# moberweger/deep-prior-pp

Measured on AMD Instinct MI355X. Metric: depth-crops/sec (NYU ResNet50 bs128) 1/2/4/8 GPU; mean 3D joint err (mm), higher is better.
Workload: dtype f32; 1 GPU; NYU posereg_embedding ResNet (type 0, 30-D PCA prior) train step: fused augment + fwd + bwd + ADAM, bs128/GPU fp32, 128x128x1 crops; global_batch=128, parallelism=dp1, augment=True, augment_pipelined=True, bn=local per-GPU batch statistics, launch_mode=native

## Files before the change

deep-prior-pp_amd/csrc/elementwise.hip:

```cpp
#include "dpp_common.h"

namespace {

__global__ __launch_bounds__(DPP_THREADS) void colsum_partial_kernel(const float* __restrict__ X, int M, int C, int rpb,
                                                                     float* __restrict__ partial) {
    __shared__ float s[DPP_THREADS];
    const int tid = threadIdx.x;
    const int RP = DPP_THREADS / C > 0 ? DPP_THREADS / C : 1;
    const int r_begin = blockIdx.x * rpb;
    const int r_end = (r_begin + rpb < M) ? r_begin + rpb : M;
    for (int c0 = 0; c0 < C; c0 += DPP_THREADS) {
        int cw = (C - c0 < DPP_THREADS) ? C - c0 : DPP_THREADS;
        int rp = DPP_THREADS / cw;
        int c = tid % cw, rr = tid / cw;
        float acc = 0.0f;
        if (rr < rp)
            for (int r = r_begin + rr; r < r_end; r += rp) acc += X[(size_t)r * C + c0 + c];
        s[tid] = acc;
        __syncthreads();
        if (tid < cw) {
            double a = 0.0;
            for (int j = 0; j < rp; ++j) a += (double)s[j * cw + tid];
            partial[(size_t)blockIdx.x * C + c0 + tid] = (float)a;
        }
        __syncthreads();
    }
    (void)RP;
}

__global__ __launch_bounds__(DPP_THREADS) void loss_sse_kernel(const float* __restrict__ out, const float* __restrict__ y, int n,
                                                               float inv_denom, float* __restrict__ cost,
                                                               float* __restrict__ dout) {
    __shared__ double s[DPP_THREADS];
    double acc = 0.0;
    for (int i = threadIdx.x; i < n; i += DPP_THREADS) {
        float d = out[i] - y[i];
        acc += (double)d * (double)d;
        if (dout) dout[i] = 2.0f * inv_denom * d;
    }
    s[threadIdx.x] = acc;
    __syncthreads();
    for (int w = DPP_THREADS / 2; w > 0; w >>= 1) {
        if ((int)threadIdx.x < w) s[threadIdx.x] += s[threadIdx.x + w];
        __syncthreads();
    }
    if (threadIdx.x == 0) cost[0] = (float)(s[0] * (double)inv_denom);
}

constexpr int RPL_THREADS = 1024;
__global__ __launch_bounds__(RPL_THREADS) void reduce_partials_loss_kernel(const float* __restrict__ partial, int nz, int n,
                                                                           const float* __restrict__ bias, int nbias, float* __restrict__ out,
                                                                           const float* __restrict__ y, float inv_denom,
                                                                           float* __restrict__ cost, float* __restrict__ dout) {
    __shared__ double s[RPL_THREADS / DPP_WAVE];
    double acc = 0.0;
    const bool vec = (n & 3) == 0 && ((reinterpret_cast<uintptr_t>(partial) | reinterpret_cast<uintptr_t>(out) | reinterpret_cast<uintptr_t>(y) |
                                       reinterpret_cast<uintptr_t>(dout)) & 15) == 0;
    if (vec) {
        const int n4 = n >> 2;
        for (int q = threadIdx.x; q < n4; q += RPL_THREADS) {
            float4 v[16];
            const int nzc = nz < 16 ? nz : 16;
#pragma unroll
            for (int z = 0; z < 16; ++z) v[z] = reinterpret_cast<const float4*>(partial + (size_t)(z < nzc ? z : 0) * n)[q];
            const float4 yv = reinterpret_cast<const float4*>(y)[q];
            const int i0 = q << 2;
            const float4 bv = bias ? make_float4(bias[i0 % nbias], bias[(i0 + 1) % nbias], bias[(i0 + 2) % nbias], bias[(i0 + 3) % nbias])
                                   : make_float4(0.f, 0.f, 0.f, 0.f);
            float4 t = v[0];
#pragma unroll
            for (int z = 1; z < 16; ++z)
                if (z < nzc) { t.x += v[z].x; t.y += v[z].y; t.z += v[z].z; t.w += v[z].w; }
            for (int z = 16; z < nz; ++z) {
                const float4 u = reinterpret_cast<const float4*>(partial + (size_t)z * n)[q];
                t.x += u.x; t.y += u.y; t.z += u.z; t.w += u.w;
            }
            t.x += bv.x; t.y += bv.y; t.z += bv.z; t.w += bv.w;
            reinterpret_cast<float4*>(out)[q] = t;
            const float d0 = t.x - yv.x, d1 = t.y - yv.y, d2 = t.z - yv.z, d3 = t.w - yv.w;
            acc += (double)d0 * (double)d0 + (double)d1 * (double)d1 + (double)d2 * (double)d2 + (double)d3 * (double)d3;
            if (dout) reinterpret_cast<float4*>(dout)[q] = make_float4(2.0f * inv_denom * d0, 2.0f * inv_denom * d1, 2.0f * inv_denom * d2, 2.0f * inv_denom * d3);
        }
    } else {
        for (int i = threadIdx.x; i < n; i += RPL_THREADS) {
            float v = 0.0f;
            for (int z = 0; z < nz; ++z) v += partial[(size_t)z * n + i];
            if (bias) v += bias[i % nbias];
            out[i] = v;
            const float d = v - y[i];
            acc += (double)d * (double)d;
            if (dout) dout[i] = 2.0f * inv_denom * d;
        }
    }
    for (int o = 32; o > 0; o >>= 1) acc += __shfl_xor(acc, o);
    if ((threadIdx.x & 63) == 0) s[threadIdx.x >> 6] = acc;
    __syncthreads();
    if (threadIdx.x == 0) {
        double tsum = 0.0;
        for (int w = 0; w < RPL_THREADS / DPP_WAVE; ++w) tsum += s[w];
        cost[0] = (float)(tsum * (double)inv_denom);
    }
}

__global__ __launch_bounds__(DPP_THREADS) void loss_sse_bcast_kernel(const float* __restrict__ out, const float* __restrict__ y, int n,
                                                                     float* __restrict__ cost, float* __restrict__ dout,
                                                                     float* __restrict__ err) {
    __shared__ double s[4][DPP_THREADS];
    double so = 0.0, soo = 0.0, sy = 0.0, syy = 0.0;
    for (int i = threadIdx.x; i < n; i += DPP_THREADS) {
        const double o = out[i], t = y[i];
        so += o; soo += o * o; sy += t; syy += t * t;
    }
    s[0][threadIdx.x] = so; s[1][threadIdx.x] = soo; s[2][threadIdx.x] = sy; s[3][threadIdx.x] = syy;
    __syncthreads();
    for (int w = DPP_THREADS / 2; w > 0; w >>= 1) {
        if ((int)threadIdx.x < w)
            for (int k = 0; k < 4; ++k) s[k][threadIdx.x] += s[k][threadIdx.x + w];
        __syncthreads();
    }
    const double B = (double)n, ybar = s[2][0] / B;
    if (threadIdx.x == 0) cost[0] = (float)((B * s[1][0] - 2.0 * s[0][0] * s[2][0] + B * s[3][0]) / (B * B));
    if (dout)
        for (int i = threadIdx.x; i < n; i += DPP_THREADS) dout[i] = (float)(2.0 / B * ((double)out[i] - ybar));
    if (err == nullptr) return;
    __syncthreads();
    double acc = 0.0, mx = 0.0;
    for (int p = threadIdx.x; p < n * n; p += DPP_THREADS) {
        const double e = fabs((double)out[p / n] - (double)y[p % n]);
        acc += e;
        mx = e > mx ? e : mx;
    }
    s[0][threadIdx.x] = acc; s[1][threadIdx.x] = mx;
    __syncthreads();
    for (int w = DPP_THREADS / 2; w > 0; w >>= 1) {
        if ((int)threadIdx.x < w) {
            s[0][threadIdx.x] += s[0][threadIdx.x + w];
            s[1][threadIdx.x] = s[1][threadIdx.x + w] > s[1][threadIdx.x] ? s[1][threadIdx.x + w] : s[1][threadIdx.x];
        }
        __syncthreads();
    }
    if (threadIdx.x == 0) { err[0] = (float)(s[0][0] / (B * B)); err[1] = (float)s[1][0]; }
}

__global__ __launch_bounds__(DPP_THREADS) void error_l2_kernel(const float* __restrict__ out, const float* __restrict__ y, int rows,
                                                               int d, float* __restrict__ err) {
    __shared__ double s[DPP_THREADS];
    __shared__ double smax[DPP_THREADS];
    double acc = 0.0, mx = 0.0;
    for (int r = threadIdx.x; r < rows; r += DPP_THREADS) {
        double q = 0.0;
        for (int j = 0; j < d; ++j) {
            double e = (double)out[(size_t)r * d + j] - (double)y[(size_t)r * d + j];
            q += e * e;
        }
        q = sqrt(q);
        acc += q;
        mx = q > mx ? q : mx;
    }
    s[threadIdx.x] = acc;
    smax[threadIdx.x] = mx;
    __syncthreads();
    for (int w = DPP_THREADS / 2; w > 0; w >>= 1) {
        if ((int)threadIdx.x < w) {
            s[threadIdx.x] += s[threadIdx.x + w];
            smax[threadIdx.x] = smax[threadIdx.x + w] > smax[threadIdx.x] ? smax[threadIdx.x + w] : smax[threadIdx.x];
        }
        __syncthreads();
    }
    if (threadIdx.x == 0) { err[0] = (float)(s[0] / (double)rows); err[1] = (float)smax[0]; }
}

__device__ __forceinline__ void adam_take_ticket(float* state) {
    __syncthreads();
    if (threadIdx.x == 0) {
        unsigned* ctr = reinterpret_cast<unsigned*>(state + 7);
        if (atomicAdd(ctr, 1u) == gridDim.x - 1) { *ctr = 0u; state[1] += 1.0f; }
    }
}

__global__ __launch_bounds__(DPP_THREADS) void adam_kernel(float* __restrict__ w, const float* __restrict__ g, float* __restrict__ m,
                                                           float* __restrict__ v, size_t n, float* state, int tick) {
    const float lr = state[0], t = state[1], beta1 = state[2], b2 = state[3], eps = state[4], gamma = state[5];
    if (state[6] != 0.0f) {
        const float od = 1.0f - b2;
        for (size_t i = (size_t)blockIdx.x * DPP_THREADS + threadIdx.x; i < n; i += (size_t)gridDim.x * DPP_THREADS) {
            const float gg = g[i];
            const float ms = b2 * v[i] + od * (gg * gg);
            w[i] = w[i] + (-lr * gg) / fmaxf(sqrtf(ms), eps);
            v[i] = ms;
        }
        if (tick) adam_take_ticket(state);
        return;
    }
    const float b1 = beta1 * powf(gamma, t - 1.0f);
    const float ob1 = 1.0f - b1, ob2 = 1.0f - b2;
    const float c1 = 1.0f - powf(beta1, t), c2 = 1.0f - powf(b2, t);
    const size_t n4 = n >> 2;
    for (size_t i = (size_t)blockIdx.x * DPP_THREADS + threadIdx.x; i < n4; i += (size_t)gridDim.x * DPP_THREADS) {
        float4 W = reinterpret_cast<float4*>(w)[i], G = reinterpret_cast<const float4*>(g)[i];
        float4 Mv = reinterpret_cast<float4*>(m)[i], V = reinterpret_cast<float4*>(v)[i];
#define DPP_ADAM1(f)                                            \
        Mv.f = b1 * Mv.f + ob1 * G.f;                           \
        V.f = b2 * V.f + ob2 * (G.f * G.f);                     \
        W.f = W.f - (lr * (Mv.f / c1)) / (sqrtf(V.f / c2) + eps);
        DPP_ADAM1(x) DPP_ADAM1(y) DPP_ADAM1(z) DPP_ADAM1(w)
        reinterpret_cast<float4*>(w)[i] = W;
        reinterpret_cast<float4*>(m)[i] = Mv;
        reinterpret_cast<float4*>(v)[i] = V;
    }
    if (blockIdx.x == 0 && threadIdx.x < (n & 3)) {
        size_t i = (n4 << 2) + threadIdx.x;
        float mm = b1 * m[i] + ob1 * g[i];
        float vv = b2 * v[i] + ob2 * (g[i] * g[i]);
        w[i] = w[i] - (lr * (mm / c1)) / (sqrtf(vv / c2) + eps);
        m[i] = mm;
        v[i] = vv;
    }
#undef DPP_ADAM1
    if (tick) adam_take_ticket(state);
}

__global__ void adam_tick_kernel(float* state) {
    if (threadIdx.x == 0 && blockIdx.x == 0) state[1] += 1.0f;
}

__global__ __launch_bounds__(DPP_THREADS) void axpy_kernel(float* __restrict__ y, const float* __restrict__ x, float alpha, size_t n) {
    for (size_t i = (size_t)blockIdx.x * DPP_THREADS + threadIdx.x; i < n; i += (size_t)gridDim.x * DPP_THREADS) y[i] += alpha * x[i];
}
// ... 270 lines not shown
```

deep-prior-pp_amd/csrc/fcgemm.hip:

```cpp
#include <stdlib.h>
#include "dpp_common.h"

namespace {

typedef __bf16 bf16x8 __attribute__((ext_vector_type(8)));
typedef __bf16 bf16x4 __attribute__((ext_vector_type(4)));

template <int PREC> struct Prec;
template <> struct Prec<0> {
    typedef float elem;
    static constexpr int EPT = 4;
    static constexpr int PAD = 4;
};
template <> struct Prec<1> {
    typedef __bf16 elem;
    static constexpr int EPT = 8;
    static constexpr int PAD = 8;
};

struct FcArgs {
    dpp_gemm_desc d;
    int vecA, vecB;
    int Kper;
};
// ... 64 lines not shown
                    for (int j = 0; j < NLD; ++j)
                        if (k + 4 * j < k_end) r[s][j] = fc_act4(fc_load4(p + ((4 * j) >> sh), k + 4 * j, k_end, vec, sh != 0), act, k + 4 * j, k_end);
                }
            } else {
                const int q = slot % (ROWS / 4), kr = slot / (ROWS / 4);
                const int row = r0 + q * 4, k = kc + kr * EPT;
                if (row < rlim) {
#pragma unroll
                    for (int j = 0; j < NLD; ++j)
                        if (k + j < k_end)
                            r[s][j] = fc_act4(fc_load4(base + (((size_t)dpp_map_row(map, k + j) * ld + row) >> sh), row, rlim, vec, sh != 0), act, row, rlim);
                }
            }
        }
    }

    __device__ __forceinline__ void commit(elem* img) const {
        const int tid = threadIdx.x;
#pragma unroll
        for (int s = 0; s < SLOTS; ++s) {
            const int slot = tid + s * DPP_THREADS;
            if (slot >= NSLOT) continue;
            if (KCONT) {
                const int row = slot / (KC / EPT), k = (slot % (KC / EPT)) * EPT;
                float v[EPT];
#pragma unroll
                for (int j = 0; j < NLD; ++j) { v[4 * j] = r[s][j].x; v[4 * j + 1] = r[s][j].y; v[4 * j + 2] = r[s][j].z; v[4 * j + 3] = r[s][j].w; }
                fc_store_run(img + row * LD + k, v);
            } else {
                const int q = slot % (ROWS / 4), kr = slot / (ROWS / 4);
#pragma unroll
                for (int e = 0; e < 4; ++e) {
                    float v[EPT];
#pragma unroll
                    for (int j = 0; j < EPT; ++j) v[j] = dpp_f4_get(r[s][j], e);
                    fc_store_run(img + (q * 4 + e) * LD + kr * EPT, v);
                }
            }
        }
    }
};

template <int PREC, int RM, int CN, int KC, bool AKC, bool BKC>
__global__ __launch_bounds__(DPP_THREADS) void fc_gemm_kernel(FcArgs ga) {
    dpp_kernarg_warm<sizeof(FcArgs)>();
    const dpp_gemm_desc& d = ga.d;
    typedef typename Prec<PREC>::elem elem;
    constexpr int EPT = Prec<PREC>::EPT;
    constexpr int BM = 64 * RM, BN = 16 * CN;
    typedef Stage<PREC, BM, KC, AKC> SA;
    typedef Stage<PREC, BN, KC, BKC> SB;
    constexpr int LD = KC + Prec<PREC>::PAD;
    constexpr int SZA = BM * LD, SZB = BN * LD;
    constexpr int OPB = 2 * (SZA + SZB) * (int)sizeof(elem);
    constexpr int EPB = (BM * (BN + 4) + 16 * BN) * 4;
    HIP_DYNAMIC_SHARED(float4, smem4)
    static_assert(OPB % 16 == 0, "buffer alignment");
    elem* const img = reinterpret_cast<elem*>(smem4);
    (void)EPB;

    const int tid = threadIdx.x, wave = tid >> 6, lane = tid & 63, l15 = lane & 15, kq = lane >> 4;
    const int row0 = blockIdx.x * BM, col0 = blockIdx.y * BN;
    const int M = d.M, N = d.N;
    const int k_begin = blockIdx.z * ga.Kper;
    const int k_end = (k_begin + ga.Kper < d.K) ? (k_begin + ga.Kper) : d.K;
    const int nchunks = (k_end > k_begin) ? (k_end - k_begin + KC - 1) / KC : 0;

    f32x4 acc[RM][CN];
#pragma unroll
    for (int i = 0; i < RM; ++i)
#pragma unroll
        for (int j = 0; j < CN; ++j) acc[i][j] = (f32x4){0.f, 0.f, 0.f, 0.f};
    dpp_wide_coef wco;
    wco.load<BN>(col0, N, d.splitk == 1 ? d.bias : nullptr, d.epi, d.splitk > 1 ? d.partial : d.C);

    SA sa;
    SB sb;
    const dpp_rowmap ident = {1, 0, 0, 0, 0};
    auto fetch = [&](int c) __attribute__((always_inline)) {
        const int kc = k_begin + c * KC;
        sa.fetch(d.A, d.lda, d.mapA, row0, M, kc, k_end, d.actA, ga.vecA, (d.store & DPP_ST_A) ? 1 : 0);
        sb.fetch(d.B, d.ldb, BKC ? ident : d.mapB, col0, N, kc, k_end, d.actB, ga.vecB);
    };
    if (nchunks > 0) fetch(0);
    for (int c = 0; c < nchunks; ++c) {
        elem* As = img + (c & 1) * (SZA + SZB);
        elem* Bs = As + SZA;
        sa.commit(As);
        sb.commit(Bs);
        if (c + 1 < nchunks) fetch(c + 1);
        __syncthreads();
#pragma unroll
        for (int k0 = 0; k0 < KC; k0 += 4 * EPT) {
            if constexpr (PREC == 0) {
                float af[RM][4], bf[CN][4];
#pragma unroll
                for (int rt = 0; rt < RM; ++rt) {
                    const float4 v = *reinterpret_cast<const float4*>(reinterpret_cast<const float*>(As) + (wave * (BM / 4) + rt * 16 + l15) * LD + k0 + kq * 4);
                    af[rt][0] = v.x; af[rt][1] = v.y; af[rt][2] = v.z; af[rt][3] = v.w;
                }
#pragma unroll
                for (int ct = 0; ct < CN; ++ct) {
                    const float4 v = *reinterpret_cast<const float4*>(reinterpret_cast<const float*>(Bs) + (ct * 16 + l15) * LD + k0 + kq * 4);
                    bf[ct][0] = v.x; bf[ct][1] = v.y; bf[ct][2] = v.z; bf[ct][3] = v.w;
                }
#pragma unroll
                for (int t = 0; t < 4; ++t)
#pragma unroll
                    for (int rt = 0; rt < RM; ++rt)
#pragma unroll
                        for (int ct = 0; ct < CN; ++ct)
                            acc[rt][ct] = __builtin_amdgcn_mfma_f32_16x16x4f32(af[rt][t], bf[ct][t], acc[rt][ct], 0, 0, 0);
            } else {
                bf16x8 af[RM], bf[CN];
#pragma unroll
                for (int rt = 0; rt < RM; ++rt)
                    af[rt] = *reinterpret_cast<const bf16x8*>(reinterpret_cast<const __bf16*>(As) + (wave * (BM / 4) + rt * 16 + l15) * LD + k0 + kq * 8);
#pragma unroll
                for (int ct = 0; ct < CN; ++ct)
                    bf[ct] = *reinterpret_cast<const bf16x8*>(reinterpret_cast<const __bf16*>(Bs) + (ct * 16 + l15) * LD + k0 + kq * 8);
#pragma unroll
                for (int rt = 0; rt < RM; ++rt)
#pragma unroll
                    for (int ct = 0; ct < CN; ++ct)
                        acc[rt][ct] = __builtin_amdgcn_mfma_f32_16x16x32_bf16(af[rt], bf[ct], acc[rt][ct], 0, 0, 0);
            }
        }
    }
    __syncthreads();

    const int nvalid = (M - row0 < BM) ? (M - row0) : BM;
    float* smem = reinterpret_cast<float*>(smem4);
    if (d.splitk > 1) {
        dpp_epilogue ep0 = {};
        float* P = d.partial + (size_t)blockIdx.z * M * N;
        dpp_epilogue_wide<RM, CN, 4, 1, BM, BN>(acc, smem, col0, N, wco, nullptr, P, ep0, nvalid, wave, 0, l15, kq, [&](int rl) {
            const int row = row0 + rl;
            return row < M ? (long)row * N : -1L;
        });
    } else {
        dpp_epilogue_wide<RM, CN, 4, 1, BM, BN>(acc, smem, col0, N, wco, d.residual, d.C, d.epi, nvalid, wave, 0, l15, kq, [&](int rl) {
            const int row = row0 + rl;
            return row < M ? (long)dpp_map_row(d.mapC, row) * d.ldc : -1L;
        });
    }
}


struct FsArgs {
    dpp_gemm_desc d;
    int Kper;
};

template <int PREC, int BN, bool AKC, bool BKC>
__global__ __launch_bounds__(DPP_THREADS) DPP_WAVES_PER_EU(1, 2) void fc_stream_kernel(FsArgs ga) {
    dpp_kernarg_warm<sizeof(FsArgs)>();
    const dpp_gemm_desc& d = ga.d;
    typedef typename Prec<PREC>::elem elem;
    constexpr int BM = 128, KC = 32, LD = KC + Prec<PREC>::PAD, NST = 3, WM = 2, WN = 2;
    constexpr int RM = BM / (16 * WM), CN = BN / (16 * WN);
    constexpr int SZA = BM * LD, SZB = BN * LD, SZ = SZA + SZB;
    HIP_DYNAMIC_SHARED(float4, smem4)
    elem* const img = reinterpret_cast<elem*>(smem4);
    auto put4 = [](elem* dst, float x, float y, float z, float w) __attribute__((always_inline)) {
        if constexpr (PREC == 0) *reinterpret_cast<float4*>(dst) = make_float4(x, y, z, w);
        else {
            bf16x4 o;
            o[0] = (__bf16)x; o[1] = (__bf16)y; o[2] = (__bf16)z; o[3] = (__bf16)w;
            *reinterpret_cast<bf16x4*>(dst) = o;
        }
    };
    const int tid = threadIdx.x, wave = tid >> 6, lane = tid & 63, l15 = lane & 15, kq = lane >> 4;
    const int wm = wave / WN, wn = wave % WN;
    const int row0 = blockIdx.x * BM, col0 = blockIdx.y * BN;
    const int M = d.M, N = d.N;
    const int k_begin = blockIdx.z * ga.Kper;
    const int nchunks = ga.Kper / KC;

    constexpr int SA = AKC ? BM / 32 : 4, SB = BKC ? BN / 32 : 4;
    const int shA = (d.store & DPP_ST_A) ? 1 : 0;
    const float* pa[SA];
    const float* pb[SB];
    int la, lb;
    bool bvalid = true;
    if (AKC) {
        const int r = tid >> 3, quad = (tid & 7) * 4;
#pragma unroll
        for (int s = 0; s < SA; ++s) pa[s] = d.A + (((size_t)(row0 + r + 32 * s) * d.lda + k_begin + quad) >> shA);
        la = r * LD + quad;
    } else {
        const int cq = tid % (BM / 4), kg = tid / (BM / 4);
#pragma unroll
        for (int s = 0; s < SA; ++s) pa[s] = d.A + (((size_t)(k_begin + 4 * kg + s) * d.lda + row0 + 4 * cq) >> shA);
        la = (4 * cq) * LD + 4 * kg;
    }
    if (BKC) {
        const int r = tid >> 3, quad = (tid & 7) * 4;
#pragma unroll
        for (int s = 0; s < SB; ++s) pb[s] = d.B + (size_t)(col0 + r + 32 * s) * d.ldb + k_begin + quad;
        lb = r * LD + quad;
    } else {
        const int cq = tid % (BN / 4), kg = tid / (BN / 4);
        bvalid = kg < KC / 4;
#pragma unroll
        for (int s = 0; s < SB; ++s) pb[s] = d.B + (size_t)(k_begin + 4 * (bvalid ? kg : 0) + s) * d.ldb + col0 + 4 * cq;
        lb = (4 * cq) * LD + 4 * kg;
    }
    const int modeA = d.actA.mode;
    float4 mu = make_float4(0.f, 0.f, 0.f, 0.f), sc = mu, be = mu;
    int cidx = 0;
    if (modeA & 2) {
        cidx = AKC ? (k_begin + (tid & 7) * 4) % d.actA.cmod : (row0 + 4 * (tid % (BM / 4))) % d.actA.cmod;
        if (!AKC) {
            mu = *reinterpret_cast<const float4*>(d.actA.mean + cidx);
            sc = *reinterpret_cast<const float4*>(d.actA.scale + cidx);
            be = *reinterpret_cast<const float4*>(d.actA.beta + cidx);
        }
    }
    float4 ra[SA];
    f32x4 rb[SB];
    const size_t stepA = AKC ? (size_t)KC : (size_t)KC * d.lda, stepB = BKC ? (size_t)KC : (size_t)KC * d.ldb;
    auto fetch = [&](int c) __attribute__((always_inline)) {
        if (AKC && (modeA & 2)) {
            mu = *reinterpret_cast<const float4*>(d.actA.mean + cidx);
            sc = *reinterpret_cast<const float4*>(d.actA.scale + cidx);
            be = *reinterpret_cast<const float4*>(d.actA.beta + cidx);
            cidx += KC;
            if (cidx >= d.actA.cmod) cidx -= d.actA.cmod;
        }
        if (shA) {
#pragma unroll
            for (int s = 0; s < SA; ++s) ra[s] = dpp_raw8(pa[s] + ((c * stepA) >> 1));
        } else {
#pragma unroll
            for (int s = 0; s < SA; ++s) ra[s] = *reinterpret_cast<const float4*>(pa[s] + c * stepA);
        }
        if (BKC || bvalid) {
#pragma unroll
            for (int s = 0; s < SB; ++s) rb[s] = *reinterpret_cast<const f32x4*>(pb[s] + c * stepB);
        }
    };
    auto act = [&](float4 v) __attribute__((always_inline)) {
        if (modeA & 2) {
            v.x = dpp_fma(v.x - mu.x, sc.x, be.x); v.y = dpp_fma(v.y - mu.y, sc.y, be.y);
            v.z = dpp_fma(v.z - mu.z, sc.z, be.z); v.w = dpp_fma(v.w - mu.w, sc.w, be.w);
        }
        if (modeA & 1) { v.x = fmaxf(v.x, 0.0f); v.y = fmaxf(v.y, 0.0f); v.z = fmaxf(v.z, 0.0f); v.w = fmaxf(v.w, 0.0f); }
        return v;
    };
    auto commit = [&](int buf) __attribute__((always_inline)) {
        elem* As = img + buf * SZ;
        elem* Bs = As + SZA;
        if constexpr (AKC) {
#pragma unroll
            for (int s = 0; s < SA; ++s) {
                const float4 w = shA ? dpp_widen4(ra[s]) : ra[s];
                const float4 v = modeA ? act(w) : w;
                put4(&As[la + 32 * s * LD], v.x, v.y, v.z, v.w);
            }
        } else {
            float4 v[4];
#pragma unroll
            for (int s = 0; s < 4; ++s) { const float4 w = shA ? dpp_widen4(ra[s]) : ra[s]; v[s] = modeA ? act(w) : w; }
            put4(&As[la + 0 * LD], v[0].x, v[1].x, v[2].x, v[3].x);
            put4(&As[la + 1 * LD], v[0].y, v[1].y, v[2].y, v[3].y);
            put4(&As[la + 2 * LD], v[0].z, v[1].z, v[2].z, v[3].z);
            put4(&As[la + 3 * LD], v[0].w, v[1].w, v[2].w, v[3].w);
        }
        if constexpr (BKC) {
#pragma unroll
            for (int s = 0; s < SB; ++s) {
                if constexpr (PREC == 0) *reinterpret_cast<f32x4*>(&Bs[lb + 32 * s * LD]) = rb[s];
                else put4(&Bs[lb + 32 * s * LD], rb[s][0], rb[s][1], rb[s][2], rb[s][3]);
            }
        } else if (bvalid) {
            put4(&Bs[lb + 0 * LD], rb[0][0], rb[1][0], rb[2][0], rb[3][0]);
            put4(&Bs[lb + 1 * LD], rb[0][1], rb[1][1], rb[2][1], rb[3][1]);
            put4(&Bs[lb + 2 * LD], rb[0][2], rb[1][2], rb[2][2], rb[3][2]);
            put4(&Bs[lb + 3 * LD], rb[0][3], rb[1][3], rb[2][3], rb[3][3]);
        }
    };

    f32x4 acc[RM][CN];
#pragma unroll
    for (int i = 0; i < RM; ++i)
#pragma unroll
        for (int j = 0; j < CN; ++j) acc[i][j] = (f32x4){0.f, 0.f, 0.f, 0.f};
    dpp_wide_coef wco;
    wco.load<BN>(col0, N, d.splitk == 1 ? d.bias : nullptr, d.epi, d.splitk > 1 ? d.partial : d.C);

    fetch(0);
    commit(0);
    if (nchunks > 1) fetch(1);
    __syncthreads();
    int cur = 0;
    constexpr int EPT = Prec<PREC>::EPT;
    const int aoff = (wm * (BM / WM) + l15) * LD + kq * EPT, boff = (wn * (BN / WN) + l15) * LD + kq * EPT;
    for (int c = 0; c < nchunks; ++c) {
        const int nxt = cur == NST - 1 ? 0 : cur + 1;
        if (c + 1 < nchunks) commit(nxt);
        if (c + 2 < nchunks) fetch(c + 2);
        const elem* As = img + cur * SZ;
        const elem* Bs = As + SZA;
        if constexpr (PREC == 0) {
#pragma unroll
            for (int k0 = 0; k0 < KC; k0 += 16) {
                float4 af[RM], bf[CN];
#pragma unroll
                for (int rt = 0; rt < RM; ++rt) af[rt] = *reinterpret_cast<const float4*>(&As[aoff + rt * 16 * LD + k0]);
#pragma unroll
                for (int ct = 0; ct < CN; ++ct) bf[ct] = *reinterpret_cast<const float4*>(&Bs[boff + ct * 16 * LD + k0]);
#pragma unroll
                for (int t = 0; t < 4; ++t)
#pragma unroll
                    for (int rt = 0; rt < RM; ++rt)
#pragma unroll
                        for (int ct = 0; ct < CN; ++ct)
                            acc[rt][ct] = __builtin_amdgcn_mfma_f32_16x16x4f32(dpp_f4_get(af[rt], t), dpp_f4_get(bf[ct], t), acc[rt][ct], 0, 0, 0);
            }
        } else {
            bf16x8 af[RM], bf[CN];
#pragma unroll
            for (int rt = 0; rt < RM; ++rt) af[rt] = *reinterpret_cast<const bf16x8*>(&As[aoff + rt * 16 * LD]);
#pragma unroll
            for (int ct = 0; ct < CN; ++ct) bf[ct] = *reinterpret_cast<const bf16x8*>(&Bs[boff + ct * 16 * LD]);
#pragma unroll
            for (int rt = 0; rt < RM; ++rt)
#pragma unroll
                for (int ct = 0; ct < CN; ++ct)
                    acc[rt][ct] = __builtin_amdgcn_mfma_f32_16x16x32_bf16(af[rt], bf[ct], acc[rt][ct], 0, 0, 0);
        }
        __syncthreads();
        cur = nxt;
    }

    float* smem = reinterpret_cast<float*>(smem4);
    if (d.splitk > 1) {
        dpp_epilogue ep0 = {};
        float* P = d.partial + (size_t)blockIdx.z * M * N;
        dpp_epilogue_wide<RM, CN, WM, WN, BM, BN>(acc, smem, col0, N, wco, nullptr, P, ep0, BM, wm, wn, l15, kq,
                                                  [&](int rl) { return (long)(row0 + rl) * N; });
    } else {
        dpp_epilogue_wide<RM, CN, WM, WN, BM, BN>(acc, smem, col0, N, wco, d.residual, d.C, d.epi, BM, wm, wn, l15, kq,
                                                  [&](int rl) { return (long)dpp_map_row(d.mapC, row0 + rl) * d.ldc; });
    }
}

template <int PREC, int BN, bool AKC, bool BKC>
int fs_launch(const FsArgs& ga, dim3 grid, hipStream_t st) {
    constexpr size_t opb = 3 * (size_t)(128 + BN) * (32 + Prec<PREC>::PAD) * sizeof(typename Prec<PREC>::elem);
    constexpr size_t epb = ((size_t)128 * (BN + 4) + 16 * BN) * 4;
    const size_t lds = opb > epb ? opb : epb;
    (void)hipFuncSetAttribute(reinterpret_cast<const void*>(&fc_stream_kernel<PREC, BN, AKC, BKC>), hipFuncAttributeMaxDynamicSharedMemorySize, (int)lds);
    DPP_LAUNCH((fc_stream_kernel<PREC, BN, AKC, BKC>), grid, dim3(DPP_THREADS), lds, st, ga);
    return dpp_launch_status();
}

template <int PREC, int BN>
int fs_dispatch(const FsArgs& ga, dim3 grid, hipStream_t st) {
    const dpp_gemm_desc& d = ga.d;
    if (d.a_kc && d.b_kc) return fs_launch<PREC, BN, true, true>(ga, grid, st);
    if (d.a_kc && !d.b_kc) return fs_launch<PREC, BN, true, false>(ga, grid, st);
    if (!d.a_kc && !d.b_kc) return fs_launch<PREC, BN, false, false>(ga, grid, st);
    return fs_launch<PREC, BN, false, true>(ga, grid, st);
}

bool fs_accepts(const dpp_gemm_desc& d, int& bn) {
    static const bool on = []() { const char* e = getenv("DPP_FC_STREAM3"); return !(e && e[0] == '0'); }();
    if (!on) return false;
    auto al = [](const void* p) { return (reinterpret_cast<uintptr_t>(p) & 15) == 0; };
    if (d.M % 128 || d.K % d.splitk || (d.K / d.splitk) % 32) return false;
    if (!al(d.A) || !al(d.B) || (d.lda & 3) || (d.ldb & 3)) return false;
    if (d.mapA.s != 1 || d.mapB.s != 1 || d.actB.mode != 0) return false;
    if (d.actA.mode & 2) {
        if ((d.actA.cmod & 3) || d.actA.cmod < 32) return false;
        if (!al(d.actA.mean) || !al(d.actA.scale) || !al(d.actA.beta)) return false;
    }
    bn = (d.N % 128 == 0 && (long)(d.M / 128) * (d.N / 128) * d.splitk >= 256) ? 128 : 64;
    return d.N % bn == 0;
}

template <int PREC, int RM, int CN, int KC, bool AKC, bool BKC>
int fc_launch(const FcArgs& ga, dim3 grid, hipStream_t st) {
    typedef typename Prec<PREC>::elem elem;
    constexpr int BM = 64 * RM, BN = 16 * CN, LD = KC + Prec<PREC>::PAD;
    constexpr size_t opb = 2 * (size_t)(BM + BN) * LD * sizeof(elem);
    constexpr size_t epb = ((size_t)BM * (BN + 4) + 16 * BN) * 4;
    const size_t lds = opb > epb ? opb : epb;
    if (lds > 64 * 1024)
        (void)hipFuncSetAttribute(reinterpret_cast<const void*>(&fc_gemm_kernel<PREC, RM, CN, KC, AKC, BKC>), hipFuncAttributeMaxDynamicSharedMemorySize, (int)lds);
    DPP_LAUNCH((fc_gemm_kernel<PREC, RM, CN, KC, AKC, BKC>), grid, dim3(DPP_THREADS), lds, st, ga);
    return dpp_launch_status();
}

template <int PREC, int KC>
int fc_dispatch(const FcArgs& ga, dim3 grid, hipStream_t st) {
    const dpp_gemm_desc& d = ga.d;
    if (d.a_kc && d.b_kc) return fc_launch<PREC, 2, 4, KC, true, true>(ga, grid, st);
    if (d.a_kc && !d.b_kc) return fc_launch<PREC, 2, 4, KC, true, false>(ga, grid, st);
    if (!d.a_kc && !d.b_kc) return fc_launch<PREC, 2, 4, KC, false, false>(ga, grid, st);
    return fc_launch<PREC, 2, 4, KC, false, true>(ga, grid, st);
}

}

extern "C" int dpp_fc_gemm(const dpp_gemm_desc* dp, int precision, int kchunk, dpp_stream_t stream) {
    if (!dp) return DPP_E_BADARG;
    const dpp_gemm_desc& d = *dp;
    if (!d.A || !d.B || d.M < 1 || d.N < 1 || d.K < 1 || d.splitk < 1) return DPP_E_BADARG;
    if (d.splitk > 1 ? !d.partial : !d.C) return DPP_E_BADARG;
    if (precision != 0 && precision != 1) return DPP_E_BADARG;
    if (d.actA.mode > 3 || d.actB.mode > 3 || d.epi.stats || d.epi.bn_x) return DPP_E_UNSUPPORTED;
    if (d.N % 4) return DPP_E_UNSUPPORTED;
    if (d.store & ~DPP_ST_A) return DPP_E_UNSUPPORTED;
    if ((d.store & DPP_ST_A) && ((reinterpret_cast<uintptr_t>(d.A) & 15) || (d.lda & 3))) return DPP_E_UNSUPPORTED;
    const int ldc = d.splitk > 1 ? d.N : d.ldc;
    if (ldc % 4 || (reinterpret_cast<uintptr_t>(d.splitk > 1 ? d.partial : d.C) & 15)) return DPP_E_UNSUPPORTED;
    if (d.residual && (reinterpret_cast<uintptr_t>(d.residual) & 15)) return DPP_E_UNSUPPORTED;
    if (d.splitk == 1 && d.bias && (reinterpret_cast<uintptr_t>(d.bias) & 15)) return DPP_E_UNSUPPORTED;
    const int KC = kchunk == 0 ? 64 : kchunk;
    if (KC != 32 && KC != 64) return DPP_E_BADARG;
    hipStream_t st = static_cast<hipStream_t>(stream);
    int bn3 = 0;
    static const bool fs_bf16 = []() { const char* e = getenv("DPP_FC_STREAM3_BF16"); return !(e && e[0] == '0'); }();
    if ((precision == 0 || fs_bf16) && fs_accepts(d, bn3)) {
        FsArgs fa;
        fa.d = d;
        fa.Kper = d.K / d.splitk;
        dim3 g3(d.M / 128, d.N / bn3, d.splitk);
        if (precision == 0) return bn3 == 128 ? fs_dispatch<0, 128>(fa, g3, st) : fs_dispatch<0, 64>(fa, g3, st);
        return bn3 == 128 ? fs_dispatch<1, 128>(fa, g3, st) : fs_dispatch<1, 64>(fa, g3, st);
    }
    FcArgs ga;
    ga.d = d;
    auto aligned = [](const float* p, int ld) { return (reinterpret_cast<uintptr_t>(p) & 15) == 0 && (ld & 3) == 0; };
    ga.vecA = aligned(d.A, d.lda);
    ga.vecB = aligned(d.B, d.ldb);
    int per = (d.K + d.splitk - 1) / d.splitk;
    per = (per + KC - 1) / KC * KC;
    ga.Kper = per;
    dim3 grid(dpp_cdiv(d.M, 128), dpp_cdiv(d.N, 64), d.splitk);
    if (precision == 0) return KC == 64 ? fc_dispatch<0, 64>(ga, grid, st) : fc_dispatch<0, 32>(ga, grid, st);
    return KC == 64 ? fc_dispatch<1, 64>(ga, grid, st) : fc_dispatch<1, 32>(ga, grid, st);
}
```

deep-prior-pp_amd/hipdp/backward.py:

```python
import numpy as np

from . import ops
from . import heuristics as hz
from .lib import Act, RowMap
from .store import TensorV, View, _layer_kind, _pad4


class BackwardMixin(object):
    def _grad_dtype(self, t, flattened=False):
        if not self.grad16 or not t.is16 or flattened or t.rows <= 256:
            return np.float32
        for io in self.layer_io.values():
            if io.get('out') is t and io.get('stem'):
                return np.float32
        return np.uint16

    def _view_grad(self, view):
        if view.plain:
            t = view.base
            if t.grad is None:
                t.grad = self.rt.alloc(t.shape, self._grad_dtype(t), zero=False)
            return t, t.grad
        key = view.key()
        vg = self.view_grads.get(key)
# ... 246 lines not shown
        rpb = max(32, -(-rows // 256))
        nb = -(-rows // rpb)
        part = self.rt.alloc(nb * C, zero=False)
        self.bwd.add(ops.colsum_partial(self.rt, dY, rows, C, rpb, part), side=True)
        self.bwd.add(ops.reduce_partials(self.rt, part, nb, C, gslot), side=True)

    def _bwd_conv(self, layer, io, src, dY, dY_act=None, dY_keep=None):
        rt, st = self.rt, self.store
        c = layer.cfgParams
        N, Hi, Wi, Ci = src.base.shape
        _, Co, Ho, Wo = c.outputDim
        k, s = tuple(c.filterDim), c.stride[0]
        M = N * Ho * Wo
        act = self._act(src)
        gW, gb = self._grad_view(layer.W), self._grad_view(layer.b)
        if io.get('residual') is not None:
            io['residual'].pending.append(dY)
        need_dx = src.base not in self.x_ins

        def emit_param_grads(dy, dy_act):
            self.bwd.fork()
            if dY_act is None:
                self._bias_grad(dy, M, Co, gb)
            else:
                assert k == (1, 1) and io.get('residual') is None
                self.reduce_jobs.add(dy, 0, Co, gb)
            if k != (1, 1):
                return
            mp = RowMap.strided(s, Ho, Wo, Hi, Wi) if s != 1 else None
            rpw = hz.wgrad_stream_rows(M)
            if dy_act is None and hz.WGRAD_STREAM and rpw > 0 and rt.lib.dpp_wgrad_stream_slices(Co, Ci, M, rpw) > 0:
                nsl = rt.lib.dpp_wgrad_stream_slices(Co, Ci, M, rpw)
                part = rt.alloc(nsl * Co * Ci, zero=False)
                p16 = int(bool(self._gemm_prec(0, M, role='wgrad') and rt.lib.dpp_wgrad_stream_bf16_ok(Co, Ci)))
                self.bwd.add(ops.wgrad_stream(rt, dy, Co, src.base.buf, Ci, M, rpw, part, mapX=mp, actX=act,
                                              name='wgrad1x1_%d' % layer.layerNum, precision=p16), side=True)
                self.reduce_jobs.add(part, nsl, Co * Ci, gW)
                return
            tile, splitk = hz.wgrad_plan(Co, Ci, M)
            part = rt.alloc(splitk * Co * Ci, zero=False) if splitk > 1 else None
            self.bwd.add(ops.gemm(rt, dy, src.base.buf, None if splitk > 1 else gW, Co, Ci, M, 0, 0, Co, Ci, Ci, mapB=mp, actA=dy_act,
                                  actB=act, splitk=splitk, partial=part, tile=tile, name='wgrad1x1_%d' % layer.layerNum,
                                  precision=self._gemm_prec(0, M, lazy=dy_act is not None, role='wgrad')), side=True)
            if splitk > 1:
                self.reduce_jobs.add(part, splitk, Co * Ci, gW)

        if dY_keep is None:
            emit_param_grads(dY, dY_act)
        if k == (1, 1):
            mp = RowMap.strided(s, Ho, Wo, Hi, Wi) if s != 1 else None
            if need_dx:
                tgt, dst = self._view_grad(src)
                acc = tgt.grad_written
                if s != 1 and not acc:
                    self.early_side.append(ops.fill_zero(rt, dst))
                tile, _ = hz.gemm_plan(M, Ci, Co, allow_split=False)
                rs = hz.rowstream_plan(M, Ci, Co, False)
                if rs is not None:
                    tile = rs
                ks = hz.ksplit_plan(M, Ci, Co) if (s == 1 and rs is None and dY_act is None) else None
                if ks is not None:
                    tile = ks
                ex = hz.expand_plan(M, Ci, Co, False) if (s == 1 and rs is None and ks is None) else None
                s16 = hz.stream16_plan(M, Ci, Co, False) if (s == 1 and rs is None and ks is None and dY_act is None and ex is None) else None
                if s16 is not None:
                    tile = s16
                if ex is not None:
                    tile = ex
                variant = 1 if (rs is not None and dY_act is None) else (2 if ks is not None else (4 if ex is not None else (3 if s16 is not None else 0)))

                def build(tile, variant, epi):
                    return ops.gemm(rt, dY, st.view(layer.W), dst, M, Ci, Co, 1, 0, Co, Ci, Ci, mapC=mp, actA=dY_act,
                                    residual=dst if acc else None, tile=tile, epi=epi, variant=variant,
                                    name='dgrad1x1_%d' % layer.layerNum,
                                    precision=self._gemm_prec(variant, Co, lazy=dY_act is not None, role='dgrad'))
                if variant in (2, 3, 4) and ops.gemm_variant_rows(rt, build(tile, variant, None)) != tile[0]:
                    variant, (tile, _) = 0, hz.gemm_plan(M, Ci, Co, allow_split=False)
                epi = None
                if (s == 1 and not acc and self._sole_consumer_bn_view(src)) or (acc and self._two_conv1x1_consumers(src)):
                    nb2 = -(-M // tile[0])
                    tgt.fused_reduce = (rt.alloc((nb2, 2, Ci), zero=False), nb2)
                    epi = ops.epilogue(bn=src.bn, bn_x=src.base.buf, bn_relu=src.relu, bn_partial=tgt.fused_reduce[0])
                self.bwd.add(build(tile, variant, epi))
                tgt.grad_written = True
            if dY_keep is not None:
                assert need_dx
                emit_param_grads(dY_keep, None)
        else:
            bm = 64
            p16 = int(bool(self.prec and hz.BF16_WGRAD3 and Ci == Co and rt.lib.dpp_conv3x3_wgrad_bf16_ok(N, Hi, Wi, Ci, Co)))
            rpw = hz.wgrad3_stream_rows(N * Hi * Wi, Ci) if (Ci == Co and not p16) else 0
            nblk = rt.lib.dpp_wgrad3_stream_slices(Co, Ci, N, Hi, Wi, rpw) if rpw > 0 else 0
            if nblk > 0:
                part = rt.alloc(nblk * Co * 9 * Ci, zero=False)
                self.bwd.add(ops.wgrad3_stream(rt, dY, Co, src.base.buf, Ci, N, Hi, Wi, rpw, part, actX=act), side=True)
            else:
                nblk = rt.lib.dpp_conv3x3_wgrad_blocks(N, Hi, Wi, Ci, Co, bm)
                part = rt.alloc(nblk * Co * 9 * Ci, zero=False)
                self.bwd.add(ops.conv3x3_wgrad(rt, src.base.buf, N, Hi, Wi, Ci, dY, Co, part, actX=act, bm=bm, precision=p16,
                                               name='wgrad3x3_%d' % layer.layerNum), side=True)
            self.reduce_jobs.add(part, nblk, Co * 9 * Ci, gW)
            if need_dx:
                tgt, dst = self._view_grad(src)
                acc = tgt.grad_written
                Wd = rt.alloc(Co * 9 * Ci, zero=False)
                self._wtrans_jobs.append((st.view(layer.W), Co, Ci, Wd))
                bmd = hz.conv3x3_bm(N * Hi * Wi, Ci, hw=(Hi, Wi), prec=self.prec)
                epi = None
                fuse = not acc and self._sole_consumer_bn_view(src)
                if not acc and self._conv3_stream(N, Hi, Wi, Ci, Co, dY, dst, src.base.buf if fuse else None):
                    if fuse:
                        nb2 = N * Hi * Wi // rt.lib.dpp_conv3x3_stream_rows(N, Hi, Wi, Ci)
                        tgt.fused_reduce = (rt.alloc((nb2, 2, Ci), zero=False), nb2)
                        epi = ops.epilogue(bn=src.bn, bn_x=src.base.buf, bn_relu=src.relu, bn_partial=tgt.fused_reduce[0])
                    self.bwd.add(ops.conv3x3_stream(rt, dY, N, Hi, Wi, Ci, Wd, dst, epi=epi, name='dgrad3x3_%d' % layer.layerNum))
                    tgt.grad_written = True
                    return
                if fuse:
                    nb2 = rt.lib.dpp_conv3x3_tiling(N, Hi, Wi, bmd, None, None, None)
                    tgt.fused_reduce = (rt.alloc((nb2, 2, Ci), zero=False), nb2)
                    epi = ops.epilogue(bn=src.bn, bn_x=src.base.buf, bn_relu=src.relu, bn_partial=tgt.fused_reduce[0])
                self.bwd.add(ops.conv3x3(rt, dY, N, Hi, Wi, Co, Wd, Ci, dst, residual=dst if acc else None, bm=bmd, epi=epi,
                                         name='dgrad3x3_%d' % layer.layerNum, precision=self.prec))
                tgt.grad_written = True

    def _bwd_fc(self, layer, io, src, dY):
        rt, st = self.rt, self.store
        Nb, K = src.shape
        Nout = layer.cfgParams.outputDim[1]
        gW, gb = self._grad_view(layer.W), self._grad_view(layer.b)
        act = self._act(src)
        self.bwd.fork()
        self._bias_grad(dY, Nb, Nout, gb)
        stream_kernel = self._fc1_stream(Nb, K, Nout)
        if stream_kernel and self.prec == 0 and hz.FC1_WGRAD_STREAM and (act is None or act.mode < 4) and rt.lib.dpp_fc_wgrad_stream_ok(Nb, K, Nout):
            op = self.bwd.add(ops.fc_wgrad_stream(rt, src.base.buf, dY, gW, Nb, K, Nout, actX=act, name='fc_wgrad_%d' % layer.layerNum), side=True)
            if K * Nout >= hz.EARLY_BUCKET_MIN:
                self._fc1_wgrad_op = op
        elif stream_kernel:
            op = self.bwd.add(ops.fc_gemm(rt, src.base.buf, dY, gW, K, Nout, Nb, 0, 0, K, Nout, Nout, actA=act, precision=self.prec,
                                          kchunk=hz.FC1_KCHUNK, name='fc_wgrad_%d' % layer.layerNum), side=True)
            if K * Nout >= hz.EARLY_BUCKET_MIN:
                self._fc1_wgrad_op = op
        else:
            tile, _ = hz.gemm_plan(K, Nout, Nb, allow_split=False)
            if K >= 4096 and Nout >= 64 and hz.knob('DPP_FC1_TILE128', '1') != '0':
                tile = (128, 64, 4)
            self.bwd.add(ops.gemm(rt, src.base.buf, dY, gW, K, Nout, Nb, 0, 0, K, Nout, Nout, actA=act, tile=tile,
                                  name='fc_wgrad_%d' % layer.layerNum), side=True)
        if self.dp is not None and self._early_slice is None and K * Nout >= hz.EARLY_BUCKET_MIN and hz.OVERLAP_ALLREDUCE:
            off = (gW.ptr - st.g.ptr) // 4
            self._early_slice = (off, off + K * Nout)
            self.bwd.add(self.dp.allreduce_sum_async_op(gW, self._early_work, 'grad_allreduce_early'), side=True)
        if src.base not in self.x_ins:
            tgt, dst = self._view_grad(src)
            acc = tgt.grad_written
            tile, splitk = hz.gemm_plan(Nb, K, Nout, allow_split=not acc)
            if stream_kernel:
                self.bwd.add(ops.fc_gemm(rt, dY, st.view(layer.W), dst, Nb, K, Nout, 1, 1, Nout, Nout, K, residual=dst if acc else None,
                                         precision=self.prec, kchunk=hz.FC1_KCHUNK, name='fc_dgrad_%d' % layer.layerNum))
            elif splitk > 1:
                part = self.scratch(splitk * Nb * K)
                self.bwd.add(ops.gemm(rt, dY, st.view(layer.W), None, Nb, K, Nout, 1, 1, Nout, Nout, K, splitk=splitk, partial=part,
                                      tile=tile, name='fc_dgrad_%d' % layer.layerNum))
                self.bwd.add(ops.reduce_partials(rt, part, splitk, Nb * K, dst))
            else:
                self.bwd.add(ops.gemm(rt, dY, st.view(layer.W), dst, Nb, K, Nout, 1, 1, Nout, Nout, K, residual=dst if acc else None,
                                      tile=tile, name='fc_dgrad_%d' % layer.layerNum))
            tgt.grad_written = True
            if getattr(src.base, 'concat_parts', None) is not None:
                self._split_concat_grad(src.base)
        if self._early_adam is None and K * Nout >= hz.EARLY_BUCKET_MIN and gW.ptr >= st.g.ptr and \
                gW.ptr + 4 * K * Nout <= st.g.ptr + 4 * st.n_w:
            off = (gW.ptr - st.g.ptr) // 4
            self._early_adam = dict(after=self.bwd.ops[-1][0], lo=off, hi=off + K * Nout, W=layer.W)

    def _bwd_convpool(self, layer, io, dY):
        rt, st = self.rt, self.store
        g, src = io['geom'], io['in_view']
        nW = g['Co'] * g['kh'] * g['kw'] * g['Ci']
        self.bwd.fork()
        self._bias_grad(dY, io['out'].rows, g['Co'], self._grad_view(layer.b))
        nblk = rt.lib.dpp_convpool_wgrad_blocks(g['N'], g['Hp'], g['Wp'])
        part = rt.alloc(nblk * nW, zero=False)
        self.bwd.add(ops.convpool_wgrad(rt, src.base.buf, g['N'], g['H'], g['W'], g['Ci'], dY, io['ties'], g['kh'], g['kw'], g['pad'],
                                        g['Co'], g['pool'], part, actX=self._act(src), name='convpool_wgrad_%d' % layer.layerNum), side=True)
        self.reduce_jobs.add(part, nblk, nW, self._grad_view(layer.W))
        if src.base not in self.x_ins:
            tgt, dst = self._view_grad(src)
            if tgt.grad_written:
                raise NotImplementedError("ConvPoolLayer input with several consumers")
            self.bwd.add(ops.convpool_dgrad(rt, dY, io['ties'], g['N'], g['H'], g['W'], g['Ci'], st.view(layer.W), g['kh'], g['kw'],
                                            g['pad'], g['Co'], g['pool'], dst, name='convpool_dgrad_%d' % layer.layerNum))
            tgt.grad_written = True

    def _bwd_stem(self, layer, io, dY):
        if not io.get('stem', True):
            return self._bwd_convpool(layer, io, dY)
        rt, st = self.rt, self.store
        N, H, W, _ = self.in_shape
        Co = layer.cfgParams.nFilters
        out = io['out']
        self.bwd.fork()
        self._bias_grad(dY, out.rows, Co, self._grad_view(layer.b))
        tpb = 8
        nblk = rt.lib.dpp_stem_wgrad_blocks(N, H, W, tpb)
        part = rt.alloc(nblk * Co * 25, zero=False)
        self.bwd.add(ops.stem_wgrad(rt, self.x_in.buf, N, H, W, dY, io['argmax'], Co, part, tpb),
                     side=hz.knob('DPP_STEM_WGRAD_SIDE', '0') == '1')
        self.reduce_jobs.add(part, nblk, Co * 25, self._grad_view(layer.W))
```

deep-prior-pp_amd/hipdp/engine.py:

```python
import os
from ctypes import c_int as C_int

import numpy as np

from . import evalfuse, layout, ops
from . import heuristics as hz
from .lib import Act, RowMap
from .ops import Plan
from .runtime import default_runtime
from .backward import BackwardMixin
from .store import BNState, ParamStore, TensorV, View, _collect, _dedupe_specs, _layer_kind, _pad4, _param_specs, bf16_bits_to_f32, get_store


class CompiledNet(BackwardMixin):
    def __init__(self, net, train=False, runtime=None, loss=None, weight_decay=0.0, dp=None, fuse_bn=True, bf16=None, optimizer=None,
                 fuse_blocks=None):
        self.rt = rt = runtime or default_runtime()
        self.optimizer = dict(optimizer) if optimizer else dict(name='ADAM')
        self.prec = int(bool(hz.BF16_DEFAULT if bf16 is None else bf16))
        self.store16 = self.grad16 = False
        self.dp = dp
        self.fuse_bn = bool(fuse_bn) and not (dp is not None and dp.sync_bn)
        self.net, self.train = net, train
        self.N = net.cfgParams.batch_size
        self.key = None
        self.weight_decay = float(weight_decay)
        self.order, self.consumers, self.layers = _collect(net)
        resnet_like = all(_layer_kind(l) != 'ConvPoolLayer' or (tuple(l.cfgParams.filterDim) == (5, 5) and tuple(l.cfgParams.poolsize) == (2, 2)
                                                                 and l.cfgParams.nFilters <= 32 and l.cfgParams.activation is None)
                          for l in self.layers) and not any(v.kind == 'concat' for v in self.order)
        self.store16 = bool(self.prec and hz.BF16_STORE and resnet_like)
        self.grad16 = bool(self.store16 and hz.BF16_GRADS)
        self.store = get_store(net, rt, self.layers)
        self.fwd, self.bwd, self.upd = Plan('forward'), Plan('backward'), Plan('update')
        self.views = {}
        self.tensors = []
        self.bn_states = {}
        self.layer_io = {}
        self.view_grads = {}
        self._scratch = None
        self._bn_scratch = None
        self.colsum_of = {}
        self.reduce_jobs = ops.ReduceJobs(rt)
        self.dropout_masks = {}
        self.step_ctr = rt.alloc(1, np.int64) if train else None
        in_dims = net.cfgParams.inputDim
        in_vars = net.inputVar
        if not isinstance(in_vars, (list, tuple)):
            in_dims, in_vars = [in_dims], [in_vars]
        self.x_ins, self.input_of = [], {}
        for k, (d, v) in enumerate(zip(in_dims, in_vars)):
            shp = (d[0], d[2], d[3], d[1])
            t = TensorV(rt.alloc(shp), shp, 'x%d' % k)
            self.x_ins.append(t)
            self.input_of[id(v)] = t
        self.x_in, self.in_shape = self.x_ins[0], self.x_ins[0].shape
        self._memo = {}
        self.fuse_blocks = (hz.EVAL_FUSE if fuse_blocks is None else bool(fuse_blocks)) and not train
        self.fused_blocks = []
        self._bn_eval_jobs = []
        self._beside = []
        self._bwd_after = {}
        out_view = self._emit(net.output)
        if self._bn_eval_jobs:
            self.fwd.ops[0:0] = [(ops.bn_eval_coeffs_multi(rt, self._bn_eval_jobs), False)]
        self.out = self._materialize_plain(out_view)
        self.out_dim = int(np.prod(self.out.shape[1:]))
        self.loss_cfg = loss
        if loss is not None:
            self.y_in = rt.alloc((self.N, self.out_dim))
            self.cost = rt.alloc(1)
            self.err = rt.alloc(2)
            self.lossplan = Plan('loss')
            gN = self.N * (dp.world if (dp is not None and train) else 1)
            denom = gN if loss.get('kind', 'embedding') in ('embedding', 'scalar') else gN * loss['numJoints']
            if train:
                self.out.grad = rt.alloc(self.out.shape)
                self.out.grad_written = True
            if loss.get('kind') == 'scalar':
                if self.out_dim != 1:
                    raise ValueError("the scalar cost needs a one-dimensional output")
                if dp is not None and train:
                    raise NotImplementedError("the broadcast cost of the scalar target couples all samples of the global batch")
                self.lossplan.add(ops.loss_sse_bcast(rt, self.out.buf, self.y_in, self.N, self.cost, self.out.grad if train else None,
                                                     err=None if train else self.err))
            else:
                last = self.fwd.ops[-1][0] if self.fwd.ops else None
                fus = getattr(self, '_loss_fusable', None)
                if (train and hz.FUSE_LOSS and fus is not None and fus[0] is last and fus[1]['out'] is self.out.buf
                        and self.N * self.out_dim <= 65536):
                    f = fus[1]
                    self.fwd.ops[-1] = (ops.reduce_partials_loss(rt, f['partial'], f['nz'], self.N, self.out_dim, self.out.buf, f['bias'], self.y_in,
                                                                 denom, self.cost, self.out.grad), False)
                else:
                    self.lossplan.add(ops.loss_sse(rt, self.out.buf, self.y_in, self.N, self.out_dim, denom, self.cost,
                                                   self.out.grad if train else None))
            if self.weight_decay and not net.hasDropout():
                share = self.weight_decay / (dp.world if (dp is not None and train) else 1)
                seg = self._weight_segments()
                if seg is not None:
                    self.lossplan.add(ops.sumsq_multi(rt, self.store.w, seg[0], seg[1], share, self.cost, 1))
                else:
                    for W in self._unique_weights():
                        self.lossplan.add(ops.sumsq(rt, self.store.view(W), int(np.prod(W.shape)), share, self.cost, 1))
            if not train and loss.get('kind') != 'scalar':
                d = loss['nDims'] if loss.get('kind', 'embedding') == 'joints' else self.out_dim
                rows = self.N * (loss['numJoints'] if loss.get('kind', 'embedding') == 'joints' else 1)
                self.lossplan.add(ops.error_l2(rt, self.out.buf, self.y_in, rows, d, self.err))
        if train:
            if loss is None:
                raise ValueError("a training engine needs a loss")
            self.store.ensure_train_buffers()
            self.hyper = rt.alloc(8)
            self.early_side = []
            self._early_slice, self._early_work = None, [None]
            self._early_adam = None
            self._wtrans_jobs = []
            self._emit_backward()
            if self._wtrans_jobs:
                self.early_side.append(ops.conv3x3_wtrans_multi(rt, self._wtrans_jobs))
            if self.early_side:
                self.fwd.ops[0:0] = [(ops.Fork(), False)] + [(o, True) for o in self.early_side]
                self.fwd.uses_side = True
                self.bwd.ops[0:0] = [(ops.Join(), False)]
            self._grad_allreduce = []
            if dp is not None:
                dp.broadcast_store(self.store)
                lo, hi = self._early_slice if self._early_slice is not None else (0, 0)
                n = self.store.g.size
                if self._early_slice is not None:
                    self._grad_allreduce.append(dp.wait_op(self._early_work, 'grad_allreduce_wait_early'))
                for a, b in ((0, lo), (hi, n)) if self._early_slice is not None else ((0, n),):
                    if b > a:
                        self._grad_allreduce.append(dp.allreduce_sum_op(self.store.g.view(a, (b - a,)), 'grad_allreduce'))
                self._grad_allreduce += self._wd_ops
                for op in self._grad_allreduce:
                    self.upd.add(op)
            self.upd.add(ops.adam(rt, self.store.w, self.store.g, self.store.m, self.store.v, self.store.n_w, self.hyper, tick=hz.ADAM_TICKED))
            if not hz.ADAM_TICKED:
                self.upd.add(ops.adam_tick(rt, self.hyper))
            if self.dropout_masks:
                self.upd.add(ops.counter_add(rt, self.step_ctr, 1))
            self._lr = None
            self.reset_optimizer()

    def scratch(self, nfloats):
        if self._scratch is None or self._scratch.size < nfloats:
            self._scratch = self.rt.alloc(max(nfloats, 1 << 20), zero=False)
        return self._scratch

    def scratch_side(self, nfloats):
        if getattr(self, '_scratch2', None) is None or self._scratch2.size < nfloats:
            self._scratch2 = self.rt.alloc(max(nfloats, 1 << 20), zero=False)
        return self._scratch2

    def _new_tensor(self, shape, name, act=False):
        t = TensorV(self.rt.alloc(shape, np.uint16 if (act and self.store16) else np.float32, zero=False), shape, name)
        self.tensors.append(t)
        return t

    def _drop_tensor(self, t):
        self.tensors = [u for u in self.tensors if u is not t]

    def _gemm_prec(self, variant, K, lazy=False, role='fwd'):
        if not (self.prec and hz.BF16_GEMM) or lazy or variant == 1:
            return 0
        if variant == 4:
            return int(K >= 32 or (K == 16 and hz.BF16_GEMM_ALL))
        if not hz.BF16_GEMM_ALL or role not in hz.BF16_GEMM_ROLES or str(variant) not in hz.BF16_GEMM_VARIANTS:
            return 0
        return int(variant in (2, 3) or K > 16)

    def _act(self, view):
        mode = (Act.BN if view.bn is not None else 0) | (Act.RELU if view.relu else 0)
        if mode == 0:
            return None
        if view.bn is not None:
            b = view.bn
            return ops.act(mode, b.mean, b.scale, b.beta_buf, view.chan)
        return ops.act(mode, None, None, None, view.chan)

    def _grad_view(self, param):
        uses = self.__dict__.setdefault('_grad_uses', {})
        n = uses.get(param.auto_name, 0)
        uses[param.auto_name] = n + 1
        slot = self.store.view(param, 'g')
        if n == 0:
            return slot
        priv = self.rt.alloc(slot.size, zero=False)
        self.__dict__.setdefault('_shared_grad_adds', []).append((slot, priv))
        return priv

    def _unique_weights(self):
        seen, out = set(), []
        for l in self.layers:
            if hasattr(l, 'W') and l.W.auto_name not in seen:
                seen.add(l.W.auto_name)
                out.append(l.W)
        return out

    def _weight_segments(self):
        if '_wseg' not in self.__dict__:
            st = self.store
            Ws = self._unique_weights()
            ok = bool(Ws) and all(st.slots[st.by_param[W.auto_name]]['trained'] for W in Ws)
            self._wseg = ops.segment_table(self.rt, st.w, [st.view(W) for W in Ws]) if ok else None
        return self._wseg

    def _fc1_stream(self, Nb, K, Nout):
        if not hz.is_fc1_shape(Nb, K, Nout) or hz.FC1_STREAM == '0':
            return False
        if hz.FC1_STREAM == '1' or self.prec == 1:
            return True
        if hz.FC1_STREAM != 'auto':
            return False
# ... 18 lines not shown
            src = self._emit(var.inputs[0])
            n = src.shape[0]
            v = View(src.base, src.bn, src.relu, shape=(n, int(np.prod(src.shape[1:]))), chan=src.base.C)
        elif k == 'relu':
            src = self._emit(var.inputs[0], residual)
            if src.relu:
                v = src
            else:
                v = View(src.base, src.bn, True, shape=src.shape, chan=src.chan)
        elif k == 'add':
            v = self._emit_add(var)
        elif k == 'concat':
            v = self._emit_concat(var)
        elif k == 'layer':
            v = self._emit_layer(var, residual, out_var)
        else:
            raise NotImplementedError("graph node '%s'" % k)
        if residual is None:
            self._memo[id(var)] = v
        return v

    def _emit_concat(self, var):
        parts = [self._emit(p) for p in var.inputs]
        if any(p.base.is16 for p in parts):
            raise NotImplementedError("concatenation of bf16-stored maps")
        N = parts[0].shape[0]
        widths = [int(p.shape[1]) for p in parts]
        total = sum(widths)
        cat = self._new_tensor((N, total), 'concat')
        cat.concat_parts = []
        off = 0
        for p, w in zip(parts, widths):
            if p.bn is not None or len(p.shape) != 2 or int(np.prod(p.base.shape[1:])) != w:
                raise NotImplementedError("concatenation of anything but flattened (ReLU) maps")
            self.fwd.add(ops.copy2d(self.rt, p.base.buf, w, cat.buf.view(off, (N * total - off,)), total, N, w, relu=p.relu,
                                    name='concat_pack'))
            cat.concat_parts.append((p, off, w))
            off += w
        return View(cat)

    def _split_concat_grad(self, cat):
        N, total = cat.shape
        for p, off, w in cat.concat_parts:
            if p.base in self.x_ins:
                continue
            tgt, dst = self._view_grad(p)
            if tgt.grad_written:
                raise NotImplementedError("concatenated value with another consumer")
            self.bwd.add(ops.copy2d(self.rt, cat.grad.view(off, (N * total - off,)), total, dst, w, N, w, name='concat_split'))
            tgt.grad_written = True

    def _emit_add(self, var):
        a, b = var.inputs
        if self.fuse_blocks:
            fused = evalfuse.emit_block(self, var)
            if fused is not None:
                return fused

        def fusable(x):
            return x.kind == 'layer' and _layer_kind(x.layer) in ('ConvLayer',) and self._single_consumer(x) \
                and x.layer.cfgParams.activation is None

        cand = [x for x in (a, b) if fusable(x)]
        if not cand:
            raise NotImplementedError("residual add whose operands are not conv outputs")
        q = max(cand, key=lambda x: (self._depth(x) if hz.SIDE_SHORTCUT else 0, x.layer.layerNum))
        p = b if q is a else a
        beside = hz.SIDE_SHORTCUT and self.train and p in cand and id(p) not in self._memo
        if beside:
            self._emit(p.inputs[0])
            n0 = len(self.fwd.ops)
        pv = self._emit(p)
        if not pv.plain:
            raise NotImplementedError("residual add on a non-materialised operand")
        if beside:
            moved = list(self.fwd.ops[n0:])
            if all(isinstance(op, ops.Launch) for op, _ in moved):
                fork = ops.Fork()
                self.fwd.ops[n0:] = [(fork, False)] + [(op, True) for op, _ in moved]
                self.fwd.uses_side = True
                self._emit(q.inputs[0])
                self.fwd.join()
                self._beside.append(([id(fork), id(self.fwd.ops[-1][0])], [id(op) for op, _ in moved]))
        if p.kind == 'layer' and p.layer.layerNum > q.layer.layerNum:
            self._bwd_after[id(p.layer)] = q.layer
        out = self._emit(q, residual=pv.base, out_var=var)
        self._memo[id(q)] = out
        return out

    def _depth(self, var):
        memo = self.__dict__.setdefault('_depth_memo', {})
        if id(var) not in memo:
            d = max([self._depth(i) for i in getattr(var, 'inputs', None) or []] or [0])
            memo[id(var)] = d + (1 if var.kind == 'layer' else 0)
        return memo[id(var)]

    def _feeds_batchnorm(self, var):
        for c in self.consumers.get(id(var), []):
            if c.kind == 'layer' and _layer_kind(c.layer) == 'BatchNormLayer':
                return True
        return False

    def _emit_layer(self, var, residual, out_var=None):
        layer = var.layer
        kind = _layer_kind(layer)
        rt, st = self.rt, self.store
        src = self._emit(var.inputs[0])
        if kind == 'BatchNormLayer':
            if not src.plain:
                raise NotImplementedError("BatchNorm on a non-materialised input")
            C = src.base.C
            M = src.base.rows
            sync = self.train and self.dp is not None and self.dp.sync_bn
            b = BNState(layer, C, M, self.dp.world if sync else 1)
            b.mean, b.inv_std, b.scale = (rt.alloc(_pad4(C)) for _ in range(3))
            b.beta_buf, b.gamma_buf = st.view(layer.beta), st.view(layer.gamma)
            b.run_mean, b.run_inv_std = st.view(layer.mean), st.view(layer.inv_std)
            self.bn_states[id(layer)] = b
            fused = getattr(src.base, 'stats', None) if self.train else None
            if fused is not None:
                part, nblk, rows = fused
                self.fwd.add(ops.bn_finalize(rt, part, nblk, M, rows, C, b.gamma_buf, layer.cfgParams.epsilon, b.mean, b.inv_std,
                                             b.scale, b.run_mean, b.run_inv_std, layer.cfgParams.alpha))
            elif self.train:
                W = b.world
                part = self.scratch(b.nb * 2 * C * (W + 1)).view(0, (b.nb * 2 * C,))
                self.fwd.add(ops.bn_stats_partial(rt, src.base.buf, M, C, b.rpb, part))
                if W > 1:
                    allp = self.scratch(b.nb * 2 * C * (W + 1)).view(b.nb * 2 * C, (W * b.nb * 2 * C,))
                    self.fwd.add(self.dp.all_gather_op(part, allp, 'bn_stats_allgather'))
                    part = allp
                self.fwd.add(ops.bn_finalize(rt, part, b.nb, M * W, b.rpb, C, b.gamma_buf, layer.cfgParams.epsilon, b.mean, b.inv_std,
                                             b.scale, b.run_mean, b.run_inv_std, layer.cfgParams.alpha, nseg=W))
            elif hz.EVAL_FUSE:
                self._bn_eval_jobs.append((b.gamma_buf, b.run_mean, b.run_inv_std, C, b.mean, b.inv_std, b.scale))
            else:
                self.fwd.add(ops.bn_eval_coeffs(rt, b.gamma_buf, b.run_mean, b.run_inv_std, C, b.mean, b.inv_std, b.scale))
            v = View(src.base, b, False, shape=src.shape, chan=src.chan)
            v.var = var
            return v
        if kind == 'NonlinearityLayer':
            if layer.cfgParams.activation is None:
                return src
            if layer.cfgParams.activation_str != 'ReLU':
                raise NotImplementedError("only ReLU is on the hot path")
            v = View(src.base, src.bn, True, shape=src.shape, chan=src.chan)
            v.var = var
            return v
        if kind == 'ConvPoolLayer':
            return self._emit_stem(layer, src, out_var if out_var is not None else var)
        if kind == 'ConvLayer':
            return self._emit_conv(layer, src, residual, out_var if out_var is not None else var)
        if kind == 'HiddenLayer':
            return self._emit_fc(layer, src)
        if kind == 'DropoutLayer':
            return self._emit_dropout(layer, src)
        raise NotImplementedError(kind)

    def _emit_stem(self, layer, src, out_var=None):
        c = layer.cfgParams
        N, H, W, Ci = src.base.shape
        ok = (src.base is self.x_in and Ci == 1 and tuple(c.filterDim) == (5, 5) and c.border_mode == 'half' and
              tuple(c.poolsize) == (2, 2) and tuple(c.stride) == (1, 1) and c.activation is None and c.nFilters <= 32)
        if not ok:
            return self._emit_convpool(layer, src)
        Co = c.nFilters
        out = self._new_tensor((N, H // 2, W // 2, Co), 'stem', act=True)
        arg = self.rt.alloc((N, H // 2, W // 2, Co), np.uint8, zero=False) if self.train else None
        stats = None
        if self.train and self.fuse_bn and H % 16 == 0 and W % 16 == 0 and out_var is not None and self._feeds_batchnorm(out_var):
            nblk = N * (H // 16) * (W // 16)
            out.stats = (self.rt.alloc((nblk, 2, Co), zero=False), nblk, 64)
            stats = out.stats[0]
        self.fwd.add(ops.stem_fwd(self.rt, src.base.buf.reshape(N, H, W), N, H, W, self.store.view(layer.W), self.store.view(layer.b), Co,
                                  out.buf, arg, stats))
        self.layer_io[id(layer)] = dict(in_view=src, out=out, argmax=arg, stem=True)
        return View(out)

    def _emit_convpool(self, layer, src):
        c = layer.cfgParams
        N, H, W, Ci = src.base.shape
        kh, kw = c.filterDim[0], c.filterDim[1]
        if len(src.shape) != 4:
            raise NotImplementedError("ConvPoolLayer on a flattened input")
        if self.store16:
            raise NotImplementedError("bf16 storage is built for the ResNet path (stem + ConvLayer); the generic ConvPoolLayer kernels are f32")
        if c.border_mode not in ('valid', 'half') or tuple(c.stride) != (1, 1) or c.poolsize[0] != c.poolsize[1]:
            raise NotImplementedError("ConvPoolLayer border %s stride %s pool %s" % (c.border_mode, c.stride, c.poolsize))
        if c.border_mode == 'half' and (kh % 2 == 0 or kw % 2 == 0):
            raise NotImplementedError("'half' padding with an even filter size")
        pad = kh // 2 if c.border_mode == 'half' else 0
        if c.border_mode == 'half' and kh != kw:
            raise NotImplementedError("'half' padding with a non-square filter")
        pool, Co = int(c.poolsize[0]), c.nFilters
        _, Co_, Hp, Wp = c.outputDim
        assert Co_ == Co
        out = self._new_tensor((N, Hp, Wp, Co), 'convpool%d' % layer.layerNum)
        ties = self.rt.alloc((N, Hp, Wp, Co), np.uint16, zero=False) if (self.train and pool > 1) else None
        geom = dict(N=N, H=H, W=W, Ci=Ci, kh=kh, kw=kw, pad=pad, Co=Co, pool=pool, Hp=Hp, Wp=Wp)
        self.fwd.add(ops.convpool_fwd(self.rt, src.base.buf, N, H, W, Ci, self.store.view(layer.W), kh, kw, pad, Co, pool,
                                      self.store.view(layer.b), out.buf, ties, actX=self._act(src), name='convpool_%d' % layer.layerNum))
        self.layer_io[id(layer)] = dict(in_view=src, out=out, ties=ties, geom=geom, stem=False)
        return View(out)

    def _emit_conv(self, layer, src, residual, out_var=None):
        c = layer.cfgParams
        N, Hi, Wi, Ci = src.base.shape
        _, Co, Ho, Wo = c.outputDim
        k, s = tuple(c.filterDim), tuple(c.stride)
        if c.border_mode != 'half' or k not in ((1, 1), (3, 3)) or s[0] != s[1] or (k == (3, 3) and s != (1, 1)):
            raise NotImplementedError("ConvLayer %s stride %s border %s" % (k, s, c.border_mode))
        out = self._new_tensor((N, Ho, Wo, Co), 'conv%d' % layer.layerNum, act=True)
        act = self._act(src)
        rt, st = self.rt, self.store
        res = residual.buf if residual is not None else None
        want_stats = self.train and self.fuse_bn and out_var is not None and self._feeds_batchnorm(out_var)
        M = N * Ho * Wo
        epi = None
        if k == (1, 1):
            tile, _ = hz.gemm_plan(M, Co, Ci, allow_split=False)
            rs = hz.rowstream_plan(M, Co, Ci, True)
            if rs is not None:
                tile = rs
            ks = hz.ksplit_plan(M, Co, Ci) if (s[0] == 1 and rs is None) else None
            if ks is not None:
                tile = ks
            ex = hz.expand_plan(M, Co, Ci, True) if (s[0] == 1 and rs is None and ks is None) else None
            s16 = hz.stream16_plan(M, Co, Ci, True) if (s[0] == 1 and rs is None and ks is None and ex is None) else None
            if s16 is not None:
                tile = s16
            if ex is not None:
                tile = ex
            mp = RowMap.strided(s[0], Ho, Wo, Hi, Wi) if s[0] != 1 else None
            variant = 1 if rs is not None else (2 if ks is not None else (4 if ex is not None else (3 if s16 is not None else 0)))

            def build(tile, variant, epi):
                return ops.gemm(rt, src.base.buf, st.view(layer.W), out.buf, M, Co, Ci, 1, 1, Ci, Ci, Co, mapA=mp, actA=act,
                                bias=st.view(layer.b), residual=res, tile=tile, epi=epi, variant=variant,
                                name='conv1x1_%d' % layer.layerNum, precision=self._gemm_prec(variant, Ci))
            if variant in (2, 3, 4) and ops.gemm_variant_rows(rt, build(tile, variant, None)) != tile[0]:
                variant, (tile, _) = 0, hz.gemm_plan(M, Co, Ci, allow_split=False)
            if want_stats:
                nblk = -(-M // tile[0])
                out.stats = (rt.alloc((nblk, 2, Co), zero=False), nblk, tile[0])
                epi = ops.epilogue(stats=out.stats[0])
            self.fwd.add(build(tile, variant, epi))
        elif self._conv3_stream(N, Hi, Wi, Ci, Co, src.base.buf, out.buf) and residual is None:
            rows = rt.lib.dpp_conv3x3_stream_rows(N, Hi, Wi, Ci)
            if want_stats:
                out.stats = (rt.alloc((M // rows, 2, Co), zero=False), M // rows, rows)
                epi = ops.epilogue(stats=out.stats[0])
            self.fwd.add(ops.conv3x3_stream(rt, src.base.buf, N, Hi, Wi, Ci, st.view(layer.W), out.buf, actX=act, bias=st.view(layer.b), epi=epi,
                                            name='conv3x3_%d' % layer.layerNum))
        else:
            bm = hz.conv3x3_bm(M, Co, hw=(Hi, Wi), prec=self.prec)
            if want_stats:
                th, tw, img = (C_int() for _ in range(3))
                nblk = rt.lib.dpp_conv3x3_tiling(N, Hi, Wi, bm, th, tw, img)
                if Hi % th.value == 0 and Wi % tw.value == 0 and (N % img.value == 0 or nblk == 1):
                    out.stats = (rt.alloc((nblk, 2, Co), zero=False), nblk, bm)
                    epi = ops.epilogue(stats=out.stats[0])
            self.fwd.add(ops.conv3x3(rt, src.base.buf, N, Hi, Wi, Ci, st.view(layer.W), Co, out.buf, actX=act, bias=st.view(layer.b),
                                     residual=res, bm=bm, epi=epi, name='conv3x3_%d' % layer.layerNum, precision=self.prec))
        self.layer_io[id(layer)] = dict(in_view=src, out=out, residual=residual)
        return View(out)

    def _conv3_stream(self, N, H, W, Ci, Co, *bufs):
        if Ci != Co or Ci not in hz.CONV3_STREAM_C or self.prec:
            return False
        if any(b is not None and b.dtype == ops.BF16 for b in bufs):
            return False
        return self.rt.lib.dpp_conv3x3_stream_rows(N, H, W, Ci) > 0

    def _emit_fc(self, layer, src):
        c = layer.cfgParams
        if len(src.shape) != 2:
            raise NotImplementedError("HiddenLayer on a non-flattened input")
        Nb, K = src.shape
        Nout = c.outputDim[1]
        assert K == c.inputDim[1], (K, c.inputDim)
        out = self._new_tensor((Nb, Nout), 'fc%d' % layer.layerNum)
        rt, st = self.rt, self.store
        act = self._act(src)
        if self._fc1_stream(Nb, K, Nout):
            splitk = max(1, min(hz.FC1_SLICES, K // 512))
            part = self.scratch(splitk * Nb * Nout)
            self.fwd.add(ops.fc_gemm(rt, src.base.buf, st.view(layer.W), None, Nb, Nout, K, 1, 0, K, Nout, Nout, actA=act, splitk=splitk,
                                     partial=part, precision=self.prec, kchunk=hz.FC1_KCHUNK, name='fc_%d' % layer.layerNum))
            self.fwd.add(ops.reduce_partials(rt, part, splitk, Nb * Nout, out.buf, bias=st.view(layer.b), nbias=Nout))
            self.layer_io[id(layer)] = dict(in_view=src, out=out)
            return View(out)
        tile, splitk = hz.gemm_plan(Nb, Nout, K)
        if K >= 4096 and Nb <= 128 and Nout >= 64:
            tile, splitk = ((128, 64, 4) if Nb > 64 and hz.knob('DPP_FC1_TILE128', '1') != '0' else (64, 64, 4)), max(1, K // 512)
        act = self._act(src)
        if splitk > 1:
            part = self.scratch(splitk * Nb * Nout)
            self.fwd.add(ops.gemm(rt, src.base.buf, st.view(layer.W), None, Nb, Nout, K, 1, 0, K, Nout, Nout, actA=act, splitk=splitk,
                                  partial=part, tile=tile, name='fc_%d' % layer.layerNum))
            red = self.fwd.add(ops.reduce_partials(rt, part, splitk, Nb * Nout, out.buf, bias=st.view(layer.b), nbias=Nout))
            self._loss_fusable = (red, dict(partial=part, nz=splitk, bias=st.view(layer.b), out=out.buf))
        else:
            self.fwd.add(ops.gemm(rt, src.base.buf, st.view(layer.W), out.buf, Nb, Nout, K, 1, 0, K, Nout, Nout, actA=act,
                                  bias=st.view(layer.b), tile=tile, name='fc_%d' % layer.layerNum))
        self.layer_io[id(layer)] = dict(in_view=src, out=out)
        return View(out)

    def _emit_dropout(self, layer, src):
        if src.bn is not None or len(src.shape) != 2:
            raise NotImplementedError("DropoutLayer after BatchNorm / on a 4-D map")
        n = int(np.prod(src.shape))
        out = self._new_tensor(src.shape, 'drop%d' % layer.layerNum)
        keep = np.float32(1.0 - layer.cfgParams.p)
        mask = None
        if self.train:
            mask = self.rt.alloc(src.shape)
            self.dropout_masks[id(layer)] = (mask, float(keep), layer.mask_seed)
            rank = self.dp.rank if self.dp is not None else 0
            self.fwd.add(ops.bernoulli_mask(self.rt, mask, n, float(keep), layer.mask_seed, (layer.layerNum << 40) + (rank << 32), self.step_ctr))
        self.fwd.add(ops.scale(self.rt, src.base.buf, out.buf, n, a=keep, relu=src.relu, mask=mask))
        self.layer_io[id(layer)] = dict(in_view=src, out=out, mask=mask)
        return View(out)

    def set_input(self, x):
        xs = x if isinstance(x, (list, tuple)) else [x]
        if len(xs) != len(self.x_ins):
            raise ValueError("the net takes %d inputs, got %d" % (len(self.x_ins), len(xs)))
        for t, a in zip(self.x_ins, xs):
            a = np.asarray(a, np.float32)
            want = (t.shape[0], t.shape[3], t.shape[1], t.shape[2])
            if tuple(a.shape) != want:
                raise ValueError("input shape %s, expected %s" % (a.shape, want))
            t.buf.set(a if a.shape[1] == 1 else layout.nchw_to_nhwc(a))

    def forward(self, x=None):
        self.store.check_live()
        if x is not None:
            self.set_input(x)
        self.fwd.run(self.rt)
        return self.out.buf.get()

    def reset_optimizer(self, lr=0.0):
        f = np.float32
        o = self.optimizer
        if o.get('name', 'ADAM') == 'RMSProp':
            self.hyper.set(np.array([f(lr), f(1.0), 0, f(o.get('decay', 0.9)), f(o.get('epsilon', 1.0 / 100.)), 0, 1, 0], np.float32))
        else:
            self.hyper.set(np.array([f(lr), f(1.0), f(o.get('beta1', 0.9)), f(o.get('beta2', 0.999)), f(o.get('epsilon', 1e-8)),
                                     f(o.get('gamma', 1 - 1e-8)), 0, 0], np.float32))
        self.store.m.zero()
        self.store.v.zero()
        self._lr = float(lr)

    def set_lr(self, lr):
        if self._lr != float(np.float32(lr)):
            self.hyper.view(0, (1,)).set(np.array([lr], np.float32))
            self._lr = float(np.float32(lr))

    def run_step_plans(self, allreduce=None):
        st = self.rt
        self.store.check_live()
        if allreduce is None:
            self.step_plan().run(st)
            return
        self.fwd.run(st)
        self.lossplan.run(st)
        self.bwd.run(st)
        allreduce(self.store.g)
        self.upd.run(st)

    def step_plan(self, before=None, prefetch=None, early=None):
        key = (id(before) if before is not None else 0, id(prefetch) if prefetch is not None else 0, id(early) if early is not None else 0)
        cache = self.__dict__.setdefault('_step_plans', {})
        if key not in cache:
            bwd, upd = self._early_adam_plans()
            fwd = self.fwd
            if early is not None and self._beside:
                marks = set(m for ms, _ in self._beside for m in ms)
                chain = set(o for _, os_ in self._beside for o in os_)
                fwd = Plan('forward')
                fwd.ops = [(op, side and id(op) not in chain) for (op, side) in self.fwd.ops if id(op) not in marks]
                fwd.uses_side = getattr(self.fwd, 'uses_side', False)
            parts = ([before] if before is not None else []) + [fwd, self.lossplan, bwd]
            if prefetch is not None:
                pre, post = Plan('prefetch_join'), Plan('prefetch')
                pre.join()
                post.fork()
                for op in prefetch.steps():
                    post.add(op, side=True)
                parts = [pre] + parts + [post]
            if early is not None:
                head = Plan('early')
                head.fork()
                for op in early.steps():
                    head.add(op, side=True)
                at = 1 if prefetch is not None else 0
                parts = parts[:at] + [head] + parts[at:]
            plan = Plan.concat('step', parts + [upd])
            skip = tuple(x for x in hz.knob('DPP_WHATIF_SKIP', '').split(',') if x)
            if skip:
                plan.ops = [(op, side) for (op, side) in plan.ops if not str(getattr(op, 'name', '')).startswith(skip)]
            cache[key] = (before, prefetch, early, plan)
        return cache[key][-1]

    def _early_adam_plans(self):
        ea = self._early_adam
        if not hz.EARLY_ADAM or ea is None or self.dp is not None:
            return self.bwd, self.upd
        if '_early_adam_cache' in self.__dict__:
            return self._early_adam_cache
        rt, st = self.rt, self.store
        lo, hi, n = ea['lo'], ea['hi'], st.n_w
        sl = lambda b, a, z: b.view(a, (z - a,))
        bwd = Plan('backward')
        early = [o for o in self._wd_ops if self._wd_of.get(id(o)) == ea['W'].auto_name]
        early.append(ops.adam(rt, sl(st.w, lo, hi), sl(st.g, lo, hi), sl(st.m, lo, hi), sl(st.v, lo, hi), hi - lo, self.hyper, name='adam_fc1'))
        pos = 1 + [i for i, (op, _) in enumerate(self.bwd.ops) if op is ea['after']][0]
        head = list(self.bwd.ops[:pos])
        tail = [(op, side) for (op, side) in self.bwd.ops[pos:] if not any(op is e for e in early)]
        bwd.ops = head + [(ops.Fork(), False)] + [(o, True) for o in early] + tail
        bwd.uses_side = True
        upd = Plan('update')
        for a, z in ((0, lo), (hi, n)):
            if z > a:
                upd.add(ops.adam(rt, sl(st.w, a, z), sl(st.g, a, z), sl(st.m, a, z), sl(st.v, a, z), z - a, self.hyper))
        if hz.ADAM_TICKED:
            upd.add(ops.adam_tick(rt, self.hyper))
        for (op, side) in self.upd.ops:
            if getattr(op, 'name', '') != 'adam':
                upd.add(op, side)
        self._early_adam_cache = (bwd, upd)
        return self._early_adam_cache

    def train_step_device(self, lr, allreduce=None):
        self.set_lr(lr)
        self.run_step_plans(allreduce)

    def train_step(self, x, y, lr):
        self.set_input(x)
        self.y_in.set(np.asarray(y, np.float32).reshape(self.N, self.out_dim))
        self.train_step_device(lr)
        return float(self.cost.get()[0])

    def cost_and_grads(self, x, y):
        self.set_input(x)
        self.y_in.set(np.asarray(y, np.float32).reshape(self.N, self.out_dim))
        st = self.rt
        self.fwd.run(st)
        self.lossplan.run(st)
        self.bwd.run(st)
        return float(self.cost.get()[0]), self.out.buf.get()

    def global_cost(self):
        c = float(self.cost.get()[0])
        if self.dp is None:
            return c
        import torch
        t = torch.tensor([c], dtype=torch.float64)
        if self.dp.dist.get_backend() == 'nccl':
# ... 22 lines not shown
```

deep-prior-pp_amd/hipdp/heuristics.py:

```python
import os

def knob(name, default):
    if os.environ.get('DPP_EXPERIMENT', '0') != '1':
        return default
    return os.environ.get(name, default)


BN_RPB_TARGET_BLOCKS = int(knob('DPP_BN_BLOCKS', '1024'))
BN_BWD_FUSE_MAX_BLOCKS = int(knob('DPP_BN_BWD_FUSE_NB', '0'))
BN_BWD_FUSE_TARGET_WGS = int(knob('DPP_BN_BWD_FUSE_WGS', '512'))



GEMM_TARGET_BLOCKS = int(knob('DPP_GEMM_TARGET_BLOCKS', '1024'))


def gemm_plan(M, N, K, allow_split=True):
    if M <= 16:
        bm, bn, wm = 16, 64, 1
    elif M <= 32:
        bm, bn, wm = 32, 64, 1
    else:
        wm = 4
        cands = [(128, 64), (64, 64), (128, 32), (64, 32), (128, 16), (64, 16)]
        if knob('DPP_NO_128x64', '1') != '0':
            cands = cands[1:]
        cands = [(a, b) for (a, b) in cands if b <= max(16, 16 * (-(-N // 16))) or b == 16]
        bm, bn = cands[-1]
        for (a, b) in cands:
            if (-(-M // a)) * (-(-N // b)) >= GEMM_TARGET_BLOCKS:
                bm, bn = a, b
                break
    tiles = (-(-M // bm)) * (-(-N // bn))
    splitk = 1
    if allow_split and tiles < 512 and K >= 256:
        splitk = int(min(max(1, 2048 // tiles), max(1, K // 128), 256))
    return (bm, bn, wm), splitk


EVAL_FUSE = knob('DPP_EVAL_FUSE', '1') != '0'
FUSE_LOSS = knob('DPP_FUSE_LOSS', '1') != '0'
ADAM_TICKED = knob('DPP_ADAM_TICKED', '1') != '0'
EVAL_FUSE_BF16 = knob('DPP_EVAL_FUSE_BF16', '1') != '0'
OVERLAP_ALLREDUCE = knob('DPP_OVERLAP_ALLREDUCE', '1') != '0'
EARLY_BUCKET_MIN = int(knob('DPP_EARLY_BUCKET_MIN', str(1 << 22)))
LAZY_BN_BWD = int(knob('DPP_LAZY_BN_BWD', '0'))
BF16_DEFAULT = os.environ.get('DPP_BF16', '0') == '1'
BF16_STORE = knob('DPP_BF16_STORE', '1') != '0'
BF16_GRADS = knob('DPP_BF16_GRADS', '1') != '0'
BF16_GEMM = knob('DPP_BF16_GEMM', '1') != '0'
BF16_GEMM_ALL = knob('DPP_BF16_GEMM_ALL', '1') != '0'
BF16_GEMM_ROLES = tuple(knob('DPP_BF16_GEMM_ROLES', 'fwd,dgrad,wgrad').split(','))
BF16_GEMM_VARIANTS = tuple(knob('DPP_BF16_GEMM_VARIANTS', '0,2,3').split(','))
BF16_WGRAD3 = knob('DPP_BF16_WGRAD3', '1') != '0'
EARLY_ADAM = knob('DPP_EARLY_ADAM', '0') != '0'
EARLY_REDUCE_BYTES = int(knob('DPP_EARLY_REDUCE_MB', '0')) << 20
TAIL_REDUCE = knob('DPP_TAIL_REDUCE', '0') != '0'
FC1_STREAM = knob('DPP_FC1_STREAM', 'auto')
FC1_WGRAD_STREAM = knob('DPP_FC1_WGRAD_STREAM', '1') != '0'
FC1_WGRAD_DEFER = int(knob('DPP_FC1_WGRAD_DEFER', '0'))
FC1_KCHUNK = int(knob('DPP_FC1_KCHUNK', '0'))
FC1_SLICES = int(knob('DPP_FC1_SLICES', '32'))
FC1_MIN_K = int(knob('DPP_FC1_MIN_K', '4096'))


def is_fc1_shape(Nb, K, Nout):
    return K >= FC1_MIN_K and Nout >= 64 and Nout % 4 == 0 and K % 4 == 0
ROWSTREAM = knob('DPP_ROWSTREAM', '0') != '0'

def rowstream_plan(M, N, K, b_kc):
    if not ROWSTREAM or M < 2048:
        return None
    K16 = (K + 15) // 16 * 16
    for bn in (64, 32, 16):
        if bn > 16 and bn >= 2 * N:
            continue
        lds = (bn * (K16 + 4) if b_kc else K16 * (bn + 4)) * 4
        if lds > 48 * 1024:
            continue
        bm = 128 if (M // 128) * (-(-N // bn)) >= 1024 else 64
        return (bm, bn, 4)
    return None


KSPLIT = int(knob('DPP_KSPLIT', '2'))
KSPLIT_MAX_M = int(knob('DPP_KSPLIT_MAX_M', '65536'))


def ksplit_plan(M, N, K):
    if KSPLIT <= 0 or M % 32 or M > KSPLIT_MAX_M * (2 if K == 128 else 1):
        return None
    if K == 256 and N % 64 == 0:
        return (32, 64, 4)
    if K == 128 and N % 32 == 0 and KSPLIT >= 2:
        return (32, 32, 4)
    return None


STREAM16 = int(knob('DPP_STREAM16', '2'))
STREAM16_MIN_M = int(knob('DPP_STREAM16_MIN_M', '128'))


def stream16_plan(M, N, K, forward):
    if STREAM16 <= 0 or M < STREAM16_MIN_M:
        return None
    if N == 16 and K == 64 and M % 128 == 0:
        return (128, 16, 4)
    if N == 64 and K == 16 and M % 64 == 0 and (STREAM16 >= 3 or (STREAM16 >= 2 and not forward)):
        return (64, 64, 4)
    return None


EXPAND = int(knob('DPP_EXPAND', '3'))
EXPAND_RPW = tuple(int(v) for v in knob('DPP_EXPAND_RPW', '128,64,32').split(','))
EXPAND_MAX_WGS = int(knob('DPP_EXPAND_MAX_WGS', '256'))


def expand_plan(M, N, K, forward):
    if not (EXPAND & (1 if forward else 2)) or K not in (16, 32, 64) or N % 64 or N < 2 * K:
        return None
    rpw = EXPAND_RPW[0 if M >= 65536 else (1 if M >= 16384 else 2)]
    while rpw > 32 and M % rpw:
        rpw //= 2
    while EXPAND_MAX_WGS and (M // rpw) * (N // 64) // 4 > EXPAND_MAX_WGS and M % (2 * rpw) == 0:
        rpw *= 2
    if M % rpw:
        return None
    return (rpw, 64, 4)


C3_BM128_32 = knob('DPP_C3_BM128_32', '1') != '0'


C3_P64 = knob('DPP_C3_P64', '1') != '0'


def conv3x3_bm(pixels, Co, hw=None, prec=0):
    if Co == 64 and C3_P64 and prec and hw in ((8, 8), (16, 16)) and pixels % 128 == 0:
        return 128
    if Co == 32 and C3_BM128_32 and pixels % 128 == 0 and pixels // 128 >= 256:
        return 128
    return 128 if (pixels // 128) * (-(-Co // 64)) >= 512 else 64


SIDE_SHORTCUT = knob('DPP_SIDE_SHORTCUT', '1') != '0'


CONV3_STREAM_C = tuple(int(v) for v in knob('DPP_CONV3_STREAM_C', '').split(',') if v)


WGRAD_TARGET_BLOCKS = int(knob('DPP_WGRAD_TARGET_BLOCKS', '256'))


def wgrad_plan(Co, Ci, K):
    if Co <= 16:
        tile = (16, 64, 1)
    elif Co <= 32:
        tile = (32, 64, 1)
    else:
        tile = (64, 64 if Ci > 32 else (32 if Ci > 16 else 16), 4)
    tiles = (-(-Co // tile[0])) * (-(-Ci // tile[1]))
    splitk = int(max(1, min(WGRAD_TARGET_BLOCKS // tiles, max(K // 128, min(128, K // 64)))))
    return tile, splitk


WGRAD_STREAM = knob('DPP_WGRAD_STREAM', '1') != '0'
WGRAD_STREAM_RPW = tuple(int(v) for v in knob('DPP_WGRAD_STREAM_RPW', '256,128,128').split(','))
WGRAD_STREAM_STAGES = knob('DPP_WGRAD_STREAM_STAGES', '1')


WGRAD3_STREAM_C = tuple(int(v) for v in knob('DPP_WGRAD3_STREAM_C', '64').split(',') if v)


WGRAD3_STREAM_SLICE_BUDGET = int(knob('DPP_WGRAD3_STREAM_SLICES', '1024'))


def wgrad3_stream_rows(M, C):
    if C not in WGRAD3_STREAM_C:
        return 0
    slices = max(1, WGRAD3_STREAM_SLICE_BUDGET // max(1, (C // 16) ** 2))
    return max(64, (M // slices) & ~3)


def wgrad_stream_rows(M):
    stage = 0 if M >= 65536 else (1 if M >= 16384 else 2)
    if str(stage + 1) not in WGRAD_STREAM_STAGES:
        return 0
    r = WGRAD_STREAM_RPW[min(stage, len(WGRAD_STREAM_RPW) - 1)]
    return r if M >= 1024 else 32
```

deep-prior-pp_amd/hipdp/lib.py:

```python
import ctypes as C
import os

_HERE = os.path.dirname(os.path.abspath(__file__))
DEFAULT_LIB = os.path.join(os.path.dirname(_HERE), 'lib', 'libdpp_hip.so')

ABI_VERSION = 13
ST_A, ST_B, ST_C, ST_BNX = 1, 2, 4, 8
c_float_p = C.c_void_p
stream_t = C.c_void_p


class RowMap(C.Structure):
    _fields_ = [('s', C.c_int), ('Wo', C.c_int), ('HoWo', C.c_int), ('Wi', C.c_int), ('HiWi', C.c_int)]

    @staticmethod
    def identity():
        return RowMap(1, 0, 0, 0, 0)

    @staticmethod
    def strided(s, Ho, Wo, Hi, Wi):
        return RowMap(s, Wo, Ho * Wo, Wi, Hi * Wi)


class Act(C.Structure):
    _fields_ = [('mean', C.c_void_p), ('scale', C.c_void_p), ('beta', C.c_void_p), ('mode', C.c_int), ('cmod', C.c_int),
                ('x2', C.c_void_p), ('aux', C.c_void_p), ('out', C.c_void_p)]

    NONE, RELU, BN, BN_RELU, BN_BWD = 0, 1, 2, 3, 4

    @staticmethod
    def none():
        return Act(None, None, None, 0, 1, None, None, None)


class Epilogue(C.Structure):
    _fields_ = [('stats', C.c_void_p), ('bn_x', C.c_void_p), ('bn_mean', C.c_void_p), ('bn_inv_std', C.c_void_p),
                ('bn_scale', C.c_void_p), ('bn_beta', C.c_void_p), ('bn_relu', C.c_int), ('pad_', C.c_int),
                ('bn_partial', C.c_void_p)]


class GemmDesc(C.Structure):
    _fields_ = [('A', C.c_void_p), ('lda', C.c_int), ('a_kc', C.c_int), ('mapA', RowMap), ('actA', Act),
                ('B', C.c_void_p), ('ldb', C.c_int), ('b_kc', C.c_int), ('mapB', RowMap), ('actB', Act),
                ('C', C.c_void_p), ('ldc', C.c_int), ('mapC', RowMap),
                ('bias', C.c_void_p), ('residual', C.c_void_p),
                ('M', C.c_int), ('N', C.c_int), ('K', C.c_int),
                ('splitk', C.c_int), ('partial', C.c_void_p),
                ('bm', C.c_int), ('bn', C.c_int), ('wm', C.c_int), ('variant', C.c_int), ('epi', Epilogue), ('store', C.c_int), ('precision', C.c_int)]


class BnEval(C.Structure):
    _fields_ = [('mean', C.c_void_p), ('inv_std', C.c_void_p), ('gamma', C.c_void_p), ('beta', C.c_void_p)]


class ResblockDesc(C.Structure):
    _fields_ = [('X', C.c_void_p), ('N', C.c_int), ('H', C.c_int), ('W', C.c_int), ('Cin', C.c_int),
                ('stride', C.c_int), ('Ho', C.c_int), ('Wo', C.c_int), ('Cout', C.c_int), ('Nb', C.c_int),
                ('bn0', BnEval), ('bn1', BnEval), ('bn2', BnEval),
                ('W1', C.c_void_p), ('b1', C.c_void_p), ('W2', C.c_void_p), ('b2', C.c_void_p), ('W3', C.c_void_p), ('b3', C.c_void_p),
                ('Wsc', C.c_void_p), ('bsc', C.c_void_p), ('Y', C.c_void_p), ('store', C.c_int)]


SIGNATURES = {
    'dpp_abi_version': (C.c_int, []),
    'dpp_gemm': (C.c_int, [C.POINTER(GemmDesc), stream_t]),
    'dpp_gemm_variant_rows': (C.c_int, [C.POINTER(GemmDesc)]),
    'dpp_fc_gemm': (C.c_int, [C.POINTER(GemmDesc), C.c_int, C.c_int, stream_t]),
    'dpp_reduce_partials': (C.c_int, [C.c_void_p, C.c_int, C.c_int, C.c_void_p, C.c_int, C.c_void_p, stream_t]),
    'dpp_conv3x3': (C.c_int, [C.c_void_p, C.c_int, C.c_int, C.c_int, C.c_int, C.POINTER(Act), C.c_void_p, C.c_int,
                              C.c_void_p, C.c_void_p, C.c_void_p, C.c_int, C.POINTER(Epilogue), C.c_int, stream_t]),
    'dpp_conv3x3_bf16': (C.c_int, [C.c_void_p, C.c_int, C.c_int, C.c_int, C.c_int, C.POINTER(Act), C.c_void_p, C.c_int,
                                   C.c_void_p, C.c_void_p, C.c_void_p, C.c_int, C.POINTER(Epilogue), C.c_int, stream_t]),
    'dpp_conv3x3_tiling': (C.c_int, [C.c_int, C.c_int, C.c_int, C.c_int, C.POINTER(C.c_int), C.POINTER(C.c_int), C.POINTER(C.c_int)]),
    'dpp_conv3x3_stream_rows': (C.c_int, [C.c_int, C.c_int, C.c_int, C.c_int]),
    'dpp_conv3x3_stream': (C.c_int, [C.c_void_p, C.c_int, C.c_int, C.c_int, C.c_int, C.POINTER(Act), C.c_void_p, C.c_void_p, C.c_void_p,
                                     C.POINTER(Epilogue), stream_t]),
    'dpp_conv3x3_wtrans': (C.c_int, [C.c_void_p, C.c_int, C.c_int, C.c_void_p, stream_t]),
    'dpp_conv3x3_wgrad_blocks': (C.c_int, [C.c_int, C.c_int, C.c_int, C.c_int, C.c_int, C.c_int]),
    'dpp_conv3x3_wgrad': (C.c_int, [C.c_void_p, C.c_int, C.c_int, C.c_int, C.c_int, C.POINTER(Act), C.c_void_p, C.c_int,
                                    C.c_void_p, C.c_int, C.c_int, stream_t]),
    'dpp_conv3x3_wgrad_bf16': (C.c_int, [C.c_void_p, C.c_int, C.c_int, C.c_int, C.c_int, C.POINTER(Act), C.c_void_p, C.c_int,
                                    C.c_void_p, C.c_int, C.c_int, stream_t]),
    'dpp_conv3x3_wgrad_bf16_ok': (C.c_int, [C.c_int, C.c_int, C.c_int, C.c_int, C.c_int]),
    'dpp_stem_fwd': (C.c_int, [C.c_void_p, C.c_int, C.c_int, C.c_int, C.c_void_p, C.c_void_p, C.c_int, C.c_void_p,
                               C.c_void_p, C.c_void_p, C.c_int, stream_t]),
    'dpp_stem_wgrad_blocks': (C.c_int, [C.c_int, C.c_int, C.c_int, C.c_int]),
    'dpp_stem_wgrad': (C.c_int, [C.c_void_p, C.c_int, C.c_int, C.c_int, C.c_void_p, C.c_void_p, C.c_int, C.c_void_p,
                                 C.c_int, stream_t]),
    'dpp_convpool_fwd': (C.c_int, [C.c_void_p, C.c_int, C.c_int, C.c_int, C.c_int, C.c_void_p, C.c_void_p, C.c_int, C.c_int,
                                   C.c_int, C.c_int, C.c_int, C.c_void_p, C.c_void_p, C.c_void_p, stream_t]),
    'dpp_convpool_wgrad_blocks': (C.c_int, [C.c_int, C.c_int, C.c_int]),
    'dpp_convpool_wgrad': (C.c_int, [C.c_void_p, C.c_int, C.c_int, C.c_int, C.c_int, C.c_void_p, C.c_void_p, C.c_void_p, C.c_int,
                                     C.c_int, C.c_int, C.c_int, C.c_int, C.c_void_p, stream_t]),
    'dpp_convpool_dgrad': (C.c_int, [C.c_void_p, C.c_void_p, C.c_int, C.c_int, C.c_int, C.c_int, C.c_void_p, C.c_int, C.c_int,
                                     C.c_int, C.c_int, C.c_int, C.c_void_p, stream_t]),
    'dpp_bn_stats_partial': (C.c_int, [C.c_void_p, C.c_int, C.c_int, C.c_int, C.c_void_p, C.c_int, stream_t]),
    'dpp_bn_finalize': (C.c_int, [C.c_void_p, C.c_int, C.c_int, C.c_int, C.c_int, C.c_int, C.c_void_p, C.c_float, C.c_void_p,
                                  C.c_void_p, C.c_void_p, C.c_void_p, C.c_void_p, C.c_float, stream_t]),
    'dpp_bn_eval_coeffs': (C.c_int, [C.c_void_p, C.c_void_p, C.c_void_p, C.c_int, C.c_void_p, C.c_void_p, C.c_void_p,
                                     stream_t]),
    'dpp_bn_eval_job_bytes': (C.c_size_t, []),
    'dpp_bn_eval_coeffs_multi': (C.c_int, [C.c_void_p, C.c_int, C.c_int, stream_t]),
    'dpp_resblock_eval_ok': (C.c_int, [C.c_int] * 5),
    'dpp_resblock_eval': (C.c_int, [C.POINTER(ResblockDesc), stream_t]),
    'dpp_resblock_eval_check': (C.c_int, [C.POINTER(ResblockDesc)]),
    'dpp_bn_bwd_reduce': (C.c_int, [C.c_void_p, C.c_void_p, C.c_int, C.c_int, C.c_void_p, C.c_void_p, C.c_void_p,
                                    C.c_void_p, C.c_int, C.c_void_p, C.c_int, C.c_void_p, C.c_int, stream_t]),
    'dpp_bn_bwd_finalize': (C.c_int, [C.c_void_p, C.c_int, C.c_int, C.c_int, C.c_int, C.c_void_p, C.c_void_p, C.c_void_p,
                                      C.c_void_p, C.c_void_p, C.c_void_p, C.c_void_p, C.c_void_p, stream_t]),
    'dpp_bn_bwd_finalize_apply_ok': (C.c_int, [C.c_int, C.c_int, C.c_int]),
    'dpp_bn_bwd_finalize_apply': (C.c_int, [C.c_void_p, C.c_void_p, C.c_int, C.c_int, C.c_void_p, C.c_void_p, C.c_void_p, C.c_void_p, C.c_int,
                                            C.c_void_p, C.c_void_p, C.c_int, C.c_void_p, C.c_void_p, C.c_void_p, C.c_int, stream_t]),
    'dpp_bn_bwd_apply': (C.c_int, [C.c_void_p, C.c_void_p, C.c_int, C.c_int, C.c_void_p, C.c_void_p, C.c_void_p,
                                   C.c_void_p, C.c_void_p, C.c_void_p, C.c_void_p, C.c_int, C.c_void_p, C.c_int, stream_t]),
    'dpp_reduce_job_bytes': (C.c_size_t, []),
    'dpp_reduce_multi_block_cols': (C.c_int, []),
    'dpp_reduce_multi': (C.c_int, [C.c_void_p, C.c_int, C.c_int, stream_t]),
    'dpp_colsum_partial': (C.c_int, [C.c_void_p, C.c_int, C.c_int, C.c_int, C.c_void_p, stream_t]),
    'dpp_wgrad_stream_slices': (C.c_int, [C.c_int, C.c_int, C.c_int, C.c_int]),
    'dpp_wgrad_stream': (C.c_int, [C.c_void_p, C.c_int, C.c_void_p, C.c_int, C.c_void_p, C.c_void_p, C.c_int, C.c_int, C.c_void_p, C.c_int, stream_t]),
    'dpp_fc_wgrad_stream_ok': (C.c_int, [C.c_int, C.c_int, C.c_int]),
    'dpp_fc_wgrad_stream': (C.c_int, [C.c_void_p, C.c_void_p, C.c_void_p, C.c_int, C.c_int, C.c_int, C.c_void_p, C.c_int, stream_t]),
    'dpp_wgrad_stream_bf16': (C.c_int, [C.c_void_p, C.c_int, C.c_void_p, C.c_int, C.c_void_p, C.c_void_p, C.c_int, C.c_int, C.c_void_p, C.c_int, stream_t]),
    'dpp_wgrad_stream_bf16_ok': (C.c_int, [C.c_int, C.c_int]),
    'dpp_wgrad3_stream_slices': (C.c_int, [C.c_int] * 6),
    'dpp_wgrad3_stream': (C.c_int, [C.c_void_p, C.c_int, C.c_void_p, C.c_int, C.c_int, C.c_int, C.c_int, C.c_void_p, C.c_int, C.c_void_p, C.c_int, stream_t]),
    'dpp_wtrans_job_bytes': (C.c_size_t, []),
    'dpp_conv3x3_wtrans_multi': (C.c_int, [C.c_void_p, C.c_int, C.c_int, stream_t]),
    'dpp_loss_sse': (C.c_int, [C.c_void_p, C.c_void_p, C.c_int, C.c_int, C.c_int, C.c_void_p, C.c_void_p, stream_t]),
    'dpp_reduce_partials_loss': (C.c_int, [C.c_void_p, C.c_int, C.c_int, C.c_int, C.c_void_p, C.c_void_p, C.c_void_p, C.c_int, C.c_void_p, C.c_void_p, stream_t]),
    'dpp_loss_sse_bcast': (C.c_int, [C.c_void_p, C.c_void_p, C.c_int, C.c_void_p, C.c_void_p, C.c_void_p, stream_t]),
    'dpp_error_l2': (C.c_int, [C.c_void_p, C.c_void_p, C.c_int, C.c_int, C.c_void_p, stream_t]),
    'dpp_adam': (C.c_int, [C.c_void_p, C.c_void_p, C.c_void_p, C.c_void_p, C.c_size_t, C.c_void_p, stream_t]),
    'dpp_adam_ticked': (C.c_int, [C.c_void_p, C.c_void_p, C.c_void_p, C.c_void_p, C.c_size_t, C.c_void_p, stream_t]),
    'dpp_adam_tick': (C.c_int, [C.c_void_p, stream_t]),
    'dpp_counter_add': (C.c_int, [C.c_void_p, C.c_ulonglong, stream_t]),
    'dpp_axpy': (C.c_int, [C.c_void_p, C.c_void_p, C.c_float, C.c_size_t, stream_t]),
    'dpp_sumsq': (C.c_int, [C.c_void_p, C.c_size_t, C.c_float, C.c_void_p, C.c_int, stream_t]),
    'dpp_sumsq_multi_workspace_bytes': (C.c_size_t, []),
    'dpp_sumsq_multi': (C.c_int, [C.c_void_p, C.c_void_p, C.c_int, C.c_float, C.c_void_p, C.c_void_p, C.c_int, stream_t]),
    'dpp_axpy_multi': (C.c_int, [C.c_void_p, C.c_void_p, C.c_void_p, C.c_int, C.c_float, stream_t]),
    'dpp_scale': (C.c_int, [C.c_void_p, C.c_void_p, C.c_float, C.c_int, C.c_void_p, C.c_size_t, stream_t]),
    'dpp_relu_bwd': (C.c_int, [C.c_void_p, C.c_void_p, C.c_void_p, C.c_float, C.c_void_p, C.c_size_t, stream_t]),
    'dpp_fill_zero': (C.c_int, [C.c_void_p, C.c_size_t, stream_t]),
    'dpp_copy2d': (C.c_int, [C.c_void_p, C.c_int, C.c_void_p, C.c_int, C.c_int, C.c_int, C.c_int, stream_t]),
    'dpp_rowscale': (C.c_int, [C.c_void_p, C.c_void_p, C.c_int, C.c_int, C.c_float, C.c_void_p, C.c_int, C.c_int, stream_t]),
    'dpp_crop_center': (C.c_int, [C.c_void_p, C.c_int, C.c_int, C.c_int, C.c_void_p, C.c_int, C.c_int, stream_t]),
    'dpp_bernoulli_mask': (C.c_int, [C.c_void_p, C.c_size_t, C.c_float, C.c_ulonglong, C.c_ulonglong, C.c_void_p, stream_t]),
    'dpp_augment_record_bytes': (C.c_size_t, []),
    'dpp_augment_prepare': (C.c_int, [C.c_void_p] * 5 + [C.c_int] * 3 + [C.c_void_p] * 5 + [C.c_int, C.c_ulonglong,
                                      C.c_ulonglong, C.c_double, C.c_double, C.c_double, C.c_double, C.c_double,
                                      C.c_double, C.c_double, C.c_int, C.c_int, C.c_void_p, C.c_void_p, C.c_int, C.c_void_p,
                                      C.c_void_p, C.c_void_p, C.c_void_p, stream_t]),
    'dpp_augment_warp': (C.c_int, [C.c_void_p, C.c_void_p, C.c_int, C.c_int, C.c_void_p, stream_t]),
    'dpp_augment': (C.c_int, [C.c_void_p] * 5 + [C.c_int] * 3 + [C.c_void_p] * 5 + [C.c_int, C.c_ulonglong,
                              C.c_ulonglong, C.c_double, C.c_double, C.c_double, C.c_double, C.c_double,
                              C.c_double, C.c_double, C.c_int, C.c_int, C.c_void_p, C.c_void_p, C.c_int, C.c_void_p,
                              C.c_void_p, C.c_void_p, C.c_void_p, C.c_void_p, C.c_void_p, C.c_ulonglong, C.c_ulonglong, C.c_int,
                              stream_t]),
    'dpp_crop_record_bytes': (C.c_size_t, []),
    'dpp_crop_prepare': (C.c_int, [C.c_void_p, C.c_int, C.c_int, C.c_int, C.c_void_p, C.c_void_p, C.c_double, C.c_double, C.c_int, C.c_int,
                                   C.c_void_p, C.c_void_p, stream_t]),
    'dpp_crop_com_workspace_bytes': (C.c_size_t, [C.c_int]),
    'dpp_crop_com': (C.c_int, [C.c_void_p, C.c_void_p, C.c_int, C.c_int, C.c_int, C.c_void_p, C.c_void_p, stream_t]),
    'dpp_crop_warp': (C.c_int, [C.c_void_p, C.c_void_p, C.c_int, C.c_int, C.c_int, C.c_int, C.c_int, C.c_float, C.c_void_p, stream_t]),
    'dpp_crop_warp_ex': (C.c_int, [C.c_void_p, C.c_void_p, C.c_int, C.c_int, C.c_int, C.c_int, C.c_int, C.c_float, C.c_float, C.c_float,
                                   C.c_void_p, stream_t]),
    'dpp_resize_crops': (C.c_int, [C.c_void_p, C.c_int, C.c_int, C.c_int, C.c_int, C.c_int, C.c_int, C.c_float, C.c_void_p, stream_t]),
    'dpp_recrop': (C.c_int, [C.c_void_p, C.c_int, C.c_int, C.c_int, C.c_void_p, C.c_void_p, C.c_int, C.c_int, C.c_float, C.c_double, C.c_int,
                             C.c_void_p, C.c_void_p, stream_t]),
    'dpp_inverse_crop': (C.c_int, [C.c_void_p, C.c_int, C.c_int, C.c_int, C.c_void_p, C.c_void_p, C.c_int, C.c_int, C.c_int, C.c_float, C.c_float,
                                   C.c_int, C.c_void_p, stream_t]),
    'dpp_crop_refine': (C.c_int, [C.c_void_p, C.c_void_p, C.c_int, C.c_int, C.c_int, C.c_void_p, C.c_void_p, C.c_void_p, C.c_double, C.c_double,
                                  C.c_double, C.c_double, C.c_int, C.c_void_p, C.c_int, C.c_void_p, C.c_void_p, C.c_int, C.c_void_p, C.c_void_p,
                                  C.c_void_p, C.c_void_p, stream_t]),
    'dpp_frame_range_bytes': (C.c_size_t, [C.c_int]),
    'dpp_frame_range': (C.c_int, [C.c_void_p, C.c_int, C.c_int, C.c_int, C.c_void_p, stream_t]),
    'dpp_crop_prepare_ranged': (C.c_int, [C.c_void_p, C.c_int, C.c_void_p, C.c_void_p, C.c_double, C.c_double, C.c_int, C.c_int, C.c_void_p,
                                          C.c_void_p, stream_t]),
    'dpp_track_refine': (C.c_int, [C.c_void_p, C.c_void_p, C.c_int, C.c_int, C.c_int, C.c_void_p, C.c_void_p, C.c_void_p] + [C.c_double] * 4 +
                         [C.c_int, C.c_double, C.c_double, C.c_int] + [C.c_void_p] * 5 + [stream_t]),
    'dpp_pose_finish': (C.c_int, [C.c_void_p, C.c_int, C.c_int, C.c_void_p, C.c_void_p] + [C.c_double] * 4 + [C.c_int, C.c_int, C.c_void_p,
                                                                                                              C.c_void_p, stream_t]),
    'dpp_refine_com_iterative': (C.c_int, [C.c_void_p, C.c_void_p, C.c_int, C.c_int, C.c_int, C.c_void_p, C.c_void_p, C.c_double, C.c_double,
                                           C.c_int, C.c_void_p, C.c_void_p, stream_t]),
    'dpp_pose_sample': (C.c_int, [C.c_void_p, C.c_void_p, C.c_void_p, C.c_int, C.c_int, C.c_void_p, C.c_void_p, C.c_void_p, C.c_void_p,
                                  C.c_void_p, C.c_long, C.c_double, C.c_double, C.c_double, C.c_double, C.c_int, C.c_void_p, C.c_void_p,
                                  C.c_void_p, stream_t]),
    'dpp_pose_sample_rot3d': (C.c_int, [C.c_void_p, C.c_void_p, C.c_void_p, C.c_int, C.c_int, C.c_void_p, C.c_void_p, C.c_void_p, C.c_void_p,
                                        C.c_void_p, C.c_long, C.c_double, C.c_double, C.c_double, C.c_double, C.c_int, C.c_void_p, C.c_void_p,
                                        C.c_void_p, stream_t]),
    'dpp_pca_workspace_bytes': (C.c_size_t, [C.c_long, C.c_int]),
    'dpp_pca_fit': (C.c_int, [C.c_void_p, C.c_long, C.c_int, C.c_void_p, C.c_void_p, C.c_void_p, C.c_void_p, stream_t]),
    'dpp_pose_eval': (C.c_int, [C.c_void_p, C.c_void_p, C.c_int, C.c_int, C.c_void_p, C.c_int, C.c_void_p, C.c_void_p, C.c_void_p, stream_t]),
    'dpp_prof_set': (C.c_int, [C.c_void_p]),
    'dpp_plan_create': (C.c_int, [C.POINTER(C.c_void_p)]),
    'dpp_plan_destroy': (C.c_int, [C.c_void_p]),
    'dpp_plan_record_begin': (C.c_int, [C.c_void_p]),
    'dpp_plan_record_lane': (C.c_int, [C.c_void_p, C.c_int]),
    'dpp_plan_record_end': (C.c_int, [C.c_void_p]),
    'dpp_plan_fork': (C.c_int, [C.c_void_p]),
    'dpp_plan_join': (C.c_int, [C.c_void_p]),
    'dpp_plan_count': (C.c_int, [C.c_void_p, C.POINTER(C.c_int), C.POINTER(C.c_int), C.POINTER(C.c_int)]),
    'dpp_plan_run': (C.c_int, [C.c_void_p, stream_t, stream_t]),
    'dpp_plan_graph_build': (C.c_int, [C.c_void_p, C.c_int]),
    'dpp_plan_graph_launch': (C.c_int, [C.c_void_p, stream_t]),
}


class DppError(RuntimeError):
    pass


def check(status, what):
    if status != 0:
        raise DppError("%s failed with status %d" % (what, status))


_cache = {}

# ... 19 lines not shown
```

deep-prior-pp_amd/hipdp/ops.py:

```python
import ctypes as C
import os

import numpy as np

from .lib import ST_A, ST_B, ST_BNX, ST_C, Act, BnEval, DppError, Epilogue, GemmDesc, ResblockDesc, RowMap, check


class Launch(object):
    __slots__ = ('fn', 'args', 'keep', 'name', 'meta', 'kernels')

    def __init__(self, fn, args, keep, name, meta=None, kernels=1):
        self.fn, self.args, self.keep, self.name, self.meta = fn, args, keep, name, meta
        self.kernels = kernels

    def __call__(self, stream):
        st = self.fn(*self.args, stream)
        if st != 0:
            check(st, self.name)


class Fork(object):
    name = 'fork'
    meta = None

# ... 137 lines not shown
        return segs

    def segment_counts(self):
        native, host, open_ = 0, 0, False
        for op, _ in self.ops:
            if isinstance(op, (Launch, Fork, Join)):
                if not open_:
                    native, open_ = native + 1, True
            else:
                host, open_ = host + 1, False
        return native, host

    def run(self, rt_or_stream):
        rt = rt_or_stream if hasattr(rt_or_stream, 'stream') else None
        if rt is not None and LAUNCH_MODE != 'python':
            for seg in self._compile(rt):
                if isinstance(seg, NativePlan):
                    seg.run(rt)
                else:
                    seg(rt.stream)
            return
        if rt is None or not self.uses_side or not getattr(rt, 'has_side_stream', False):
            st = rt.stream if rt is not None else rt_or_stream
            for op, _ in self.ops:
                if not isinstance(op, (Fork, Join)):
                    op(st)
            return
        main, side = rt.stream, rt.side_stream
        for op, on_side in self.ops:
            if isinstance(op, Fork):
                rt.side_wait_main()
            elif isinstance(op, Join):
                rt.main_wait_side()
            else:
                op(side if on_side else main)

    def __len__(self):
        return len(self.launches())


def _p(buf):
    return None if buf is None else buf.ptr


BF16 = np.dtype(np.uint16)


def _is16(buf):
    return buf is not None and getattr(buf, 'dtype', None) == BF16


def _store(a=None, b=None, c=None, bnx=None):
    return (ST_A if _is16(a) else 0) | (ST_B if _is16(b) else 0) | (ST_C if _is16(c) else 0) | (ST_BNX if _is16(bnx) else 0)


def _esz(buf):
    return 2.0 if _is16(buf) else 4.0


def act(mode=0, mean=None, scale=None, beta=None, cmod=1, x2=None, aux=None, out=None):
    a = Act(_p(mean), _p(scale), _p(beta), int(mode), int(cmod), _p(x2), _p(aux), _p(out))
    a._keep = (mean, scale, beta, x2, aux, out)
    return a


def act_bn_bwd(bn, q, p, x, C, out=None):
    return act(Act.BN_BWD, mean=bn.mean, scale=bn.scale, beta=q, cmod=C, x2=x, aux=p, out=out)


def epilogue(stats=None, bn=None, bn_x=None, bn_relu=True, bn_partial=None):
    e = Epilogue()
    e.stats = _p(stats)
    if bn is not None:
        e.bn_x, e.bn_mean, e.bn_inv_std, e.bn_scale, e.bn_beta = bn_x.ptr, bn.mean.ptr, bn.inv_std.ptr, bn.scale.ptr, bn.beta_buf.ptr
        e.bn_relu, e.bn_partial = int(bn_relu), bn_partial.ptr
    e._bn_x = bn_x
    e._keep = (stats, bn, bn_x, bn_partial)
    return e


def gemm(rt, A, B, Cbuf, M, N, K, a_kc, b_kc, lda, ldb, ldc=0, mapA=None, mapB=None, mapC=None, actA=None, actB=None,
         bias=None, residual=None, splitk=1, partial=None, tile=(0, 0, 0), epi=None, variant=0, name='gemm', precision=0):
    d = GemmDesc()
    d.A, d.lda, d.a_kc = A.ptr, lda, int(a_kc)
    d.mapA = mapA or RowMap.identity()
    d.actA = actA or Act.none()
    d.B, d.ldb, d.b_kc = B.ptr, ldb, int(b_kc)
    d.mapB = mapB or RowMap.identity()
    d.actB = actB or Act.none()
    d.C, d.ldc = _p(Cbuf), ldc
    d.mapC = mapC or RowMap.identity()
    d.bias, d.residual = _p(bias), _p(residual)
    d.M, d.N, d.K = int(M), int(N), int(K)
    d.splitk, d.partial = int(splitk), _p(partial)
    d.bm, d.bn, d.wm = tile
    d.variant = int(variant)
    if epi is not None:
        d.epi = epi
    if _is16(residual) != _is16(Cbuf) and residual is not None and Cbuf is not None:
        raise ValueError("dpp_gemm: C and residual must be stored alike")
    d.store = _store(A, B, Cbuf, getattr(epi, '_bn_x', None) if epi is not None else None)
    d.precision = int(precision)
    meta = dict(kernel='gemm_mfma_bf16' if precision else 'gemm_mfma_f32', flops=2.0 * M * N * K,
                bytes=_esz(A) * M * K + _esz(B) * K * N + (4.0 * M * N * max(1, splitk) if splitk > 1 else _esz(Cbuf) * M * N) +
                (_esz(residual) * M * N if residual is not None else 0))
    return Launch(rt.lib.dpp_gemm, (C.byref(d),), (d, A, B, Cbuf, bias, residual, partial, actA, actB, epi), name, meta)


def gemm_variant_rows(rt, launch):
    return int(rt.lib.dpp_gemm_variant_rows(C.byref(launch.keep[0])))


def wgrad_stream(rt, dY, Co, X, Ci, M, rows_per_wave, partial, mapX=None, actX=None, name='wgrad_stream', precision=0):
    nsl = rt.lib.dpp_wgrad_stream_slices(Co, Ci, M, rows_per_wave)
    meta = dict(kernel='gemm_mfma_bf16' if precision else 'gemm_mfma_f32', flops=2.0 * M * Co * Ci,
                bytes=_esz(dY) * M * Co + 4.0 * nsl * Co * Ci + _esz(X) * M * Ci)
    return Launch(rt.lib.dpp_wgrad_stream_bf16 if precision else rt.lib.dpp_wgrad_stream, (dY.ptr, int(Co), X.ptr, int(Ci), C.byref(mapX) if mapX is not None else None, _actp(actX), int(M),
                                            int(rows_per_wave), partial.ptr, _store(a=dY, b=X)), (dY, X, partial, mapX, actX), name, meta)


def wgrad3_stream(rt, dY, Co, X, Ci, N, H, W, rows_per_wave, partial, actX=None, name='conv3x3_wgrad_stream'):
    nsl = rt.lib.dpp_wgrad3_stream_slices(Co, Ci, N, H, W, rows_per_wave)
    px = float(N) * H * W
    meta = dict(kernel='conv3x3_wgrad_mfma_f32', flops=2.0 * px * 9 * Ci * Co, bytes=4.0 * (px * Co + nsl * 9.0 * Ci * Co) + _esz(X) * px * Ci)
    return Launch(rt.lib.dpp_wgrad3_stream, (dY.ptr, int(Co), X.ptr, int(Ci), int(N), int(H), int(W), _actp(actX), int(rows_per_wave),
                                             partial.ptr, _store(a=dY, b=X)), (dY, X, partial, actX), name, meta)


def fc_gemm(rt, A, B, Cbuf, M, N, K, a_kc, b_kc, lda, ldb, ldc=0, actA=None, actB=None, bias=None, residual=None, splitk=1, partial=None,
            precision=0, kchunk=0, name='fc_gemm'):
    d = GemmDesc()
    d.A, d.lda, d.a_kc = A.ptr, lda, int(a_kc)
    d.mapA, d.mapB, d.mapC = RowMap.identity(), RowMap.identity(), RowMap.identity()
    d.actA = actA or Act.none()
    d.B, d.ldb, d.b_kc = B.ptr, ldb, int(b_kc)
    d.actB = actB or Act.none()
    d.C, d.ldc = _p(Cbuf), ldc
    d.bias, d.residual = _p(bias), _p(residual)
    d.M, d.N, d.K = int(M), int(N), int(K)
    d.splitk, d.partial = int(splitk), _p(partial)
    d.store = _store(A, B, Cbuf)
    if _is16(residual) != _is16(Cbuf) and residual is not None and Cbuf is not None:
        raise ValueError("dpp_fc_gemm: C and residual must be stored alike")
    meta = dict(kernel='fc_gemm_mfma_bf16' if precision else 'gemm_mfma_f32', flops=2.0 * M * N * K,
                bytes=4.0 * (M * K + K * N + M * N * (max(1, splitk) if splitk > 1 else 1) + (M * N if residual is not None else 0)))
    return Launch(rt.lib.dpp_fc_gemm, (C.byref(d), int(precision), int(kchunk)), (d, A, B, Cbuf, bias, residual, partial, actA, actB), name, meta)


def fc_wgrad_stream(rt, X, dY, dW, Nb, K, N, actX=None, name='fc_wgrad_stream'):
    meta = dict(kernel='gemm_mfma_f32', flops=2.0 * Nb * K * N, bytes=4.0 * (Nb * K + Nb * N + K * N))
    return Launch(rt.lib.dpp_fc_wgrad_stream, (X.ptr, dY.ptr, dW.ptr, int(Nb), int(K), int(N), _actp(actX), _store(b=X)), (X, dY, dW, actX), name, meta)


def reduce_partials(rt, partial, nz, n, out, bias=None, nbias=1, name='reduce_partials'):
    return Launch(rt.lib.dpp_reduce_partials, (partial.ptr, int(nz), int(n), _p(bias), int(nbias), out.ptr),
                  (partial, out, bias), name, dict(kernel='reduce_partials', flops=float(nz) * n, bytes=4.0 * (nz + 1) * n))


def _actp(a):
    return C.byref(a) if a is not None else None


def conv3x3(rt, X, N, H, W, Ci, Wk, Co, Y, actX=None, bias=None, residual=None, bm=0, epi=None, name='conv3x3', precision=0):
    px = float(N) * H * W
    meta = dict(kernel='conv3x3_mfma_bf16' if precision else 'conv3x3_mfma_f32', flops=2.0 * px * 9 * Ci * Co,
                bytes=px * (_esz(X) * Ci + _esz(Y) * Co + (_esz(residual) * Co if residual is not None else 0)) + 4.0 * 9 * Ci * Co)
    if residual is not None and _is16(residual) != _is16(Y):
        raise ValueError("dpp_conv3x3: Y and residual must be stored alike")
    st = _store(X, None, Y, getattr(epi, '_bn_x', None) if epi is not None else None)
    return Launch(rt.lib.dpp_conv3x3_bf16 if precision else rt.lib.dpp_conv3x3, (X.ptr, N, H, W, Ci, _actp(actX), Wk.ptr, Co, _p(bias), _p(residual), Y.ptr, bm,
                                       C.byref(epi) if epi is not None else None, st),
                  (X, Wk, Y, actX, bias, residual, epi), name, meta)


def conv3x3_stream(rt, X, N, H, W, Cc, Wk, Y, actX=None, bias=None, epi=None, name='conv3x3'):
    _f32_only('dpp_conv3x3_stream', X, Y, getattr(epi, '_bn_x', None) if epi is not None else None)
    px = float(N) * H * W
    meta = dict(kernel='conv3x3_mfma_f32', flops=2.0 * px * 9 * Cc * Cc, bytes=px * 8.0 * Cc + 4.0 * 9 * Cc * Cc)
    return Launch(rt.lib.dpp_conv3x3_stream, (X.ptr, N, H, W, Cc, _actp(actX), Wk.ptr, _p(bias), Y.ptr, C.byref(epi) if epi is not None else None),
                  (X, Wk, Y, actX, bias, epi), name, meta)


def conv3x3_wtrans(rt, Wk, Co, Ci, Wd, name='conv3x3_wtrans'):
    return Launch(rt.lib.dpp_conv3x3_wtrans, (Wk.ptr, Co, Ci, Wd.ptr), (Wk, Wd), name)


def conv3x3_wtrans_multi(rt, jobs, name='conv3x3_wtrans'):
    import struct
    assert rt.lib.dpp_wtrans_job_bytes() == 32
    raw, block0 = b'', 0
    for (Wk, Co, Ci, Wd) in jobs:
        raw += struct.pack('<QQiiii', Wk.ptr, Wd.ptr, int(Co), int(Ci), block0, 0)
        block0 += -(-(Co * 9 * Ci) // 256)
    table = rt.upload(np.frombuffer(raw, np.uint8).copy())
    return Launch(rt.lib.dpp_conv3x3_wtrans_multi, (table.ptr, len(jobs), block0), (table, list(jobs)), name)


def conv3x3_wgrad(rt, X, N, H, W, Ci, dY, Co, partial, actX=None, bm=64, name='conv3x3_wgrad', precision=0):
    px = float(N) * H * W
    nblk = rt.lib.dpp_conv3x3_wgrad_blocks(N, H, W, Ci, Co, bm)
    meta = dict(kernel='conv3x3_wgrad_mfma_bf16' if precision else 'conv3x3_wgrad_mfma_f32', flops=2.0 * px * 9 * Ci * Co,
                bytes=_esz(dY) * px * Co + 4.0 * nblk * 9.0 * Ci * Co + _esz(X) * px * Ci)
    fn = rt.lib.dpp_conv3x3_wgrad_bf16 if precision else rt.lib.dpp_conv3x3_wgrad
    return Launch(fn, (X.ptr, N, H, W, Ci, _actp(actX), dY.ptr, Co, partial.ptr, bm, _store(a=X, b=dY)),
                  (X, dY, partial, actX), name, meta)


def stem_fwd(rt, X, N, H, W, Wk, bias, Co, Y, argmax, stats=None, name='stem_fwd'):
    px = float(N) * H * W
    return Launch(rt.lib.dpp_stem_fwd, (X.ptr, N, H, W, Wk.ptr, bias.ptr, Co, Y.ptr, _p(argmax), _p(stats), _store(c=Y)), (X, Wk, bias, Y, argmax, stats), name,
                  dict(kernel='stem_fwd_mfma_f32', flops=2.0 * px * 25 * Co, bytes=4.0 * px + px / 4 * Co * (1.0 + _esz(Y))))


def stem_wgrad(rt, X, N, H, W, dY, argmax, Co, partial, tiles_per_block, name='stem_wgrad'):
    px = float(N) * H * W
    return Launch(rt.lib.dpp_stem_wgrad, (X.ptr, N, H, W, dY.ptr, argmax.ptr, Co, partial.ptr, tiles_per_block),
                  (X, dY, argmax, partial), name, dict(kernel='stem_wgrad', flops=2.0 * px / 4 * Co * 25, bytes=4.0 * px + px / 4 * Co * 5.0))


def convpool_fwd(rt, X, N, H, W, Ci, Wk, kh, kw, pad, Co, pool, bias, Y, ties=None, actX=None, name='convpool_fwd'):
    px = float(N) * (H + 2 * pad - kh + 1) * (W + 2 * pad - kw + 1)
    return Launch(rt.lib.dpp_convpool_fwd, (X.ptr, N, H, W, Ci, _actp(actX), Wk.ptr, kh, kw, pad, Co, pool, bias.ptr, Y.ptr, _p(ties)),
                  (X, Wk, bias, Y, ties, actX), name,
                  dict(kernel='convpool_fwd', flops=2.0 * px * kh * kw * Ci * Co, bytes=4.0 * N * H * W * Ci + 6.0 * px / (pool * pool) * Co))


def convpool_wgrad(rt, X, N, H, W, Ci, dY, ties, kh, kw, pad, Co, pool, partial, actX=None, name='convpool_wgrad'):
    px = float(N) * (H + 2 * pad - kh + 1) * (W + 2 * pad - kw + 1) / (pool * pool)
    return Launch(rt.lib.dpp_convpool_wgrad, (X.ptr, N, H, W, Ci, _actp(actX), dY.ptr, _p(ties), kh, kw, pad, Co, pool, partial.ptr),
                  (X, dY, ties, partial, actX), name,
                  dict(kernel='convpool_wgrad', flops=2.0 * px * kh * kw * Ci * Co, bytes=4.0 * N * H * W * Ci + 6.0 * px * Co))


def convpool_dgrad(rt, dY, ties, N, H, W, Ci, Wk, kh, kw, pad, Co, pool, dX, name='convpool_dgrad'):
    px = float(N) * (H + 2 * pad - kh + 1) * (W + 2 * pad - kw + 1) / (pool * pool)
    return Launch(rt.lib.dpp_convpool_dgrad, (dY.ptr, _p(ties), N, H, W, Ci, Wk.ptr, kh, kw, pad, Co, pool, dX.ptr), (dY, ties, Wk, dX), name,
                  dict(kernel='convpool_dgrad', flops=2.0 * px * kh * kw * Ci * Co, bytes=4.0 * N * H * W * Ci + 6.0 * px * Co))


def bn_stats_partial(rt, X, M, Cc, rpb, partial, name='bn_stats_partial'):
    return Launch(rt.lib.dpp_bn_stats_partial, (X.ptr, M, Cc, rpb, partial.ptr, _store(a=X)), (X, partial), name,
                  dict(kernel='bn_stats_partial', flops=3.0 * M * Cc, bytes=_esz(X) * M * Cc))


def bn_finalize(rt, partial, nb, M, rpb, Cc, gamma, eps, mean, inv_std, scale, run_mean=None, run_inv_std=None, alpha=0.0,
                nseg=1, name='bn_finalize'):
    return Launch(rt.lib.dpp_bn_finalize, (partial.ptr, nb, int(nseg), M, rpb, Cc, gamma.ptr, float(eps), mean.ptr, inv_std.ptr, scale.ptr,
                                           _p(run_mean), _p(run_inv_std), float(alpha)),
                  (partial, gamma, mean, inv_std, scale, run_mean, run_inv_std), name,
                  dict(kernel='bn_finalize', flops=0.0, bytes=8.0 * nb * Cc))


def bn_eval_coeffs(rt, gamma, run_mean, run_inv_std, Cc, mean, inv_std, scale, name='bn_eval_coeffs'):
    return Launch(rt.lib.dpp_bn_eval_coeffs, (gamma.ptr, run_mean.ptr, run_inv_std.ptr, Cc, mean.ptr, inv_std.ptr, scale.ptr),
                  (gamma, run_mean, run_inv_std, mean, inv_std, scale), name)


def bn_eval_coeffs_multi(rt, jobs, name='bn_eval_coeffs'):
    import struct
    assert rt.lib.dpp_bn_eval_job_bytes() == 56
    raw, block0 = b'', 0
    for (gamma, rm, ris, Cc, mean, inv_std, scale) in jobs:
        raw += struct.pack('<QQQQQQii', gamma.ptr, rm.ptr, ris.ptr, mean.ptr, inv_std.ptr, scale.ptr, int(Cc), block0)
        block0 += -(-int(Cc) // 256)
    table = rt.upload(np.frombuffer(raw, np.uint8).copy())
    return Launch(rt.lib.dpp_bn_eval_coeffs_multi, (table.ptr, len(jobs), block0), (table, list(jobs)), name,
                  dict(kernel='bn_eval_coeffs', flops=0.0, bytes=24.0 * sum(int(j[3]) for j in jobs)))


def bn_eval(mean, inv_std, gamma, beta):
    b = BnEval(mean.ptr, inv_std.ptr, gamma.ptr, beta.ptr)
    b._keep = (mean, inv_std, gamma, beta)
    return b


def resblock_eval(rt, X, N, H, W, Cin, stride, Cout, Nb, bn0, bn1, bn2, W1, b1, W2, b2, W3, b3, Y, Wsc=None, bsc=None, name='resblock_eval'):
    d = ResblockDesc()
    d.store = _store(a=X, c=Y)
    Ho, Wo = -(-H // stride), -(-W // stride)
    d.X, d.N, d.H, d.W, d.Cin = X.ptr, int(N), int(H), int(W), int(Cin)
    d.stride, d.Ho, d.Wo, d.Cout, d.Nb = int(stride), Ho, Wo, int(Cout), int(Nb)
    d.bn0, d.bn1, d.bn2 = bn0, bn1, bn2
    d.W1, d.b1, d.W2, d.b2, d.W3, d.b3 = W1.ptr, b1.ptr, W2.ptr, b2.ptr, W3.ptr, b3.ptr
    d.Wsc, d.bsc, d.Y = _p(Wsc), _p(bsc), Y.ptr
    px = float(N) * Ho * Wo
    flops = 2.0 * px * (Cin * Nb + 9.0 * Nb * Nb + Nb * Cout + (Cin * Cout if Wsc is not None else 0))
    byts = _esz(X) * (float(N) * H * W * Cin + (px * Cout if Wsc is None else 0)) + _esz(Y) * px * Cout + 4.0 * (Cin * Nb + 9.0 * Nb * Nb + Nb * Cout)
    return Launch(rt.lib.dpp_resblock_eval, (C.byref(d),), (d, X, Y, bn0, bn1, bn2, W1, b1, W2, b2, W3, b3, Wsc, bsc), name,
                  dict(kernel='resblock_eval_mfma_f32', flops=flops, bytes=byts))


def bn_bwd_reduce(rt, dA, X, M, Cc, mean, inv_std, scale, beta, relu, G, rpb, partial, name='bn_bwd_reduce'):
    return Launch(rt.lib.dpp_bn_bwd_reduce, (dA.ptr, X.ptr, M, Cc, mean.ptr, inv_std.ptr, scale.ptr, beta.ptr, int(relu), G.ptr, rpb,
                                             partial.ptr, _store(a=dA, c=G, bnx=X)), (dA, X, mean, inv_std, scale, beta, G, partial), name,
                  dict(kernel='bn_bwd_reduce', flops=8.0 * M * Cc, bytes=(8.0 + _esz(X)) * M * Cc))


def bn_bwd_finalize(rt, partial, nb, M, Cc, dbeta, dgamma, c1, c2, nseg=1, bn=None, q=None, p=None, name='bn_bwd_finalize'):
    return Launch(rt.lib.dpp_bn_bwd_finalize, (partial.ptr, nb, int(nseg), M, Cc, dbeta.ptr, dgamma.ptr, c1.ptr, c2.ptr,
                                               _p(bn.inv_std) if q is not None else None, _p(bn.scale) if q is not None else None,
                                               _p(q), _p(p)),
                  (partial, dbeta, dgamma, c1, c2, bn, q, p), name, dict(kernel='bn_bwd_finalize', flops=0.0, bytes=8.0 * nb * Cc))


def bn_bwd_apply(rt, G, X, M, Cc, mean, inv_std, scale, c1, c2, dX, add=None, rpb=None, colsum=None, name='bn_bwd_apply'):
    rpb = rpb or max(32, -(-M // 1024))
# ... 290 lines not shown
```

include/dpp_hip.h:

```cpp
#ifndef DPP_HIP_H
#define DPP_HIP_H

#include <stddef.h>
#include <stdint.h>

#ifdef __cplusplus
extern "C" {
#endif

typedef void* dpp_stream_t;

#define DPP_OK 0
#define DPP_E_BADARG 10001
#define DPP_E_UNSUPPORTED 10002

#define DPP_ABI_VERSION 13
int dpp_abi_version(void);

#define DPP_ST_A 1
#define DPP_ST_B 2
#define DPP_ST_C 4
#define DPP_ST_BNX 8

typedef struct {
    int s, Wo, HoWo, Wi, HiWi;
} dpp_rowmap;

typedef struct {
    const float* mean;
    const float* scale;
    const float* beta;
    int mode;
    int cmod;
    const float* x2;
    const float* aux;
    float* out;
} dpp_act;

typedef struct {
    float* stats;
    const float* bn_x;
    const float* bn_mean;
    const float* bn_inv_std;
    const float* bn_scale;
    const float* bn_beta;
    int bn_relu;
    int pad_;
    float* bn_partial;
} dpp_epilogue;

typedef struct {
    const float* A; int lda; int a_kc; dpp_rowmap mapA; dpp_act actA;
    const float* B; int ldb; int b_kc; dpp_rowmap mapB; dpp_act actB;
    float* C; int ldc; dpp_rowmap mapC;
    const float* bias;
    const float* residual;
    int M, N, K;
    int splitk;
    float* partial;
    int bm, bn, wm;
    int variant;
    dpp_epilogue epi;
    int store;
    int precision;
} dpp_gemm_desc;
int dpp_gemm(const dpp_gemm_desc* d, dpp_stream_t stream);
int dpp_gemm_variant_rows(const dpp_gemm_desc* d);

int dpp_wgrad_stream_slices(int Co, int Ci, int M, int rows_per_wave);
int dpp_wgrad_stream(const float* dY, int Co, const float* X, int Ci, const dpp_rowmap* mapX, const dpp_act* actX, int M,
                     int rows_per_wave, float* partial, int store , dpp_stream_t stream);
int dpp_wgrad_stream_bf16_ok(int Co, int Ci);
int dpp_wgrad_stream_bf16(const float* dY, int Co, const float* X, int Ci, const dpp_rowmap* mapX, const dpp_act* actX, int M,
                     int rows_per_wave, float* partial, int store , dpp_stream_t stream);

int dpp_fc_wgrad_stream_ok(int Nb, int K, int N);
int dpp_fc_wgrad_stream(const float* X, const float* dY, float* dW, int Nb, int K, int N, const dpp_act* actX,
                        int store , dpp_stream_t stream);
int dpp_wgrad3_stream_slices(int Co, int Ci, int N, int H, int W, int rows_per_wave);
int dpp_wgrad3_stream(const float* dY, int Co, const float* X, int Ci, int N, int H, int W, const dpp_act* actX, int rows_per_wave,
                      float* partial, int store , dpp_stream_t stream);

int dpp_fc_gemm(const dpp_gemm_desc* d, int precision, int kchunk, dpp_stream_t stream);

int dpp_reduce_partials(const float* partial, int nz, int n, const float* bias, int nbias, float* out,
                        dpp_stream_t stream);


size_t dpp_reduce_job_bytes(void);
int dpp_reduce_multi_block_cols(void);
int dpp_reduce_multi(const void* jobs_dev, int njobs, int total_blocks, dpp_stream_t stream);

int dpp_conv3x3(const float* X, int N, int H, int W, int Ci, const dpp_act* act, const float* Wk, int Co,
                const float* bias, const float* residual, float* Y, int bm, const dpp_epilogue* epi,
                int store , dpp_stream_t stream);
int dpp_conv3x3_bf16(const float* X, int N, int H, int W, int Ci, const dpp_act* act, const float* Wk, int Co,
                     const float* bias, const float* residual, float* Y, int bm, const dpp_epilogue* epi, int store, dpp_stream_t stream);
int dpp_conv3x3_stream_rows(int N, int H, int W, int C);
int dpp_conv3x3_stream(const float* X, int N, int H, int W, int C, const dpp_act* act, const float* Wk, const float* bias, float* Y,
                       const dpp_epilogue* epi, dpp_stream_t stream);
int dpp_conv3x3_tiling(int N, int H, int W, int bm, int* th, int* tw, int* img);
int dpp_conv3x3_wtrans(const float* Wk, int Co, int Ci, float* Wd, dpp_stream_t stream);
size_t dpp_wtrans_job_bytes(void);
int dpp_conv3x3_wtrans_multi(const void* jobs_dev, int njobs, int total_blocks, dpp_stream_t stream);
int dpp_conv3x3_wgrad_blocks(int N, int H, int W, int Ci, int Co, int bm);
int dpp_conv3x3_wgrad(const float* X, int N, int H, int W, int Ci, const dpp_act* act, const float* dY, int Co,
                      float* partial, int bm, int store , dpp_stream_t stream);
int dpp_conv3x3_wgrad_bf16_ok(int N, int H, int W, int Ci, int Co);
int dpp_conv3x3_wgrad_bf16(const float* X, int N, int H, int W, int Ci, const dpp_act* act, const float* dY, int Co,
                           float* partial, int bm, int store , dpp_stream_t stream);

int dpp_stem_fwd(const float* X, int N, int H, int W, const float* Wk, const float* bias, int Co, float* Y, uint8_t* argmax,
                 float* stats, int store , dpp_stream_t stream);
int dpp_stem_wgrad_blocks(int N, int H, int W, int tiles_per_block);
int dpp_stem_wgrad(const float* X, int N, int H, int W, const float* dY, const uint8_t* argmax, int Co, float* partial,
                   int tiles_per_block, dpp_stream_t stream);

int dpp_convpool_fwd(const float* X, int N, int H, int W, int Ci, const dpp_act* act, const float* Wk, int kh, int kw, int pad,
                     int Co, int pool, const float* bias, float* Y, uint16_t* ties, dpp_stream_t stream);
int dpp_convpool_wgrad_blocks(int N, int Hp, int Wp);
int dpp_convpool_wgrad(const float* X, int N, int H, int W, int Ci, const dpp_act* act, const float* dY, const uint16_t* ties,
                       int kh, int kw, int pad, int Co, int pool, float* partial, dpp_stream_t stream);
int dpp_convpool_dgrad(const float* dY, const uint16_t* ties, int N, int H, int W, int Ci, const float* Wk, int kh, int kw,
                       int pad, int Co, int pool, float* dX, dpp_stream_t stream);

int dpp_bn_stats_partial(const float* X, int M, int C, int rows_per_block, float* partial, int store ,
                         dpp_stream_t stream);
int dpp_bn_finalize(const float* partial, int nb, int nseg, int M, int rows_per_block, int C, const float* gamma, float eps,
                    float* mean, float* inv_std, float* scale, float* run_mean, float* run_inv_std, float alpha,
                    dpp_stream_t stream);
int dpp_bn_eval_coeffs(const float* gamma, const float* run_mean, const float* run_inv_std, int C, float* mean,
                       float* inv_std, float* scale, dpp_stream_t stream);
size_t dpp_bn_eval_job_bytes(void);
int dpp_bn_eval_coeffs_multi(const void* jobs, int njobs, int total_blocks, dpp_stream_t stream);
int dpp_bn_bwd_reduce(const float* dA, const float* X, int M, int C, const float* mean, const float* inv_std,
                      const float* scale, const float* beta, int relu, float* G, int rows_per_block, float* partial,
                      int store , dpp_stream_t stream);
int dpp_bn_bwd_finalize(const float* partial, int nb, int nseg, int M, int C, float* dbeta, float* dgamma, float* c1, float* c2,
                        const float* inv_std, const float* scale, float* q, float* p, dpp_stream_t stream);
int dpp_bn_bwd_apply(const float* G, const float* X, int M, int C, const float* mean, const float* inv_std,
                     const float* scale, const float* c1, const float* c2, const float* add, float* dX,
                     int rows_per_block, float* colsum_partial ,
                     int store , dpp_stream_t stream);
int dpp_bn_bwd_finalize_apply_ok(int M, int C, int nb);
int dpp_bn_bwd_finalize_apply(const float* G, const float* X, int M, int C, const float* mean, const float* inv_std,
                              const float* scale, const float* partial, int nb, const float* add, float* dX, int rows_per_block,
                              float* colsum_partial, float* dbeta, float* dgamma, int store, dpp_stream_t stream);

int dpp_colsum_partial(const float* X, int M, int C, int rows_per_block, float* partial, dpp_stream_t stream);
int dpp_loss_sse(const float* out, const float* y, int rows, int d, int denom, float* cost, float* dout, dpp_stream_t stream);
int dpp_reduce_partials_loss(const float* partial, int nz, int rows, int d, const float* bias, float* out, const float* y, int denom,
                             float* cost, float* dout, dpp_stream_t stream);
int dpp_loss_sse_bcast(const float* out, const float* y, int n, float* cost, float* dout, float* err, dpp_stream_t stream);
int dpp_error_l2(const float* out, const float* y, int rows, int d, float* err, dpp_stream_t stream);
int dpp_adam(float* w, const float* g, float* m, float* v, size_t n, const float* state, dpp_stream_t stream);
int dpp_adam_ticked(float* w, const float* g, float* m, float* v, size_t n, float* hyper, dpp_stream_t stream);
int dpp_adam_tick(float* state, dpp_stream_t stream);
int dpp_axpy(float* y, const float* x, float alpha, size_t n, dpp_stream_t stream);
int dpp_sumsq(const float* x, size_t n, float alpha, float* out, int accumulate, dpp_stream_t stream);
size_t dpp_sumsq_multi_workspace_bytes(void);
int dpp_sumsq_multi(const float* base, const long long* seg, int nseg, float alpha, void* workspace, float* out, int accumulate,
                    dpp_stream_t stream);
int dpp_axpy_multi(float* ybase, const float* xbase, const long long* seg, int nseg, float alpha, dpp_stream_t stream);
int dpp_scale(const float* x, const float* mask, float a, int relu, float* y, size_t n, dpp_stream_t stream);
int dpp_relu_bwd(const float* dy, const float* pre, const float* mask, float a, float* g, size_t n, dpp_stream_t stream);

int dpp_fill_zero(void* p, size_t nbytes, dpp_stream_t stream);
int dpp_copy2d(const float* src, int lds, float* dst, int ldd, int rows, int cols, int relu, dpp_stream_t stream);
int dpp_rowscale(const float* x, const float* s, int sld, int scol, float factor, float* out, int rows, int cols, dpp_stream_t stream);
int dpp_crop_center(const float* src, int B, int H, int W, float* dst, int h, int w, dpp_stream_t stream);
int dpp_bernoulli_mask(float* mask, size_t n, float keep, unsigned long long seed, unsigned long long counter,
                       const unsigned long long* counter_dev, dpp_stream_t stream);

size_t dpp_augment_record_bytes(void);
int dpp_augment_prepare(const float* img, const float* com3d, const float* cube, const float* Mcrop, const float* gt3d,
                        int B, int J, int dsz, const int* mode, const double* off, const double* rot, const double* sc,
                        const int* mode_table, int n_modes, unsigned long long seed, unsigned long long counter,
                        double sigma_com, double sigma_sc, double rot_range, double fx, double fy, double ux, double uy,
                        int flip_y, int norm_zero_one, const float* pca_mean, const float* pca_comp, int E, void* records, float* out_y,
                        int* out_mode, const unsigned long long* counter_dev, dpp_stream_t stream);
int dpp_counter_add(unsigned long long* counter, unsigned long long inc, dpp_stream_t stream);
int dpp_augment_warp(const float* img, const void* records, int B, int dsz, float* out, dpp_stream_t stream);
int dpp_augment(const float* img, const float* com3d, const float* cube, const float* Mcrop, const float* gt3d,
                int B, int J, int dsz, const int* mode, const double* off, const double* rot, const double* sc,
                const int* mode_table, int n_modes, unsigned long long seed, unsigned long long counter,
                double sigma_com, double sigma_sc, double rot_range, double fx, double fy, double ux, double uy,
                int flip_y, int norm_zero_one, const float* pca_mean, const float* pca_comp, int E, void* records,
                float* out_x, float* out_y, int* out_mode, unsigned long long* counter_dev, unsigned* ticket,
                unsigned long long sample0, unsigned long long global_batch, int splits, dpp_stream_t stream);

size_t dpp_crop_record_bytes(void);
int dpp_crop_prepare(const float* frames, int B, int H, int W, const float* com, const float* cube, double fx, double fy,
                     int dsz, int stretch, void* records, float* M_out, dpp_stream_t stream);
int dpp_crop_warp(const float* frames, const void* records, int B, int H, int W, int dsz, int normalize, float nd_value,
                  float* out, dpp_stream_t stream);
size_t dpp_crop_com_workspace_bytes(int B);
int dpp_crop_com(const float* frames, const void* records, int B, int H, int W, void* workspace, float* com_out, dpp_stream_t stream);
int dpp_crop_refine(const float* frames, const void* records, int B, int H, int W, const float* com_in, const float* cube,
                    const float* net_out, double fx, double fy, double ux, double uy, int flip_y, const float* gt3d_orig, int J,
                    const float* pca_mean, const float* pca_comp, int E, float* com_out, float* com3d_out, float* gt3d_crop,
                    float* out_y, dpp_stream_t stream);

int dpp_crop_warp_ex(const float* frames, const void* records, int B, int H, int W, int dsz, int flags, float nd_value, float fill_value,
                     float pad_value, float* out, dpp_stream_t stream);
int dpp_resize_crops(const float* src, int B, int sh, int sw, int dh, int dw, int bilinear, float nd_value, float* out, dpp_stream_t stream);
int dpp_recrop(const float* crops, int B, int h, int w, const double* M, const double* Mnew, int th, int tw, float background,
               double nv_val, int thresh_z, const float* zrange, float* out, dpp_stream_t stream);
int dpp_inverse_crop(const float* crops, int B, int ch, int cw, const int* bounds, const float* zrange, int H, int W, int bilinear,
                     float nd_value, float background, int thresh_z, float* out, dpp_stream_t stream);

#define DPP_CROP_FLIP_X 16
size_t dpp_frame_range_bytes(int B);
int dpp_frame_range(const float* frames, int B, int H, int W, float* partial, dpp_stream_t stream);
int dpp_crop_prepare_ranged(const float* partial, int B, const float* com, const float* cube, double fx, double fy, int dsz, int stretch,
                            void* records, float* M_out, dpp_stream_t stream);
int dpp_track_refine(const float* frames, const void* records_in, int B, int H, int W, const float* com_in, const float* cube,
                     const float* net_out, double fx, double fy, double ux, double uy, int flip_y, double crop_fx, double crop_fy, int dsz,
                     float* com_out, float* com3d_out, void* records_out, float* M_out, int* status, dpp_stream_t stream);
int dpp_pose_finish(const float* net_out, int B, int J, const float* cube, const float* com3d, double fx, double fy, double ux, double uy,
                    int flip_y, int flags, float* pose3d, float* pose_img, dpp_stream_t stream);
int dpp_refine_com_iterative(const float* frames, const float* partial, int B, int H, int W, const float* com_in, const float* cube,
                             double fx, double fy, int num_iter, float* com_out, int* status, dpp_stream_t stream);

int dpp_pose_sample(const float* base_poses, const float* base_com, const float* base_cube, int n_base, int J, const int* mode,
                    const int* ridx, const double* off, const double* sc, const double* rot, long n, double fx, double fy,
                    double ux, double uy, int flip_y, float* out_poses, float* out_com, float* out_cube, dpp_stream_t stream);
int dpp_pose_sample_rot3d(const float* base_poses, const float* base_com, const float* base_cube, int n_base, int J, const int* mode,
                          const int* ridx, const double* off, const double* sc, const double* rot3, long n, double fx, double fy,
                          double ux, double uy, int flip_y, float* out_poses, float* out_com, float* out_cube, dpp_stream_t stream);
size_t dpp_pca_workspace_bytes(long N, int D);
int dpp_pca_fit(const float* X, long N, int D, void* workspace, double* mean, double* evals, double* components, dpp_stream_t stream);
int dpp_pose_eval(const float* gt, const float* pred, int N, int J, const double* thresholds, int T, double* err, double* frame,
                  double* out, dpp_stream_t stream);

typedef struct {
    const float* mean;
// ... 38 lines not shown
```

Baseline: 38040 depth-crops/sec.

## Fuse the last two FC layers into dedicated head forward and backward kernels

Adds fc_head forward and backward kernels that compute fc2 (with ReLU and bias) and the final projection fc3 in one launch. Per-slice partial outputs are then reduced, with the reduction loop now batching loads 16 at a time. The backward kernel fuses the dout·W3 product with the ReLU mask and the dW2-side gradient to the first hidden layer. This removes separate GEMM launches and intermediate round trips for the small head. It also adds an opt-in swizzled, unpadded LDS layout variant of the FC stream GEMM behind an environment flag. The head fusion is on by default and replaces a well-tuned GEMM path, so it risks lower MFMA efficiency on a part of the step that may be small.

Result: no change. 38270 depth-crops/sec (median of 6 runs) (+0.6%).

```diff
diff --git a/deep-prior-pp_amd/csrc/elementwise.hip b/deep-prior-pp_amd/csrc/elementwise.hip
--- a/deep-prior-pp_amd/csrc/elementwise.hip
+++ b/deep-prior-pp_amd/csrc/elementwise.hip
@@ -71,9 +71,12 @@
 #pragma unroll
             for (int z = 1; z < 16; ++z)
                 if (z < nzc) { t.x += v[z].x; t.y += v[z].y; t.z += v[z].z; t.w += v[z].w; }
-            for (int z = 16; z < nz; ++z) {
-                const float4 u = reinterpret_cast<const float4*>(partial + (size_t)z * n)[q];
-                t.x += u.x; t.y += u.y; t.z += u.z; t.w += u.w;
+            for (int zb = 16; zb < nz; zb += 16) {
+#pragma unroll
+                for (int z = 0; z < 16; ++z) v[z] = reinterpret_cast<const float4*>(partial + (size_t)(zb + z < nz ? zb + z : 0) * n)[q];
+#pragma unroll
+                for (int z = 0; z < 16; ++z)
+                    if (zb + z < nz) { t.x += v[z].x; t.y += v[z].y; t.z += v[z].z; t.w += v[z].w; }
             }
             t.x += bv.x; t.y += bv.y; t.z += bv.z; t.w += bv.w;
             reinterpret_cast<float4*>(out)[q] = t;
diff --git a/deep-prior-pp_amd/csrc/fcgemm.hip b/deep-prior-pp_amd/csrc/fcgemm.hip
--- a/deep-prior-pp_amd/csrc/fcgemm.hip
+++ b/deep-prior-pp_amd/csrc/fcgemm.hip
@@ -240,12 +240,13 @@
     int Kper;
 };
 
-template <int PREC, int BN, bool AKC, bool BKC>
+template <int PREC, int BN, bool AKC, bool BKC, bool SWZ = false>
 __global__ __launch_bounds__(DPP_THREADS) DPP_WAVES_PER_EU(1, 2) void fc_stream_kernel(FsArgs ga) {
     dpp_kernarg_warm<sizeof(FsArgs)>();
     const dpp_gemm_desc& d = ga.d;
     typedef typename Prec<PREC>::elem elem;
-    constexpr int BM = 128, KC = 32, LD = KC + Prec<PREC>::PAD, NST = 3, WM = 2, WN = 2;
+    static_assert(!SWZ || PREC == 0, "the swizzled image is the f32 one");
+    constexpr int BM = 128, KC = 32, LD = SWZ ? KC : KC + Prec<PREC>::PAD, NST = 3, WM = 2, WN = 2;
     constexpr int RM = BM / (16 * WM), CN = BN / (16 * WN);
     constexpr int SZA = BM * LD, SZB = BN * LD, SZ = SZA + SZB;
     HIP_DYNAMIC_SHARED(float4, smem4)
@@ -270,29 +271,32 @@
     const float* pa[SA];
     const float* pb[SB];
     int la, lb;
+    int la2 = 0, lb2 = 0;
     bool bvalid = true;
     if (AKC) {
         const int r = tid >> 3, quad = (tid & 7) * 4;
 #pragma unroll
         for (int s = 0; s < SA; ++s) pa[s] = d.A + (((size_t)(row0 + r + 32 * s) * d.lda + k_begin + quad) >> shA);
-        la = r * LD + quad;
+        la = r * LD + (SWZ ? (((tid & 7) ^ ((r >> 1) & 7)) * 4) : quad);
     } else {
         const int cq = tid % (BM / 4), kg = tid / (BM / 4);
 #pragma unroll
         for (int s = 0; s < SA; ++s) pa[s] = d.A + (((size_t)(k_begin + 4 * kg + s) * d.lda + row0 + 4 * cq) >> shA);
-        la = (4 * cq) * LD + 4 * kg;
+        la = (4 * cq) * LD + (SWZ ? ((kg ^ ((2 * cq) & 7)) * 4) : 4 * kg);
+        la2 = (4 * cq) * LD + (SWZ ? ((kg ^ ((2 * cq + 1) & 7)) * 4) : 4 * kg);
     }
     if (BKC) {
         const int r = tid >> 3, quad = (tid & 7) * 4;
 #pragma unroll
         for (int s = 0; s < SB; ++s) pb[s] = d.B + (size_t)(col0 + r + 32 * s) * d.ldb + k_begin + quad;
-        lb = r * LD + quad;
+        lb = r * LD + (SWZ ? (((tid & 7) ^ ((r >> 1) & 7)) * 4) : quad);
     } else {
         const int cq = tid % (BN / 4), kg = tid / (BN / 4);
         bvalid = kg < KC / 4;
 #pragma unroll
         for (int s = 0; s < SB; ++s) pb[s] = d.B + (size_t)(k_begin + 4 * (bvalid ? kg : 0) + s) * d.ldb + col0 + 4 * cq;
-        lb = (4 * cq) * LD + 4 * kg;
+        lb = (4 * cq) * LD + (SWZ ? (((kg & 7) ^ ((2 * cq) & 7)) * 4) : 4 * kg);
+        lb2 = (4 * cq) * LD + (SWZ ? (((kg & 7) ^ ((2 * cq + 1) & 7)) * 4) : 4 * kg);
     }
     const int modeA = d.actA.mode;
     float4 mu = make_float4(0.f, 0.f, 0.f, 0.f), sc = mu, be = mu;
@@ -352,8 +356,8 @@
             for (int s = 0; s < 4; ++s) { const float4 w = shA ? dpp_widen4(ra[s]) : ra[s]; v[s] = modeA ? act(w) : w; }
             put4(&As[la + 0 * LD], v[0].x, v[1].x, v[2].x, v[3].x);
             put4(&As[la + 1 * LD], v[0].y, v[1].y, v[2].y, v[3].y);
-            put4(&As[la + 2 * LD], v[0].z, v[1].z, v[2].z, v[3].z);
-            put4(&As[la + 3 * LD], v[0].w, v[1].w, v[2].w, v[3].w);
+            put4(&As[la2 + 2 * LD], v[0].z, v[1].z, v[2].z, v[3].z);
+            put4(&As[la2 + 3 * LD], v[0].w, v[1].w, v[2].w, v[3].w);
         }
         if constexpr (BKC) {
 #pragma unroll
@@ -364,8 +368,8 @@
         } else if (bvalid) {
             put4(&Bs[lb + 0 * LD], rb[0][0], rb[1][0], rb[2][0], rb[3][0]);
             put4(&Bs[lb + 1 * LD], rb[0][1], rb[1][1], rb[2][1], rb[3][1]);
-            put4(&Bs[lb + 2 * LD], rb[0][2], rb[1][2], rb[2][2], rb[3][2]);
-            put4(&Bs[lb + 3 * LD], rb[0][3], rb[1][3], rb[2][3], rb[3][3]);
+            put4(&Bs[lb2 + 2 * LD], rb[0][2], rb[1][2], rb[2][2], rb[3][2]);
+            put4(&Bs[lb2 + 3 * LD], rb[0][3], rb[1][3], rb[2][3], rb[3][3]);
         }
     };
 
@@ -383,7 +387,8 @@
     __syncthreads();
     int cur = 0;
     constexpr int EPT = Prec<PREC>::EPT;
-    const int aoff = (wm * (BM / WM) + l15) * LD + kq * EPT, boff = (wn * (BN / WN) + l15) * LD + kq * EPT;
+    const int aoff = (wm * (BM / WM) + l15) * LD + (SWZ ? 0 : kq * EPT), boff = (wn * (BN / WN) + l15) * LD + (SWZ ? 0 : kq * EPT);
+    const int swz = (l15 >> 1) & 7;
     for (int c = 0; c < nchunks; ++c) {
         const int nxt = cur == NST - 1 ? 0 : cur + 1;
         if (c + 1 < nchunks) commit(nxt);
@@ -394,10 +399,11 @@
 #pragma unroll
             for (int k0 = 0; k0 < KC; k0 += 16) {
                 float4 af[RM], bf[CN];
-#pragma unroll
-                for (int rt = 0; rt < RM; ++rt) af[rt] = *reinterpret_cast<const float4*>(&As[aoff + rt * 16 * LD + k0]);
-#pragma unroll
-                for (int ct = 0; ct < CN; ++ct) bf[ct] = *reinterpret_cast<const float4*>(&Bs[boff + ct * 16 * LD + k0]);
+                const int kc = SWZ ? ((((k0 >> 2) + kq) ^ swz) << 2) : k0;
+#pragma unroll
+                for (int rt = 0; rt < RM; ++rt) af[rt] = *reinterpret_cast<const float4*>(&As[aoff + rt * 16 * LD + kc]);
+#pragma unroll
+                for (int ct = 0; ct < CN; ++ct) bf[ct] = *reinterpret_cast<const float4*>(&Bs[boff + ct * 16 * LD + kc]);
 #pragma unroll
                 for (int t = 0; t < 4; ++t)
 #pragma unroll
@@ -434,23 +440,28 @@
     }
 }
 
-template <int PREC, int BN, bool AKC, bool BKC>
+template <int PREC, int BN, bool AKC, bool BKC, bool SWZ = false>
 int fs_launch(const FsArgs& ga, dim3 grid, hipStream_t st) {
-    constexpr size_t opb = 3 * (size_t)(128 + BN) * (32 + Prec<PREC>::PAD) * sizeof(typename Prec<PREC>::elem);
+    constexpr size_t opb = 3 * (size_t)(128 + BN) * (32 + (SWZ ? 0 : Prec<PREC>::PAD)) * sizeof(typename Prec<PREC>::elem);
     constexpr size_t epb = ((size_t)128 * (BN + 4) + 16 * BN) * 4;
     const size_t lds = opb > epb ? opb : epb;
-    (void)hipFuncSetAttribute(reinterpret_cast<const void*>(&fc_stream_kernel<PREC, BN, AKC, BKC>), hipFuncAttributeMaxDynamicSharedMemorySize, (int)lds);
-    DPP_LAUNCH((fc_stream_kernel<PREC, BN, AKC, BKC>), grid, dim3(DPP_THREADS), lds, st, ga);
+    (void)hipFuncSetAttribute(reinterpret_cast<const void*>(&fc_stream_kernel<PREC, BN, AKC, BKC, SWZ>), hipFuncAttributeMaxDynamicSharedMemorySize, (int)lds);
+    DPP_LAUNCH((fc_stream_kernel<PREC, BN, AKC, BKC, SWZ>), grid, dim3(DPP_THREADS), lds, st, ga);
     return dpp_launch_status();
 }
 
-template <int PREC, int BN>
+template <int PREC, int BN, bool SWZ = false>
 int fs_dispatch(const FsArgs& ga, dim3 grid, hipStream_t st) {
     const dpp_gemm_desc& d = ga.d;
-    if (d.a_kc && d.b_kc) return fs_launch<PREC, BN, true, true>(ga, grid, st);
-    if (d.a_kc && !d.b_kc) return fs_launch<PREC, BN, true, false>(ga, grid, st);
-    if (!d.a_kc && !d.b_kc) return fs_launch<PREC, BN, false, false>(ga, grid, st);
-    return fs_launch<PREC, BN, false, true>(ga, grid, st);
+    if (d.a_kc && d.b_kc) return fs_launch<PREC, BN, true, true, SWZ>(ga, grid, st);
+    if (d.a_kc && !d.b_kc) return fs_launch<PREC, BN, true, false, SWZ>(ga, grid, st);
+    if (!d.a_kc && !d.b_kc) return fs_launch<PREC, BN, false, false, SWZ>(ga, grid, st);
+    return fs_launch<PREC, BN, false, true, SWZ>(ga, grid, st);
+}
+
+bool fs_two_per_cu(const dpp_gemm_desc& d, int bn) {
+    const char* e = getenv("DPP_FC_STREAM_2WG");
+    return e && e[0] == '1' && bn == 128 && (long)(d.M / 128) * (d.N / 128) * d.splitk <= 256;
 }
 
 bool fs_accepts(const dpp_gemm_desc& d, int& bn) {
@@ -516,6 +527,7 @@
         fa.d = d;
         fa.Kper = d.K / d.splitk;
         dim3 g3(d.M / 128, d.N / bn3, d.splitk);
+        if (precision == 0 && fs_two_per_cu(d, bn3)) return fs_dispatch<0, 64, true>(fa, dim3(d.M / 128, d.N / 64, d.splitk), st);
         if (precision == 0) return bn3 == 128 ? fs_dispatch<0, 128>(fa, g3, st) : fs_dispatch<0, 64>(fa, g3, st);
         return bn3 == 128 ? fs_dispatch<1, 128>(fa, g3, st) : fs_dispatch<1, 64>(fa, g3, st);
     }
diff --git a/deep-prior-pp_amd/csrc/fchead.hip b/deep-prior-pp_amd/csrc/fchead.hip
--- /dev/null
+++ b/deep-prior-pp_amd/csrc/fchead.hip
@@ -0,0 +1,295 @@
+#include "dpp_common.h"
+
+namespace {
+
+constexpr int FH_BM = 16;
+constexpr int FH_BN = 32;
+constexpr int FH_PF = 8;
+constexpr int FH_N3MAX = 32;
+constexpr int FH_N2MAX = 2048;
+
+struct FhFwdArgs {
+    const float* h1;
+    const float* W2;
+    const float* b2;
+    const float* W3;
+    float* h2pre;
+    float* slices;
+    int M, K, N2, N3, relu_in;
+};
+
+struct FhBwdArgs {
+    const float* dout;
+    const float* W3;
+    const float* h2pre;
+    const float* W2;
+    const float* h1pre;
+    float* dh2pre;
+    float* dh1pre;
+    int M, K, N2, N3;
+};
+
+__host__ __device__ __forceinline__ int fh_min(int x, int y) { return x < y ? x : y; }
+
+__device__ __forceinline__ float fh_sum4(const float (*red)[FH_BM][FH_BN + 1], int r, int c) {
+    return ((red[0][r][c] + red[1][r][c]) + red[2][r][c]) + red[3][r][c];
+}
+
+__global__ __launch_bounds__(DPP_THREADS) DPP_WAVES_PER_EU(1, 2) void fc_head_fwd_kernel(FhFwdArgs a) {
+    dpp_kernarg_warm<sizeof(FhFwdArgs)>();
+    __shared__ float red[4][FH_BM][FH_BN + 1];
+    __shared__ float Hs[FH_BM][FH_BN + 1];
+    __shared__ float W3s[FH_BN][FH_N3MAX + 1];
+    const int tid = threadIdx.x, wave = tid >> 6, lane = tid & 63, l15 = lane & 15, kq = lane >> 4;
+    const int row0 = blockIdx.x * FH_BM, col0 = blockIdx.y * FH_BN;
+    const int M = a.M, K = a.K, N2 = a.N2, N3 = a.N3;
+    const int arow = fh_min(row0 + l15, M - 1);
+    const int bcol = col0 + 2 * l15;
+    const float* pa = a.h1 + (size_t)arow * K + kq * 4;
+    const float* pb = a.W2 + (size_t)(kq * 4) * N2 + (bcol < N2 ? bcol : 0);
+    const int ngroups = K / 16;
+    const int ng = (ngroups - wave + 3) / 4;
+    float4 ra[FH_PF];
+    float2 rb[FH_PF][4];
+    auto issue = [&](int s, int i) __attribute__((always_inline)) {
+        const int k0 = (wave + 4 * i) * 16;
+        ra[s] = *reinterpret_cast<const float4*>(pa + k0);
+#pragma unroll
+        for (int t = 0; t < 4; ++t) rb[s][t] = *reinterpret_cast<const float2*>(pb + (size_t)(k0 + t) * N2);
+    };
+#pragma unroll
+    for (int s = 0; s < FH_PF; ++s)
+        if (s < ng) issue(s, s);
+    float w3r[4];
+#pragma unroll
+    for (int s = 0; s < 4; ++s) {
+        const int e = tid + s * DPP_THREADS, c = e >> 5, j = e & 31;
+        w3r[s] = (col0 + c < N2 && j < N3) ? a.W3[(size_t)(col0 + c) * N3 + j] : 0.0f;
+    }
+    const int er = tid >> 4, ec = (tid & 15) * 2;
+    const bool eok = row0 + er < M && col0 + ec < N2;
+    float2 bias = make_float2(0.f, 0.f);
+    if (col0 + ec < N2) bias = *reinterpret_cast<const float2*>(a.b2 + col0 + ec);
+
+    f32x4 acc0 = {0.f, 0.f, 0.f, 0.f}, acc1 = {0.f, 0.f, 0.f, 0.f};
+    const bool relu = a.relu_in != 0;
+    for (int base = 0; base < ng; base += FH_PF) {
+#pragma unroll
+        for (int s = 0; s < FH_PF; ++s) {
+            if (base + s < ng) {
+                float av[4] = {ra[s].x, ra[s].y, ra[s].z, ra[s].w};
+                if (relu) {
+#pragma unroll
+                    for (int t = 0; t < 4; ++t) av[t] = fmaxf(av[t], 0.0f);
+                }
+#pragma unroll
+                for (int t = 0; t < 4; ++t) {
+                    acc0 = __builtin_amdgcn_mfma_f32_16x16x4f32(av[t], rb[s][t].x, acc0, 0, 0, 0);
+                    acc1 = __builtin_amdgcn_mfma_f32_16x16x4f32(av[t], rb[s][t].y, acc1, 0, 0, 0);
+                }
+                if (base + s + FH_PF < ng) issue(s, base + s + FH_PF);
+            }
+        }
+    }
+#pragma unroll
+    for (int r = 0; r < 4; ++r) {
+        red[wave][kq * 4 + r][2 * l15] = acc0[r];
+        red[wave][kq * 4 + r][2 * l15 + 1] = acc1[r];
+    }
+#pragma unroll
+    for (int s = 0; s < 4; ++s) {
+        const int e = tid + s * DPP_THREADS;
+        W3s[e >> 5][e & 31] = w3r[s];
+    }
+    __syncthreads();
+    {
+        const float v0 = fh_sum4(red, er, ec) + bias.x, v1 = fh_sum4(red, er, ec + 1) + bias.y;
+        if (eok) *reinterpret_cast<float2*>(a.h2pre + (size_t)(row0 + er) * N2 + col0 + ec) = make_float2(v0, v1);
+        Hs[er][ec] = eok ? fmaxf(v0, 0.0f) : 0.0f;
+        Hs[er][ec + 1] = eok ? fmaxf(v1, 0.0f) : 0.0f;
+    }
+    __syncthreads();
+    {
+        const int jj = tid & 15;
+        float s0 = 0.0f, s1 = 0.0f;
+#pragma unroll
+        for (int c = 0; c < FH_BN; ++c) {
+            const float h = Hs[er][c];
+            s0 = dpp_fma(h, W3s[c][jj], s0);
+            s1 = dpp_fma(h, W3s[c][jj + 16], s1);
+        }
+        if (row0 + er < M) {
+            float* out = a.slices + ((size_t)blockIdx.y * M + row0 + er) * N3;
+            if (jj < N3) out[jj] = s0;
+            if (jj + 16 < N3) out[jj + 16] = s1;
+        }
+    }
+}
+
+template <bool V2>
+__global__ __launch_bounds__(DPP_THREADS) DPP_WAVES_PER_EU(1, 2) void fc_head_bwd_kernel(FhBwdArgs a) {
+    dpp_kernarg_warm<sizeof(FhBwdArgs)>();
+    HIP_DYNAMIC_SHARED(float4, smem4)
+    const int tid = threadIdx.x, wave = tid >> 6, lane = tid & 63, l15 = lane & 15, kq = lane >> 4;
+    const int row0 = blockIdx.x * FH_BM, col0 = blockIdx.y * FH_BN;
+    const int M = a.M, K = a.K, N2 = a.N2, N3 = a.N3;
+    const int ngroups = (N2 + 15) / 16;
+    const int LD = ngroups * 16 + 4;
+    float* const As = reinterpret_cast<float*>(smem4);
+    float (*const red)[FH_BM][FH_BN + 1] = reinterpret_cast<float (*)[FH_BM][FH_BN + 1]>(As + FH_BM * LD);
+
+    const int per = (ngroups + 3) / 4;
+    const int g_begin = fh_min(wave * per, ngroups), g_end = fh_min(g_begin + per, ngroups);
+    const int ng2 = g_end - g_begin;
+    const float* pw[2];
+#pragma unroll
+    for (int ct = 0; ct < 2; ++ct) pw[ct] = a.W2 + (size_t)fh_min(col0 + ct * 16 + l15, K - 1) * N2;
+    f32x4 rw[FH_PF][2];
+    auto issue2 = [&](int s, int i) __attribute__((always_inline)) {
+        const int n = (g_begin + i) * 16 + kq * 4;
+        const int nn = n < N2 ? n : 0;
+#pragma unroll
+        for (int ct = 0; ct < 2; ++ct) rw[s][ct] = *reinterpret_cast<const f32x4*>(pw[ct] + nn);
+    };
+#pragma unroll
+    for (int s = 0; s < FH_PF; ++s)
+        if (s < ng2) issue2(s, s);
+    const int er = tid >> 4, ec = (tid & 15) * 2;
+    const bool eok = row0 + er < M && col0 + ec < K;
+    float2 h1 = make_float2(-1.f, -1.f);
+    if (eok) h1 = *reinterpret_cast<const float2*>(a.h1pre + (size_t)(row0 + er) * K + col0 + ec);
+
+    float da[2][4];
+    {
+        const float* pd = a.dout + (size_t)fh_min(row0 + l15, M - 1) * N3;
+#pragma unroll
+        for (int jh = 0; jh < 2; ++jh)
+#pragma unroll
+            for (int t = 0; t < 4; ++t) {
+                const int j = jh * 16 + kq * 4 + t;
+                da[jh][t] = j < N3 ? pd[j] : 0.0f;
+            }
+    }
+    const int nt1 = (ngroups - wave + 3) / 4;
+    float w3[FH_PF][2][4], hm[FH_PF][4];
+    auto issue1 = [&](int s, int i) __attribute__((always_inline)) {
+        const int n = (wave + 4 * i) * 16 + l15;
+        const int nc = fh_min(n, N2 - 1);
+        const float* p3 = a.W3 + (size_t)nc * N3;
+#pragma unroll
+        for (int jh = 0; jh < 2; ++jh) {
+            const int j = jh * 16 + kq * 4;
+            if (V2) {
+#pragma unroll
+                for (int h = 0; h < 2; ++h) {
+                    float2 v = make_float2(0.f, 0.f);
+                    if (j + 2 * h < N3) v = *reinterpret_cast<const float2*>(p3 + j + 2 * h);
+                    w3[s][jh][2 * h] = v.x;
+                    w3[s][jh][2 * h + 1] = v.y;
+                }
+            } else {
+#pragma unroll
+                for (int t = 0; t < 4; ++t) w3[s][jh][t] = j + t < N3 ? p3[j + t] : 0.0f;
+            }
+        }
+#pragma unroll
+        for (int r = 0; r < 4; ++r) hm[s][r] = a.h2pre[(size_t)fh_min(row0 + kq * 4 + r, M - 1) * N2 + nc];
+    };
+#pragma unroll
+    for (int s = 0; s < FH_PF; ++s)
+        if (s < nt1) issue1(s, s);
+    const bool writer = blockIdx.y == 0;
+    for (int base = 0; base < nt1; base += FH_PF) {
+#pragma unroll
+        for (int s = 0; s < FH_PF; ++s) {
+            if (base + s < nt1) {
+                f32x4 acc = {0.f, 0.f, 0.f, 0.f};
+#pragma unroll
+                for (int jh = 0; jh < 2; ++jh)
+#pragma unroll
+                    for (int t = 0; t < 4; ++t) acc = __builtin_amdgcn_mfma_f32_16x16x4f32(da[jh][t], w3[s][jh][t], acc, 0, 0, 0);
+                const int n = (wave + 4 * (base + s)) * 16 + l15;
+#pragma unroll
+                for (int r = 0; r < 4; ++r) {
+                    const float v = (n < N2 && hm[s][r] >= 0.0f) ? acc[r] : 0.0f;
+                    As[(kq * 4 + r) * LD + n] = v;
+                    if (writer && n < N2 && row0 + kq * 4 + r < M) a.dh2pre[(size_t)(row0 + kq * 4 + r) * N2 + n] = v;
+                }
+                if (base + s + FH_PF < nt1) issue1(s, base + s + FH_PF);
+            }
+        }
+    }
+    __syncthreads();
+
+    f32x4 acc2[2] = {{0.f, 0.f, 0.f, 0.f}, {0.f, 0.f, 0.f, 0.f}};
+    for (int base = 0; base < ng2; base += FH_PF) {
+#pragma unroll
+        for (int s = 0; s < FH_PF; ++s) {
+            if (base + s < ng2) {
+                const int n = (g_begin + base + s) * 16 + kq * 4;
+                const float4 av = *reinterpret_cast<const float4*>(&As[l15 * LD + n]);
+                const bool nin = n < N2;
+#pragma unroll
+                for (int t = 0; t < 4; ++t)
+#pragma unroll
+                    for (int ct = 0; ct < 2; ++ct)
+                        acc2[ct] = __builtin_amdgcn_mfma_f32_16x16x4f32(dpp_f4_get(av, t), nin ? rw[s][ct][t] : 0.0f, acc2[ct], 0, 0, 0);
+                if (base + s + FH_PF < ng2) issue2(s, base + s + FH_PF);
+            }
+        }
+    }
+#pragma unroll
+    for (int ct = 0; ct < 2; ++ct)
+#pragma unroll
+        for (int r = 0; r < 4; ++r) red[wave][kq * 4 + r][ct * 16 + l15] = acc2[ct][r];
+    __syncthreads();
+    if (eok) {
+        const float v0 = fh_sum4(red, er, ec), v1 = fh_sum4(red, er, ec + 1);
+        *reinterpret_cast<float2*>(a.dh1pre + (size_t)(row0 + er) * K + col0 + ec) = make_float2(h1.x >= 0.0f ? v0 : 0.0f, h1.y >= 0.0f ? v1 : 0.0f);
+    }
+}
+
+bool fh_dims_ok(int M, int K, int N2, int N3) {
+    return M >= 1 && K >= 16 && K % 16 == 0 && N2 >= 4 && N2 % 4 == 0 && N2 <= FH_N2MAX && N3 >= 1 && N3 <= FH_N3MAX;
+}
+
+bool fh_aligned(const void* p, int bytes) { return (reinterpret_cast<uintptr_t>(p) & (uintptr_t)(bytes - 1)) == 0; }
+
+}
+
+extern "C" int dpp_fc_head_ok(int M, int K, int N2, int N3) { return fh_dims_ok(M, K, N2, N3) ? 1 : 0; }
+
+extern "C" int dpp_fc_head_slices(int N2) { return N2 >= 1 ? dpp_cdiv(N2, FH_BN) : 0; }
+
+extern "C" int dpp_fc_head_fwd(const float* h1, int relu_in, const float* W2, const float* b2, const float* W3, float* h2pre, float* slices, int M,
+                               int K, int N2, int N3, dpp_stream_t stream) {
+    if (!h1 || !W2 || !b2 || !W3 || !h2pre || !slices) return DPP_E_BADARG;
+    if (!fh_dims_ok(M, K, N2, N3)) return DPP_E_UNSUPPORTED;
+    if (!fh_aligned(h1, 16) || !fh_aligned(W2, 8) || !fh_aligned(b2, 8) || !fh_aligned(h2pre, 8)) return DPP_E_UNSUPPORTED;
+    FhFwdArgs a = {h1, W2, b2, W3, h2pre, slices, M, K, N2, N3, relu_in};
+    DPP_LAUNCH(fc_head_fwd_kernel, dim3(dpp_cdiv(M, FH_BM), dpp_cdiv(N2, FH_BN)), dim3(DPP_THREADS), 0, static_cast<hipStream_t>(stream), a);
+    return dpp_launch_status();
+}
+
+extern "C" int dpp_fc_head_bwd(const float* dout, const float* W3, const float* h2pre, const float* W2, const float* h1pre, float* dh2pre,
+                               float* dh1pre, int M, int K, int N2, int N3, dpp_stream_t stream) {
+    if (!dout || !W3 || !h2pre || !W2 || !h1pre || !dh2pre || !dh1pre) return DPP_E_BADARG;
+    if (!fh_dims_ok(M, K, N2, N3)) return DPP_E_UNSUPPORTED;
+    const bool v2 = (N3 & 1) == 0;
+    if (!fh_aligned(W2, 16) || !fh_aligned(h1pre, 8) || !fh_aligned(dh1pre, 8) || (v2 && !fh_aligned(W3, 8))) return DPP_E_UNSUPPORTED;
+    FhBwdArgs a = {dout, W3, h2pre, W2, h1pre, dh2pre, dh1pre, M, K, N2, N3};
+    const int ld = dpp_cdiv(N2, 16) * 16 + 4;
+    const size_t lds = ((size_t)FH_BM * ld + 4 * FH_BM * (FH_BN + 1)) * sizeof(float);
+    const dim3 grid(dpp_cdiv(M, FH_BM), dpp_cdiv(K, FH_BN));
+    hipStream_t st = static_cast<hipStream_t>(stream);
+    if (v2) {
+        if (lds > 64 * 1024)
+            (void)hipFuncSetAttribute(reinterpret_cast<const void*>(&fc_head_bwd_kernel<true>), hipFuncAttributeMaxDynamicSharedMemorySize, (int)lds);
+        DPP_LAUNCH(fc_head_bwd_kernel<true>, grid, dim3(DPP_THREADS), lds, st, a);
+    } else {
+        if (lds > 64 * 1024)
+            (void)hipFuncSetAttribute(reinterpret_cast<const void*>(&fc_head_bwd_kernel<false>), hipFuncAttributeMaxDynamicSharedMemorySize, (int)lds);
+        DPP_LAUNCH(fc_head_bwd_kernel<false>, grid, dim3(DPP_THREADS), lds, st, a);
+    }
+    return dpp_launch_status();
+}
diff --git a/deep-prior-pp_amd/hipdp/backward.py b/deep-prior-pp_amd/hipdp/backward.py
--- a/deep-prior-pp_amd/hipdp/backward.py
+++ b/deep-prior-pp_amd/hipdp/backward.py
@@ -422,7 +422,18 @@
             off = (gW.ptr - st.g.ptr) // 4
             self._early_slice = (off, off + K * Nout)
             self.bwd.add(self.dp.allreduce_sum_async_op(gW, self._early_work, 'grad_allreduce_early'), side=True)
-        if src.base not in self.x_ins:
+        head = self.__dict__.get('_fc_head')
+        if head is not None and layer is head['fc3']:
+            fc2, t1, t2 = head['fc2'], head['t1'], head['t2']
+            _, K1, N2, N3 = head['dims']
+            dh2, dh1 = rt.alloc((Nb, N2), zero=False), rt.alloc((Nb, K1), zero=False)
+            self.bwd.add(ops.fc_head_bwd(rt, dY, st.view(layer.W), t2.buf, st.view(fc2.W), t1.buf, dh2, dh1, Nb, K1, N2, N3,
+                                         name='fc_head_bwd_%d' % layer.layerNum))
+            t2.pending.append(dh2)
+            t1.pending.append(dh1)
+        elif head is not None and layer is head['fc2']:
+            pass
+        elif src.base not in self.x_ins:
             tgt, dst = self._view_grad(src)
             acc = tgt.grad_written
             tile, splitk = hz.gemm_plan(Nb, K, Nout, allow_split=not acc)
diff --git a/deep-prior-pp_amd/hipdp/engine.py b/deep-prior-pp_amd/hipdp/engine.py
--- a/deep-prior-pp_amd/hipdp/engine.py
+++ b/deep-prior-pp_amd/hipdp/engine.py
@@ -61,6 +61,7 @@
         self._bn_eval_jobs = []
         self._beside = []
         self._bwd_after = {}
+        self._loss_kind = None if loss is None else loss.get('kind', 'embedding')
         out_view = self._emit(net.output)
         if self._bn_eval_jobs:
             self.fwd.ops[0:0] = [(ops.bn_eval_coeffs_multi(rt, self._bn_eval_jobs), False)]
@@ -385,7 +386,7 @@
         if kind == 'ConvLayer':
             return self._emit_conv(layer, src, residual, out_var if out_var is not None else var)
         if kind == 'HiddenLayer':
-            return self._emit_fc(layer, src)
+            return self._emit_fc(layer, src, var)
         if kind == 'DropoutLayer':
             return self._emit_dropout(layer, src)
         raise NotImplementedError(kind)
@@ -505,13 +506,71 @@
             return False
         return self.rt.lib.dpp_conv3x3_stream_rows(N, H, W, Ci) > 0
 
-    def _emit_fc(self, layer, src):
+    def _fc_head_match(self, layer, src, var):
+        if not (hz.FC_HEAD_FUSED and self.train and self.prec == 0 and not self.store16 and self._loss_kind in ('embedding', 'joints')):
+            return None
+        if var is None or var is not self.net.output or len(src.shape) != 2:
+            return None
+
+        def relu_of_hidden(v, consumer):
+            if v.kind != 'relu' or [id(c) for c in self.consumers.get(id(v), [])] != [id(consumer)]:
+                return None
+            w = v.inputs[0]
+            if w.kind != 'layer' or _layer_kind(w.layer) != 'HiddenLayer' or [id(c) for c in self.consumers.get(id(w), [])] != [id(v)]:
+                return None
+            return w
+        v2 = relu_of_hidden(var.inputs[0], var)
+        v1 = relu_of_hidden(v2.inputs[0], v2) if v2 is not None else None
+        if v1 is None:
+            return None
+        fc2, fc1 = v2.layer, v1.layer
+        io2, io1 = self.layer_io.get(id(fc2)), self.layer_io.get(id(fc1))
+        if io2 is None or io1 is None or io2.get('fwd_ops', (0, -1))[1] != len(self.fwd.ops):
+            return None
+        t1, t2, in2 = io1['out'], io2['out'], io2['in_view']
+        if src.base is not t2 or not src.relu or src.bn is not None or in2.base is not t1 or not in2.relu or in2.bn is not None:
+            return None
+        if t1.is16 or t2.is16 or t1 in self.x_ins:
+            return None
+        Nb, N2 = src.shape
+        K, N3 = in2.shape[1], layer.cfgParams.outputDim[1]
+        if self._fc1_stream(Nb, K, N2):
+            return None
+        st = self.store
+        bufs = (t1.buf, t2.buf, st.view(fc2.W), st.view(fc2.b), st.view(layer.W))
+        if not self.rt.lib.dpp_fc_head_ok(Nb, K, N2, N3) or any(b.ptr % 16 for b in bufs):
+            return None
+        return dict(fc2=fc2, fc3=layer, t1=t1, t2=t2, dims=(Nb, K, N2, N3))
+
+    def _emit_fc(self, layer, src, var=None):
         c = layer.cfgParams
         if len(src.shape) != 2:
             raise NotImplementedError("HiddenLayer on a non-flattened input")
         Nb, K = src.shape
         Nout = c.outputDim[1]
         assert K == c.inputDim[1], (K, c.inputDim)
+        rt, st = self.rt, self.store
+        head = self._fc_head_match(layer, src, var)
+        if head is not None:
+            fc2, t1, t2 = head['fc2'], head['t1'], head['t2']
+            _, K1, N2, N3 = head['dims']
+            del self.fwd.ops[self.layer_io[id(fc2)]['fwd_ops'][0]:]
+            out = self._new_tensor((Nb, Nout), 'fc%d' % layer.layerNum)
+            nsl = int(rt.lib.dpp_fc_head_slices(N2))
+            part = self.scratch(nsl * Nb * N3)
+            self.fwd.add(ops.fc_head_fwd(rt, t1.buf, True, st.view(fc2.W), st.view(fc2.b), st.view(layer.W), t2.buf, part, Nb, K1, N2, N3,
+                                         name='fc_head_fwd_%d' % layer.layerNum))
+            red = self.fwd.add(ops.reduce_partials(rt, part, nsl, Nb * N3, out.buf, bias=st.view(layer.b), nbias=N3))
+            self._loss_fusable = (red, dict(partial=part, nz=nsl, bias=st.view(layer.b), out=out.buf))
+            self._fc_head = head
+            self.layer_io[id(layer)] = dict(in_view=src, out=out)
+            return View(out)
+        first_op = len(self.fwd.ops)
+        out = self._emit_fc_plain(layer, src, Nb, K, Nout)
+        self.layer_io[id(layer)]['fwd_ops'] = (first_op, len(self.fwd.ops))
+        return View(out)
+
+    def _emit_fc_plain(self, layer, src, Nb, K, Nout):
         out = self._new_tensor((Nb, Nout), 'fc%d' % layer.layerNum)
         rt, st = self.rt, self.store
         act = self._act(src)
@@ -522,7 +581,7 @@
                                      partial=part, precision=self.prec, kchunk=hz.FC1_KCHUNK, name='fc_%d' % layer.layerNum))
             self.fwd.add(ops.reduce_partials(rt, part, splitk, Nb * Nout, out.buf, bias=st.view(layer.b), nbias=Nout))
             self.layer_io[id(layer)] = dict(in_view=src, out=out)
-            return View(out)
+            return out
         tile, splitk = hz.gemm_plan(Nb, Nout, K)
         if K >= 4096 and Nb <= 128 and Nout >= 64:
             tile, splitk = ((128, 64, 4) if Nb > 64 and hz.knob('DPP_FC1_TILE128', '1') != '0' else (64, 64, 4)), max(1, K // 512)
@@ -537,7 +596,7 @@
             self.fwd.add(ops.gemm(rt, src.base.buf, st.view(layer.W), out.buf, Nb, Nout, K, 1, 0, K, Nout, Nout, actA=act,
                                   bias=st.view(layer.b), tile=tile, name='fc_%d' % layer.layerNum))
         self.layer_io[id(layer)] = dict(in_view=src, out=out)
-        return View(out)
+        return out
 
     def _emit_dropout(self, layer, src):
         if src.bn is not None or len(src.shape) != 2:
diff --git a/deep-prior-pp_amd/hipdp/heuristics.py b/deep-prior-pp_amd/hipdp/heuristics.py
--- a/deep-prior-pp_amd/hipdp/heuristics.py
+++ b/deep-prior-pp_amd/hipdp/heuristics.py
@@ -42,6 +42,7 @@
 FUSE_LOSS = knob('DPP_FUSE_LOSS', '1') != '0'
 ADAM_TICKED = knob('DPP_ADAM_TICKED', '1') != '0'
 EVAL_FUSE_BF16 = knob('DPP_EVAL_FUSE_BF16', '1') != '0'
+FC_HEAD_FUSED = knob('DPP_FC_HEAD_FUSED', '1') != '0'
 OVERLAP_ALLREDUCE = knob('DPP_OVERLAP_ALLREDUCE', '1') != '0'
 EARLY_BUCKET_MIN = int(knob('DPP_EARLY_BUCKET_MIN', str(1 << 22)))
 LAZY_BN_BWD = int(knob('DPP_LAZY_BN_BWD', '0'))
diff --git a/deep-prior-pp_amd/hipdp/lib.py b/deep-prior-pp_amd/hipdp/lib.py
--- a/deep-prior-pp_amd/hipdp/lib.py
+++ b/deep-prior-pp_amd/hipdp/lib.py
@@ -4,7 +4,7 @@
 _HERE = os.path.dirname(os.path.abspath(__file__))
 DEFAULT_LIB = os.path.join(os.path.dirname(_HERE), 'lib', 'libdpp_hip.so')
 
-ABI_VERSION = 13
+ABI_VERSION = 14
 ST_A, ST_B, ST_C, ST_BNX = 1, 2, 4, 8
 c_float_p = C.c_void_p
 stream_t = C.c_void_p
@@ -66,6 +66,11 @@
     'dpp_gemm': (C.c_int, [C.POINTER(GemmDesc), stream_t]),
     'dpp_gemm_variant_rows': (C.c_int, [C.POINTER(GemmDesc)]),
     'dpp_fc_gemm': (C.c_int, [C.POINTER(GemmDesc), C.c_int, C.c_int, stream_t]),
+    'dpp_fc_head_ok': (C.c_int, [C.c_int] * 4),
+    'dpp_fc_head_slices': (C.c_int, [C.c_int]),
+    'dpp_fc_head_fwd': (C.c_int, [C.c_void_p, C.c_int, C.c_void_p, C.c_void_p, C.c_void_p, C.c_void_p, C.c_void_p, C.c_int, C.c_int, C.c_int, C.c_int,
+                                  stream_t]),
+    'dpp_fc_head_bwd': (C.c_int, [C.c_void_p] * 7 + [C.c_int] * 4 + [stream_t]),
     'dpp_reduce_partials': (C.c_int, [C.c_void_p, C.c_int, C.c_int, C.c_void_p, C.c_int, C.c_void_p, stream_t]),
     'dpp_conv3x3': (C.c_int, [C.c_void_p, C.c_int, C.c_int, C.c_int, C.c_int, C.POINTER(Act), C.c_void_p, C.c_int,
                               C.c_void_p, C.c_void_p, C.c_void_p, C.c_int, C.POINTER(Epilogue), C.c_int, stream_t]),
diff --git a/deep-prior-pp_amd/hipdp/ops.py b/deep-prior-pp_amd/hipdp/ops.py
--- a/deep-prior-pp_amd/hipdp/ops.py
+++ b/deep-prior-pp_amd/hipdp/ops.py
@@ -313,6 +313,19 @@
     return Launch(rt.lib.dpp_fc_wgrad_stream, (X.ptr, dY.ptr, dW.ptr, int(Nb), int(K), int(N), _actp(actX), _store(b=X)), (X, dY, dW, actX), name, meta)
 
 
+def fc_head_fwd(rt, h1, relu_in, W2, b2, W3, h2pre, slices, M, K, N2, N3, name='fc_head_fwd'):
+    nsl = int(rt.lib.dpp_fc_head_slices(N2))
+    meta = dict(kernel='gemm_mfma_f32', flops=2.0 * M * N2 * (K + N3), bytes=4.0 * (M * K + K * N2 + N2 + N2 * N3 + M * N2 + nsl * M * N3))
+    return Launch(rt.lib.dpp_fc_head_fwd, (h1.ptr, int(bool(relu_in)), W2.ptr, b2.ptr, W3.ptr, h2pre.ptr, slices.ptr, int(M), int(K), int(N2), int(N3)),
+                  (h1, W2, b2, W3, h2pre, slices), name, meta)
+
+
+def fc_head_bwd(rt, dout, W3, h2pre, W2, h1pre, dh2pre, dh1pre, M, K, N2, N3, name='fc_head_bwd'):
+    meta = dict(kernel='gemm_mfma_f32', flops=2.0 * M * N2 * (K + N3), bytes=4.0 * (M * N3 + N2 * N3 + 2.0 * M * N2 + K * N2 + 2.0 * M * K))
+    return Launch(rt.lib.dpp_fc_head_bwd, (dout.ptr, W3.ptr, h2pre.ptr, W2.ptr, h1pre.ptr, dh2pre.ptr, dh1pre.ptr, int(M), int(K), int(N2), int(N3)),
+                  (dout, W3, h2pre, W2, h1pre, dh2pre, dh1pre), name, meta)
+
+
 def reduce_partials(rt, partial, nz, n, out, bias=None, nbias=1, name='reduce_partials'):
     return Launch(rt.lib.dpp_reduce_partials, (partial.ptr, int(nz), int(n), _p(bias), int(nbias), out.ptr),
                   (partial, out, bias), name, dict(kernel='reduce_partials', flops=float(nz) * n, bytes=4.0 * (nz + 1) * n))
diff --git a/include/dpp_hip.h b/include/dpp_hip.h
--- a/include/dpp_hip.h
+++ b/include/dpp_hip.h
@@ -14,7 +14,7 @@
 #define DPP_E_BADARG 10001
 #define DPP_E_UNSUPPORTED 10002
 
-#define DPP_ABI_VERSION 13
+#define DPP_ABI_VERSION 14
 int dpp_abi_version(void);
 
 #define DPP_ST_A 1
@@ -82,6 +82,13 @@
                       float* partial, int store , dpp_stream_t stream);
 
 int dpp_fc_gemm(const dpp_gemm_desc* d, int precision, int kchunk, dpp_stream_t stream);
+
+int dpp_fc_head_ok(int M, int K, int N2, int N3);
+int dpp_fc_head_slices(int N2);
+int dpp_fc_head_fwd(const float* h1, int relu_in, const float* W2, const float* b2, const float* W3, float* h2pre, float* slices, int M,
+                    int K, int N2, int N3, dpp_stream_t stream);
+int dpp_fc_head_bwd(const float* dout, const float* W3, const float* h2pre, const float* W2, const float* h1pre, float* dh2pre,
+                    float* dh1pre, int M, int K, int N2, int N3, dpp_stream_t stream);
 
 int dpp_reduce_partials(const float* partial, int nz, int n, const float* bias, int nbias, float* out,
                         dpp_stream_t stream);
```
